# GadGadGad/Convolutional-KAN-for-Image-Classification

Measured on AMD Instinct MI355X. Metric: images/sec fwd+bwd KAN-VGG11 3x32x32 bs=256/GPU, higher is better.
Workload: dtype f32

## Files before the change

convolutional-kan-for-image-classification_amd/_lib.py:

```python
from __future__ import annotations

import ctypes as C
import os
from typing import Optional

_HERE = os.path.dirname(os.path.abspath(__file__))
LIB_PATH = os.environ.get("KANCONV_LIB") or os.path.join(_HERE, "libkanconv.so")

KAN_MAX_PLANES = 16
KAN_MAX_TABLE = 32
KAN_FP_WORDS = 192
BASIS_BSPLINE, BASIS_RBF, BASIS_CHEBY, BASIS_POLY, BASIS_FOURIER, BASIS_RELU, BASIS_GRAM = 0, 1, 2, 3, 4, 5, 6
ACT_NONE, ACT_IDENTITY, ACT_GELU, ACT_SILU, ACT_RELU, ACT_TANH, ACT_SIGMOID, ACT_GELU_TANH = -1, 0, 1, 2, 3, 4, 5, 6
ORDER_QUAD_FWD, ORDER_ROWBLK8_FWD, ORDER_QUAD_BWD_DATA, ORDER_FWD_WEIGHT_SIDE = 1, 2, 4, 8


class KanGeom(C.Structure):
    _fields_ = [(n, C.c_int) for n in ("B", "C", "H", "W", "O", "Ho", "Wo", "kh", "kw", "sh", "sw", "ph", "pw", "dh", "dw", "groups")] + \
               [("x_bstride", C.c_longlong), ("y_bstride", C.c_longlong)]


class KanBasis(C.Structure):
    _fields_ = [("kind", C.c_int), ("n_basis", C.c_int), ("order", C.c_int), ("act", C.c_int),
                ("p0", C.c_float), ("p1", C.c_float), ("table", C.c_float * KAN_MAX_TABLE), ("chan_table", C.c_void_p)]


class KanPlan(C.Structure):
    _fields_ = [(n, C.c_int) for n in ("P", "K", "IPC", "KC", "Kpad", "Opad", "fwd_splits", "bwd_data_splits", "bwd_weight_splits",
                                          "fwd_target", "bwd_data_target", "bwd_weight_target", "x_pm_wanted", "dz_pm_wanted", "bwd_weight_expanded", "row_blocks", "e_pm_wanted", "fwd_expanded", "fwd_halo", "bwd_weight_halo",
                                          "fwd_band", "bwd_weight_band")] + \
               [(n, C.c_longlong) for n in ("packed_weight_bytes", "bwd_data_weight_bytes", "fwd_slab_elems", "bwd_data_slab_elems",
                                            "bwd_weight_slab_elems", "e_pm_elems")]


class KanNormRoute(C.Structure):
    _fields_ = [(n, C.c_int) for n in ("kernel", "G", "EPL", "PPI", "NT", "pool", "lds", "held", "blocks", "strided")]


NORM_GENERIC, NORM_REGS = 0, 1
NORM_POOL_NONE, NORM_POOL_2X2, NORM_POOL_K = 0, 1, 2


class KanWavGeom(C.Structure):
    _fields_ = [(n, C.c_int) for n in ("B", "C", "H", "W", "O", "Ho", "Wo", "kh", "kw", "sh", "sw", "ph", "pw", "dh", "dw", "wavelet")] + \
               [("x_bstride", C.c_longlong), ("u_bstride", C.c_longlong)]


class KanWavRoute(C.Structure):
    _fields_ = [(n, C.c_int) for n in ("TH", "TW", "NIMG", "RH", "RW", "tiles_h", "tiles_w", "fwd_shrunk", "fwd_nimg_cut", "fwd_lds_bytes", "fwd_fits",
                                       "fwd_blocks", "bwd_input_kernel", "bwd_input_blocks", "params_kernel", "passes", "chunks", "BH", "NI", "RU",
                                       "CU", "XP", "UP", "bands", "items", "items_per_chunk", "lds_bytes", "px_per_chunk")]


WAV_BI_TAPS9, WAV_BI_STRIDE1, WAV_BI_STRIDED = 0, 1, 2
WAV_PAR_TILED, WAV_PAR_PIXEL = 0, 1


WAVELETS = {"mexican_hat": 0, "morlet": 1, "dog": 2, "meyer": 3, "shannon": 4}

_P, _I, _LL, _F, _D = C.c_void_p, C.c_int, C.c_longlong, C.c_float, C.c_double
_GP, _BP = C.POINTER(KanGeom), C.POINTER(KanBasis)
SIGNATURES = {
    "kan_version": (C.c_char_p, []),
    "kan_last_error": (C.c_char_p, []),
    "kan_plan": (_I, [_GP, _BP, C.POINTER(KanPlan)]),
    "kan_tile_orders": (_I, [_GP, _BP]),
    "kan_pack_weights": (_I, [_P, _P, _P, _P, _GP, _BP, _P]),
    "kan_pack_weights_iod": (_I, [_P, _P, _P, _GP, _BP, _P]),
    "kan_pack_cacheable": (_I, [_GP, _BP]),
    "kan_pack_weights_cached": (_I, [_P, _P, _P, _P, _GP, _BP, _P, _I, _I, _I, _P]),
    "kan_conv_fwd": (_I, [_P, _P, _P, _P, _GP, _BP, _P, _P]),
    "kan_position_major": (_I, [_P, _P, _I, _I, _I, _LL, _P]),
    "kan_conv_bwd_data": (_I, [_P, _P, _P, _P, _P, _P, _GP, _BP, _P, _P]),
    "kan_conv_bwd_data_params": (_I, [_P, _P, _P, _P, _P, _P, _P, _GP, _BP, _P, _P]),
    "kan_conv_bwd_weight": (_I, [_P, _P, _P, _P, _GP, _BP, _P, _P, _P]),
    "kan_position_major_expanded": (_I, [_P, _P, _GP, _BP, _P]),
    "kan_conv_fwd_expanded": (_I, [_P, _P, _P, _GP, _BP, _P]),
    "kan_conv_fwd_expanded_order": (_I, [_P, _P, _P, _GP, _BP, _P, _I]),
    "kan_conv_bwd_weight_expanded": (_I, [_P, _P, _P, _GP, _BP, _P]),
    "kan_unpack_wgrad": (_I, [_P, _P, _P, _GP, _BP, _P]),
    "kan_unpack_wgrad_iod": (_I, [_P, _P, _GP, _BP, _P]),
    "kan_slab_reduce": (_I, [_P, _I, _LL, _P, _I, _I, _I, _LL, _P]),
    "kan_instnorm_prelu_fwd": (_I, [_P, _I, _LL, _P, _P, _P, _P, _P, _P, _P, _I, _I, _I, _LL, _F, _I, _P]),
    "kan_instnorm_prelu_bwd": (_I, [_P, _P, _P, _P, _P, _P, _P, _P, _P, _P, _P, _I, _I, _I, _LL, _I, _P]),
    "kan_instnorm_prelu_pool_fwd": (_I, [_P, _I, _LL, _P, _P, _P, _P, _P, _P, _P, _P, _I, _I, _I, _I, _LL, _F, _I, _P]),
    "kan_instnorm_prelu_pool_bwd": (_I, [_P, _P, _P, _P, _P, _P, _P, _P, _P, _P, _P, _P, _I, _I, _I, _I, _LL, _I, _P]),
    "kan_instnorm_prelu_poolk_fwd": (_I, [_P, _I, _LL, _P, _P, _P, _P, _P, _P, _P, _P, _I, _I, _I, _I, _LL, _F, _I, _I, _I, _P]),
    "kan_instnorm_prelu_poolk_bwd": (_I, [_P, _P, _P, _P, _P, _P, _P, _P, _P, _P, _P, _P, _I, _I, _I, _I, _LL, _I, _I, _I, _P]),
    "kan_norm_route": (_I, [_I, _I, _I, _I, _I, _LL, _I, _LL, _I, _I, _I, _I, C.POINTER(KanNormRoute)]),
    "kan_batchnorm_workspace_bytes": (_LL, [_I, _I]),
    "kan_batchnorm_prelu_fwd": (_I, [_P, _I, _LL, _P, _P, _P, _P, _P, _P, _P, _P, _P, _P, _P, _I, _I, _I, _I, _LL, _F, _D, _I, _I, _P]),
    "kan_batchnorm_prelu_bwd": (_I, [_P, _P, _P, _P, _P, _P, _P, _P, _P, _P, _P, _P, _P, _I, _I, _I, _I, _LL, _I, _I, _P]),
    "kan_split_supported": (_I, [C.POINTER(KanGeom), C.POINTER(KanBasis)]),
    "kan_split_weight_bytes": (_LL, [C.POINTER(KanGeom), C.POINTER(KanBasis)]),
    "kan_split_pack_weights": (_I, [_P, _P, _P, C.POINTER(KanGeom), C.POINTER(KanBasis), _P]),
    "kan_conv_fwd_split": (_I, [_P, _P, _P, C.POINTER(KanGeom), C.POINTER(KanBasis), _P]),
    "kan_split_bwd_data_weight_bytes": (_LL, [C.POINTER(KanGeom), C.POINTER(KanBasis)]),
    "kan_split_pack_weights_bwd_data": (_I, [_P, _P, _P, C.POINTER(KanGeom), C.POINTER(KanBasis), _P]),
    "kan_conv_bwd_data_split": (_I, [_P, _P, _P, _P, C.POINTER(KanGeom), C.POINTER(KanBasis), _P]),
    "kan_split_bwd_weight_workspace_bytes": (_LL, [C.POINTER(KanGeom), C.POINTER(KanBasis)]),
    "kan_conv_bwd_weight_split": (_I, [_P, _P, _P, _P, _P, C.POINTER(KanGeom), C.POINTER(KanBasis), _P]),
    "kan_wav_fwd": (_I, [_P, _P, _P, _P, _P, C.POINTER(KanWavGeom), _P]),
    "kan_wav_bwd_input": (_I, [_P, _P, _P, _P, _P, _P, C.POINTER(KanWavGeom), _P]),
    "kan_wav_param_workspace": (_LL, [C.POINTER(KanWavGeom)]),
    "kan_wav_bwd_params": (_I, [_P, _P, _P, _P, _P, _P, _P, _P, _P, C.POINTER(KanWavGeom), _P]),
    "kan_wav_route": (_I, [C.POINTER(KanWavGeom), C.POINTER(KanWavRoute)]),
    "kan_adamw_step": (_I, [_P, _P, _P, _P, _LL, _D, _D, _D, _D, _D, _I, _F, _P]),
    "kan_adamw_step_segments": (_I, [_P, _P, _P, _P, _P, _P, _P, _P, _P, _I, _I, _D, _D, _D, _D, _D, _I, _F, _P]),
    "kan_adamw_advance": (_I, [_P, _P, _I, _P]),
    "kan_adamw_step_segments_dev": (_I, [_P, _P, _P, _P, _P, _P, _P, _P, _P, _P, _I, _I, _D, _D, _D, _D, _F, _P]),
    "kan_adamw_dev_args": (_I, [_P, _P, _D, _D, _D, _D, _F, _P, _P]),
    "kan_xent_workspace_bytes": (_LL, [_I]),
    "kan_xent_metrics_bytes": (_LL, [_I]),
    "kan_xent_fwd": (_I, [_P, _P, _I, _I, _P, _P, _P, _P, _P]),
    "kan_xent_bwd": (_I, [_P, _P, _P, _P, _P, _I, _I, _P]),
    "kan_feed_max_image_bytes": (_LL, []),
    "kan_feed_batch": (_I, [_P, _P, _P, _LL, _I, _I, _I, _I, _I, _I, _I, _P, _P, _P, _P, _P]),
    "kan_feed_resize_max_ksize": (_I, []),
    "kan_feed_resize_batch": (_I, [_P, _P, _P, _LL] + [_I] * 10 + [_P, _I] * 4 + [_P, _P, _P, _P, _P]),
}
SIGNATURES_DIGIT_NAMES = {
    "kan_set_u64_table": (_I, [_P, _I, _P, _I, _P]),
}
XENT_HEADER_WORDS = 8

_lib: Optional[C.CDLL] = None


class KanConvError(RuntimeError):
    pass


def load() -> C.CDLL:
    global _lib
    if _lib is None:
        if not os.path.exists(LIB_PATH):
            raise KanConvError(
                f"{LIB_PATH} not found: build it with `python -c 'import __graft_entry__ as g; g.build()'` "
                "(hipcc --offload-arch=gfx950).  There is no CPU / eager fallback for this path.")
        lib = C.CDLL(LIB_PATH)
        for name, (res, args) in {**SIGNATURES, **SIGNATURES_DIGIT_NAMES}.items():
            fn = getattr(lib, name)
            fn.restype, fn.argtypes = res, args
        _lib = lib
    return _lib


def check(rc: int, what: str) -> None:
    if rc != 0:
        msg = load().kan_last_error().decode(errors="replace")
        raise KanConvError(f"{what} failed (rc={rc}): {msg}")


def version() -> str:
    return load().kan_version().decode()
```

convolutional-kan-for-image-classification_amd/csrc/kan_internal.h:

```cpp
#pragma once
#include <type_traits>
#include "kanconv.h"

int kan_fail_msg(const char* fmt, const char* a);
int kan_raise_lds_limit(const void* kernel, int bytes);

enum : int {
    FAST_GENERIC = 0,
    FAST_BSPLINE_SILU = 1,
    FAST_BSPLINE_GELU = 2,
    FAST_RBF8 = 3,
    FAST_CHEBY5 = 4,
    FAST_CHEBY4 = 5,
    FAST_POLY4 = 6,
    FAST_POLY3 = 7,
    FAST_RBF5 = 8,
    FAST_RELU8 = 9,
    FAST_GRAM4 = 10,
    FAST_POLY1 = 11,
    FAST_LAST = 11
};
enum : unsigned {
    ON_TAP_MAJOR = 1u << 0,
    ON_BIG_TILES = 1u << 1,
    ON_HALO_FWD = 1u << 2,
    ON_HALO_BWD_WEIGHT = 1u << 3,
    ON_BAND_FWD = 1u << 4,
    ON_BAND_BWD_WEIGHT = 1u << 5,
    ON_EXPANDED_FWD = 1u << 6,
    ON_EXPANDED = 1u << 7,
    ON_ROWBLK_BWD_DATA = 1u << 8,
};
struct FastSpec {
    int kind, planes;
    bool base;
    bool xn_fwd, xn_bwd;
    int kc;
    unsigned routes;
};
constexpr FastSpec fast_spec(int f) {
    constexpr unsigned bspline = ON_TAP_MAJOR | ON_BIG_TILES | ON_HALO_FWD | ON_HALO_BWD_WEIGHT | ON_BAND_FWD | ON_BAND_BWD_WEIGHT |
                                 ON_EXPANDED_FWD | ON_EXPANDED | ON_ROWBLK_BWD_DATA;
    switch (f) {
        case FAST_BSPLINE_SILU: case FAST_BSPLINE_GELU: return {KAN_BASIS_BSPLINE, 9, true, false, false, 18, bspline};
        case FAST_RBF8: return {KAN_BASIS_RBF, 9, true, true, true, 18, ON_TAP_MAJOR | ON_BAND_FWD | ON_BAND_BWD_WEIGHT};
        case FAST_RBF5: return {KAN_BASIS_RBF, 6, true, true, true, 18, ON_TAP_MAJOR};
        case FAST_CHEBY5: return {KAN_BASIS_CHEBY, 5, false, false, false, 16, ON_TAP_MAJOR | ON_BIG_TILES | ON_BAND_FWD | ON_BAND_BWD_WEIGHT};
        case FAST_CHEBY4: return {KAN_BASIS_CHEBY, 4, false, false, false, 16, ON_TAP_MAJOR | ON_HALO_FWD | ON_BAND_FWD};
        case FAST_POLY4: return {KAN_BASIS_POLY, 5, true, true, false, 16, ON_TAP_MAJOR | ON_BIG_TILES | ON_HALO_FWD | ON_BAND_FWD};
        case FAST_POLY3: return {KAN_BASIS_POLY, 4, true, true, false, 16, ON_TAP_MAJOR};
        case FAST_POLY1: return {KAN_BASIS_POLY, 2, true, true, false, 16, ON_TAP_MAJOR};
        case FAST_RELU8: return {KAN_BASIS_RELU, 9, true, false, false, 16, ON_HALO_FWD | ON_HALO_BWD_WEIGHT | ON_EXPANDED_FWD | ON_EXPANDED};
        case FAST_GRAM4: return {KAN_BASIS_GRAM, 5, true, false, false, 16, ON_HALO_FWD | ON_HALO_BWD_WEIGHT | ON_EXPANDED};
        default: return {-1, 0, false, true, true, 0, 0};
    }
}
constexpr int fast_kind(int f) { return fast_spec(f).kind; }
constexpr int fast_planes(int f) { return fast_spec(f).planes; }
constexpr bool fast_has(int f, unsigned routes) { return (fast_spec(f).routes & routes) == routes && f != FAST_GENERIC; }

template <int V> using IC = std::integral_constant<int, V>;
template <unsigned ROUTES, int F = 1, class Fn>
bool dispatch_fast(int f, Fn&& fn) {
    if constexpr (F > FAST_LAST) {
        return false;
    } else {
        if constexpr (fast_has(F, ROUTES)) {
            if (f == F) { fn(IC<F>{}); return true; }
        }
        return dispatch_fast<ROUTES, F + 1>(f, fn);
    }
}
template <int V, int... REST, class Fn>
void pick(int v, Fn&& fn) {
    if constexpr (sizeof...(REST) == 0) fn(IC<V>{});
    else if (v == V) fn(IC<V>{});
    else pick<REST...>(v, fn);
}
template <class Fn>
void dispatch_kind(int kind, Fn&& fn) {
    pick<KAN_BASIS_BSPLINE, KAN_BASIS_RBF, KAN_BASIS_POLY, KAN_BASIS_FOURIER, KAN_BASIS_RELU, KAN_BASIS_GRAM, KAN_BASIS_CHEBY>(kind, fn);
}

#define KAN_BAND_MAX_TAPS 128
#define KAN_BAND_MAX_PHASES 16
typedef struct KanBandCfg {
    int ok;
    int fast, P, NG, NPLE, NPS;
    int NGR;
    int WO, MO, WP, TO, TP, NT;
    int tiles_o, tiles_p;
    int n_phase, n_taps, n_steps;
    int HC, span_r, OR0, OC0;
    int cells;
    int slots;
    int TS;
    int lds_bytes, wgs_per_cu;
    int fwd_splits;
    int bw_ok, bw_WR, bw_NI, bw_NT, bw_tiles_o, bw_row_tiles, bw_TPI, bw_ptiles, bw_cells, bw_slots, bw_lds_bytes, bw_splits;
    unsigned short bw_ph_rt0[KAN_BAND_MAX_PHASES + 1];
    unsigned char ph_a[KAN_BAND_MAX_PHASES], ph_b[KAN_BAND_MAX_PHASES];
    short ph_tap0[KAN_BAND_MAX_PHASES + 1];
    unsigned short tap_shift[KAN_BAND_MAX_TAPS];
    unsigned short tap_rt[KAN_BAND_MAX_TAPS];
    short tap_step[KAN_BAND_MAX_TAPS], tap_nt[KAN_BAND_MAX_TAPS];
} KanBandCfg;

void kan_band_cfg(const KanGeom* g, const KanBasis* b, int fast, KanBandCfg* cfg);
int kan_band_bwd_weight_launch(const float* dz, const float* x, const float* xn, float* dwp, const KanGeom* g, const KanBasis* b,
                               const KanBandCfg* cfg, int splits, long long slab_elems, void* stream);
int kan_band_fwd_launch(const float* x, const float* xn, const float* wp, float* z, const KanGeom* g, const KanBasis* b,
                        const KanBandCfg* cfg, int splits, long long slab_elems, void* stream);

constexpr int DW_T = 9;
constexpr int DW_MAX_TP = 96;

enum class Route { TAP_MAJOR, DW, BAND, HALO, EXPANDED };

struct FwdCfg { int TO, TP, tiles_o, tiles_p, chunks, splits, slots; };
struct BdCfg { int CH, tiles_c, tiles_p, n_ob, Opad32, chunks, splits; };
struct BwCfg { int TR, TO, tiles_r, tiles_o, chunks, splits, slots; };
struct BwHaloCfg { int R, nimg, spb, n_bands, tiles_r, tiles_o, splits, bands_per_split; };

struct ConvPlan {
    KanPlan pub;
    int fast;
    Route fwd, bwd_data, bwd_weight;
    bool pm_fwd, pm_bwd_data, pm_bwd_weight;
    bool rowblk_bwd_data;
    bool quad_fwd;
    bool quad_bd;
    bool rowblk8_fwd;
    bool fwd_wq;
    bool pmdma_xcd, pm_lpt, pm_xcd;
    FwdCfg fc;
    BdCfg bd;
    BwCfg bw;
    BwHaloCfg bwh;
    KanBandCfg band;
};
int plan_conv(const KanGeom* g, const KanBasis* b, ConvPlan* cp);

int live_taps_out(const KanGeom* g, int hw);
int live_taps_in(const KanGeom* g, int hw);
int live_positions_for_tap(const KanGeom* g, int tap);
int balance_tiles(const int* weight, int n, unsigned short* idx);
```

convolutional-kan-for-image-classification_amd/csrc/kanconv.hip:

```cpp
#include <hip/hip_runtime.h>
#include <cstdio>
#include <cstdlib>
#include <cstring>
#include <cmath>
#include <cstdint>
#include <mutex>
#include <type_traits>
#include <vector>
#include "kanconv.h"
#include "kan_device.h"

#include "kan_common.h"
#include "kan_internal.h"

namespace {


thread_local char g_err[512] = "";
int fail(const char* fmt, const char* a = "") {
    snprintf(g_err, sizeof(g_err), fmt, a);
    return -1;
}
}
int kan_fail_msg(const char* fmt, const char* a) { return fail(fmt, a); }

int kan_raise_lds_limit(const void* kernel, int bytes) {
    struct Raised { const void* kernel; int device, bytes; };
    static std::mutex mu;
    static std::vector<Raised> raised;
    int dev = 0;
    if (hipGetDevice(&dev) != hipSuccess) return -1;
    std::lock_guard<std::mutex> lock(mu);
    for (const Raised& r : raised)
        if (r.kernel == kernel && r.device == dev && r.bytes >= bytes) return 0;
    if (hipFuncSetAttribute(kernel, hipFuncAttributeMaxDynamicSharedMemorySize, bytes) != hipSuccess) return -1;
    raised.push_back(Raised{kernel, dev, bytes});
    return 0;
}
namespace {

struct PackGeo { int O, C, T, P, hb, nb, IPC, KC, Opad, pair, cmajor; FastDiv divT, divNb, divIPC, divP;
                 int band; short tap_step[KAN_BAND_MAX_TAPS], tap_nt[KAN_BAND_MAX_TAPS]; };

__device__ __forceinline__ int wp_row(const PackGeo& q, int tap, int c, int p) {
    if (q.band) {
        const int grp = fastdiv(c, q.divIPC);
        return (q.tap_step[tap] + grp * q.tap_nt[tap]) * q.KC + (c - grp * q.IPC) * q.P + p;
    }
    if (q.pair) return ((c >> 1) * q.T + tap) * q.KC + 2 * p + (c & 1);
    if (q.cmajor) return (c * q.T + tap) * q.P + p;
    const int item = tap * q.C + c;
    const int chunk = fastdiv(item, q.divIPC);
    return chunk * q.KC + (item - chunk * q.IPC) * q.P + p;
}
__device__ __forceinline__ int pack_row(const PackGeo& q, int src_kind, int j) {
    int cq = fastdiv(j, q.divT), tap = j - cq * q.T;
    int c = src_kind == 0 ? cq : fastdiv(cq, q.divNb);
    int p = src_kind == 0 ? 0 : q.hb + (cq - c * q.nb);
    return wp_row(q, tap, c, p);
}

constexpr int FP_LANES = 64;
__global__ __launch_bounds__(256) void k_fingerprint(const float* __restrict__ a, unsigned na, const float* __restrict__ b, unsigned nb,
                                                     unsigned stride, unsigned long long* __restrict__ ring, int cur) {
    __shared__ unsigned part[2][4];
    if (blockIdx.x == 0 && threadIdx.x < FP_LANES) ring[((cur + 1) % 3) * FP_LANES + threadIdx.x] = 0ull;
    unsigned h1 = 0u, h2 = 0u;
    auto fold = [&](unsigned w, unsigned p) { h1 += w * (2u * p + 1u); h2 += __builtin_rotateleft32(w, p & 31u); };
    constexpr int U = 8;
    const unsigned nthreads = gridDim.x * 256u, tid0 = blockIdx.x * 256u + threadIdx.x;
    auto pass = [&](const float* __restrict__ src, unsigned n, unsigned pos_base) {
        const unsigned nfull = n / 4u, ngr = (nfull + stride - 1u) / stride;
        for (unsigned i0 = tid0; i0 < ngr; i0 += nthreads * U) {
            float4 v[U]; unsigned e[U]; bool ok[U];
#pragma unroll
            for (int u = 0; u < U; ++u) {
                const unsigned i = i0 + u * nthreads;
                ok[u] = i < ngr;
                e[u] = (ok[u] ? i : ngr - 1u) * stride * 4u;
                v[u] = *reinterpret_cast<const float4*>(src + e[u]);
            }
#pragma unroll
            for (int u = 0; u < U; ++u) {
                const unsigned p = pos_base + e[u];
                if (ok[u]) { fold(__float_as_uint(v[u].x), p); fold(__float_as_uint(v[u].y), p + 1u); fold(__float_as_uint(v[u].z), p + 2u); fold(__float_as_uint(v[u].w), p + 3u); }
            }
        }
        if (tid0 == 0u) for (unsigned k = nfull * 4u; k < n; ++k) fold(__float_as_uint(src[k]), pos_base + k);
    };
    if (na) pass(a, na, 0u);
    pass(b, nb, na);
#pragma unroll
    for (int off = 32; off >= 1; off >>= 1) { h1 += __shfl_xor(h1, off, 64); h2 += __shfl_xor(h2, off, 64); }
    if ((threadIdx.x & 63) == 0) { part[0][threadIdx.x >> 6] = h1; part[1][threadIdx.x >> 6] = h2; }
    __syncthreads();
    if (threadIdx.x == 0) {
        const unsigned s1 = part[0][0] + part[0][1] + part[0][2] + part[0][3], s2 = part[1][0] + part[1][1] + part[1][2] + part[1][3];
        unsigned* w = reinterpret_cast<unsigned*>(ring + cur * FP_LANES + (blockIdx.x % FP_LANES));
        atomicAdd(w, s1);
        atomicAdd(w + 1, s2);
    }
}
__device__ __forceinline__ bool fp_unchanged(const unsigned long long* fp, int cur) {
    __shared__ int same;
    if (!fp) return false;
    if (threadIdx.x < 64) {
        const int t = threadIdx.x;
        unsigned lo_c = 0, hi_c = 0, lo_p = 0, hi_p = 0;
        if (t < FP_LANES) {
            const unsigned long long c = fp[cur * FP_LANES + t], p = fp[((cur + 2) % 3) * FP_LANES + t];
            lo_c = (unsigned)c; hi_c = (unsigned)(c >> 32); lo_p = (unsigned)p; hi_p = (unsigned)(p >> 32);
        }
#pragma unroll
        for (int off = 32; off >= 1; off >>= 1) {
            lo_c += __shfl_xor(lo_c, off, 64); hi_c += __shfl_xor(hi_c, off, 64);
            lo_p += __shfl_xor(lo_p, off, 64); hi_p += __shfl_xor(hi_p, off, 64);
        }
        if (t == 0) same = (lo_c == lo_p && hi_c == hi_p) ? 1 : 0;
    }
    __syncthreads();
    return same != 0;
}

__global__ __launch_bounds__(256) void k_pack(const float* __restrict__ src_base, const float* __restrict__ src_basis,
                                              float* __restrict__ wp, PackGeo q, int nb_base, long long wp_gstride, int tiles_x, int tiles_y,
                                              const unsigned long long* __restrict__ fp, int fp_cur) {
    __shared__ float tile[32][33];
    if (fp_unchanged(fp, fp_cur)) return;
    wp += (size_t)blockIdx.z * wp_gstride;
    const int tx = threadIdx.x & 31, ty = threadIdx.x >> 5;
    for (int tile_id = blockIdx.x; tile_id < tiles_x * tiles_y; tile_id += gridDim.x) {
        const int by = tile_id / tiles_x, bx0 = tile_id - by * tiles_x;
        const int src_kind = bx0 < nb_base ? 0 : 1;
        const int bx = src_kind == 0 ? bx0 : bx0 - nb_base;
        const int J = src_kind == 0 ? q.C * q.T : q.C * q.nb * q.T;
        const float* src = (src_kind == 0 ? src_base : src_basis) + (size_t)blockIdx.z * q.O * J;
        const int j0 = bx * 32, o0 = by * 32;
#pragma unroll
        for (int i = 0; i < 4; ++i) {
            int o = o0 + ty + 8 * i, j = j0 + tx;
            tile[ty + 8 * i][tx] = (o < q.O && j < J) ? src[(size_t)o * J + j] : 0.f;
        }
        __syncthreads();
#pragma unroll
        for (int i = 0; i < 4; ++i) {
            int j = j0 + ty + 8 * i, o = o0 + tx;
            if (j < J && o < q.Opad) wp[(size_t)pack_row(q, src_kind, j) * q.Opad + o] = tile[tx][ty + 8 * i];
        }
        __syncthreads();
    }
}

constexpr int UNPACK_TO = 64, UNPACK_TJ = 32;
__device__ __forceinline__ float4 f4_add(float4 a, float4 b) { return make_float4(a.x + b.x, a.y + b.y, a.z + b.z, a.w + b.w); }
template <int N>
__device__ __forceinline__ void unpack_tail(float4& r0, float4& r1, const float* a0, const float* a1, long long slab_elems) {
    float4 v0[N], v1[N];
#pragma unroll
    for (int i = 0; i < N; ++i) {
        v0[i] = *reinterpret_cast<const float4*>(a0 + (size_t)i * slab_elems);
        v1[i] = *reinterpret_cast<const float4*>(a1 + (size_t)i * slab_elems);
    }
#pragma unroll
    for (int i = 0; i < N; ++i) { r0 = f4_add(r0, v0[i]); r1 = f4_add(r1, v1[i]); }
}
__global__ __launch_bounds__(256) void k_unpack(const float* __restrict__ dwp, float* __restrict__ dst_base, float* __restrict__ dst_basis,
                                                PackGeo q, int nb_base, int n_slabs, long long slab_elems, long long dwp_gstride) {
    __shared__ float tile[UNPACK_TO][UNPACK_TJ + 1];
    const int src_kind = (int)blockIdx.x < nb_base ? 0 : 1;
    const int bx = src_kind == 0 ? blockIdx.x : blockIdx.x - nb_base;
    const int J = src_kind == 0 ? q.C * q.T : q.C * q.nb * q.T;
    dwp += (size_t)blockIdx.z * dwp_gstride;
    float* dst = (src_kind == 0 ? dst_base : dst_basis) + (size_t)blockIdx.z * q.O * J;
    const int j0 = bx * UNPACK_TJ, o0 = blockIdx.y * UNPACK_TO;
    const int ol = 4 * (threadIdx.x & 15), jl = threadIdx.x >> 4;
    const float* a0 = dwp + (size_t)pack_row(q, src_kind, min(j0 + jl, J - 1)) * q.Opad + o0 + ol;
    const float* a1 = dwp + (size_t)pack_row(q, src_kind, min(j0 + jl + 16, J - 1)) * q.Opad + o0 + ol;
    const float4 zero = make_float4(0.f, 0.f, 0.f, 0.f);
    float4 s[2][8];
#pragma unroll
    for (int i = 0; i < 8; ++i) s[0][i] = s[1][i] = zero;
    int sl = 0;
    for (; sl + 8 <= n_slabs; sl += 8) {
        float4 v[2][8];
#pragma unroll
        for (int i = 0; i < 8; ++i) {
            v[0][i] = *reinterpret_cast<const float4*>(a0 + (size_t)(sl + i) * slab_elems);
            v[1][i] = *reinterpret_cast<const float4*>(a1 + (size_t)(sl + i) * slab_elems);
        }
#pragma unroll
        for (int i = 0; i < 8; ++i) { s[0][i] = f4_add(s[0][i], v[0][i]); s[1][i] = f4_add(s[1][i], v[1][i]); }
    }
    {
        const float* b0 = a0 + (size_t)sl * slab_elems;
        const float* b1 = a1 + (size_t)sl * slab_elems;
        switch (n_slabs - sl) {
            case 1: unpack_tail<1>(s[0][0], s[1][0], b0, b1, slab_elems); break;
            case 2: unpack_tail<2>(s[0][0], s[1][0], b0, b1, slab_elems); break;
            case 3: unpack_tail<3>(s[0][0], s[1][0], b0, b1, slab_elems); break;
            case 4: unpack_tail<4>(s[0][0], s[1][0], b0, b1, slab_elems); break;
            case 5: unpack_tail<5>(s[0][0], s[1][0], b0, b1, slab_elems); break;
            case 6: unpack_tail<6>(s[0][0], s[1][0], b0, b1, slab_elems); break;
            case 7: unpack_tail<7>(s[0][0], s[1][0], b0, b1, slab_elems); break;
            default: break;
        }
    }
#pragma unroll
    for (int r = 0; r < 2; ++r) {
        const float4 t = f4_add(f4_add(f4_add(s[r][0], s[r][1]), f4_add(s[r][2], s[r][3])), f4_add(f4_add(s[r][4], s[r][5]), f4_add(s[r][6], s[r][7])));
        const int j = jl + 16 * r;
        tile[ol][j] = t.x; tile[ol + 1][j] = t.y; tile[ol + 2][j] = t.z; tile[ol + 3][j] = t.w;
    }
    __syncthreads();
    const int tx = threadIdx.x & 31, ty = threadIdx.x >> 5;
#pragma unroll
    for (int i = 0; i < UNPACK_TO / 8; ++i) {
        const int o = o0 + ty + 8 * i, j = j0 + tx;
        if (o < q.O && j < J) dst[(size_t)o * J + j] = tile[ty + 8 * i][tx];
    }
}

__global__ __launch_bounds__(256) void k_fold_slabs(float* __restrict__ slabs, int n_slabs, long long slab_elems, long long n) {
    __shared__ float part[4][64];
    const int e = threadIdx.x & 63, sg = threadIdx.x >> 6;
    const long long i = (long long)blockIdx.x * 64 + e;
    float a0 = 0.f, a1 = 0.f, a2 = 0.f, a3 = 0.f;
    if (i < n) {
        const float* p = slabs + i;
        int sl = sg;
        for (; sl + 12 < n_slabs; sl += 16) {
            a0 += p[(size_t)sl * slab_elems]; a1 += p[(size_t)(sl + 4) * slab_elems];
            a2 += p[(size_t)(sl + 8) * slab_elems]; a3 += p[(size_t)(sl + 12) * slab_elems];
        }
        for (; sl < n_slabs; sl += 4) a0 += p[(size_t)sl * slab_elems];
    }
    part[sg][e] = (a0 + a1) + (a2 + a3);
    __syncthreads();
    if (sg == 0 && i < n) slabs[i] = (part[0][e] + part[1][e]) + (part[2][e] + part[3][e]);
}

constexpr int IOD_TO = 256, IOD_PITCH = IOD_TO + 4;

__device__ __forceinline__ float4 iod_ld4(const float* p, bool vec) {
    return vec ? *reinterpret_cast<const float4*>(p) : make_float4(p[0], p[1], p[2], p[3]);
}
__device__ __forceinline__ void iod_st4(float* p, float4 v, bool vec) {
    if (vec) *reinterpret_cast<float4*>(p) = v;
    else { p[0] = v.x; p[1] = v.y; p[2] = v.z; p[3] = v.w; }
}
__device__ __forceinline__ float4 iod_add4(float4 a, float4 b) { return make_float4(a.x + b.x, a.y + b.y, a.z + b.z, a.w + b.w); }

struct IodTile { int c, o0, no, wq; };
__device__ __forceinline__ IodTile iod_tile(const PackGeo& q, long long tile_id, int o_tiles) {
    IodTile t;
    t.c = (int)(tile_id / o_tiles);
    t.o0 = (int)(tile_id - (long long)t.c * o_tiles) * IOD_TO;
    t.no = max(0, min(IOD_TO, q.O - t.o0));
    t.wq = min(IOD_TO, q.Opad - t.o0) >> 2;
    return t;
}

__global__ __launch_bounds__(256) void k_pack_iod(const float* __restrict__ coeffs, float* __restrict__ wp, PackGeo q, int o_tiles, long long n_tiles,
                                                  int vec) {
    __shared__ __attribute__((aligned(16))) float tile[KAN_MAX_PLANES * IOD_PITCH];
    const int n = q.nb, tid = threadIdx.x;
    for (long long tile_id = blockIdx.x; tile_id < n_tiles; tile_id += gridDim.x) {
        const IodTile t = iod_tile(q, tile_id, o_tiles);
        const float* src = coeffs + ((size_t)t.c * q.O + t.o0) * n;
        const int cnt = t.no * n;
        auto put = [&](int f, float v) { const int o = fastdiv(f, q.divNb); tile[(f - o * n) * IOD_PITCH + o] = v; };
        if (vec & 1) {
            for (int f = 4 * tid; f < cnt; f += 1024) {
                const float4 v = *reinterpret_cast<const float4*>(src + f);
                put(f, v.x); put(f + 1, v.y); put(f + 2, v.z); put(f + 3, v.w);
            }
        } else {
            for (int f = tid; f < cnt; f += 256) put(f, src[f]);
        }
        __syncthreads();
        for (int u = tid; u < n * t.wq; u += 256) {
            const int p = t.wq == IOD_TO / 4 ? u >> 6 : u / t.wq, o = 4 * (u - p * t.wq);
            float4 v = *reinterpret_cast<const float4*>(&tile[p * IOD_PITCH + o]);
            if (o + 3 >= t.no) { if (o >= t.no) v.x = 0.f; if (o + 1 >= t.no) v.y = 0.f; if (o + 2 >= t.no) v.z = 0.f; v.w = 0.f; }
            iod_st4(wp + (size_t)wp_row(q, 0, t.c, p) * q.Opad + t.o0 + o, v, vec & 2);
        }
        __syncthreads();
    }
}

__global__ __launch_bounds__(256) void k_unpack_iod(const float* __restrict__ dwp, float* __restrict__ dcoeffs, PackGeo q, int o_tiles, long long n_tiles,
                                                    int n_slabs, long long slab_elems, int vec) {
    __shared__ __attribute__((aligned(16))) float tile[KAN_MAX_PLANES * IOD_PITCH];
    const int n = q.nb, tid = threadIdx.x;
    for (long long tile_id = blockIdx.x; tile_id < n_tiles; tile_id += gridDim.x) {
        const IodTile t = iod_tile(q, tile_id, o_tiles);
        for (int u = tid; u < n * t.wq; u += 256) {
            const int p = t.wq == IOD_TO / 4 ? u >> 6 : u / t.wq, o = 4 * (u - p * t.wq);
            if (o >= t.no) continue;
            const float* a = dwp + (size_t)wp_row(q, 0, t.c, p) * q.Opad + t.o0 + o;
            const bool v2 = vec & 2;
            const float4 z = make_float4(0.f, 0.f, 0.f, 0.f);
            float4 s0 = z, s1 = z, s2 = z, s3 = z, s4 = z, s5 = z, s6 = z, s7 = z;
            int sl = 0;
            for (; sl + 8 <= n_slabs; sl += 8) {
                const float* b = a + (size_t)sl * slab_elems;
                s0 = iod_add4(s0, iod_ld4(b, v2)); s1 = iod_add4(s1, iod_ld4(b + slab_elems, v2));
                s2 = iod_add4(s2, iod_ld4(b + 2 * slab_elems, v2)); s3 = iod_add4(s3, iod_ld4(b + 3 * slab_elems, v2));
                s4 = iod_add4(s4, iod_ld4(b + 4 * slab_elems, v2)); s5 = iod_add4(s5, iod_ld4(b + 5 * slab_elems, v2));
                s6 = iod_add4(s6, iod_ld4(b + 6 * slab_elems, v2)); s7 = iod_add4(s7, iod_ld4(b + 7 * slab_elems, v2));
            }
            for (; sl < n_slabs; ++sl) s0 = iod_add4(s0, iod_ld4(a + (size_t)sl * slab_elems, v2));
            *reinterpret_cast<float4*>(&tile[p * IOD_PITCH + o]) =
                iod_add4(iod_add4(iod_add4(s0, s1), iod_add4(s2, s3)), iod_add4(iod_add4(s4, s5), iod_add4(s6, s7)));
        }
        __syncthreads();
        float* dst = dcoeffs + ((size_t)t.c * q.O + t.o0) * n;
        const int cnt = t.no * n;
        auto get = [&](int f) { const int o = fastdiv(f, q.divNb); return tile[(f - o * n) * IOD_PITCH + o]; };
        if (vec & 1) {
            for (int f = 4 * tid; f < cnt; f += 1024) *reinterpret_cast<float4*>(dst + f) = make_float4(get(f), get(f + 1), get(f + 2), get(f + 3));
        } else {
            for (int f = tid; f < cnt; f += 256) dst[f] = get(f);
        }
        __syncthreads();
    }
}

__global__ __launch_bounds__(256) void k_pack_bwd_data(const float* __restrict__ wp, float* __restrict__ wd, PackGeo q,
                                                       int CH, int n_ct, int Opad32, long long wp_gstride, int tiles_x, int tiles_y,
                                                       const unsigned long long* __restrict__ fp, int fp_cur) {
    __shared__ float tile[32][33];
    if (fp_unchanged(fp, fp_cur)) return;
    const int tap = blockIdx.z;
    const int tx = threadIdx.x & 31, ty = threadIdx.x >> 5;
    const int ncol = n_ct * 128;
    const float* const wp0 = wp; float* const wd0 = wd;
    for (int tile_id = blockIdx.x; tile_id < tiles_x * tiles_y; tile_id += gridDim.x) {
    const int byy = tile_id / tiles_x, bxx = tile_id - byy * tiles_x;
    const int oblk = Opad32 / 32, grp = byy / oblk;
    const int col0 = bxx * 32, o0 = (byy - grp * oblk) * 32;
    wp = wp0 + (size_t)grp * wp_gstride;
    wd = wd0 + (size_t)grp * q.T * Opad32 * ncol;
#pragma unroll
    for (int i = 0; i < 4; ++i) {
        int col = col0 + ty + 8 * i, o = o0 + tx;
        float v = 0.f;
        if (col < ncol) {
            int hf = col >> 6, w = col & 63, cl = fastdiv(w, q.divP), p = w - cl * q.P, c = hf * CH + cl;
            if (cl < CH && c < q.C && o < q.O) {
                v = wp[(size_t)wp_row(q, tap, c, p) * q.Opad + o];
            }
        }
        tile[ty + 8 * i][tx] = v;
    }
    __syncthreads();
#pragma unroll
    for (int i = 0; i < 4; ++i) {
        int o = o0 + ty + 8 * i, col = col0 + tx;
// ... 1210 lines not shown
    };

    f32x16 acc[2][2];
#pragma unroll
    for (int a = 0; a < 2; ++a)
#pragma unroll
        for (int b = 0; b < 2; ++b)
#pragma unroll
            for (int r = 0; r < 16; ++r) acc[a][b][r] = 0.f;

    unsigned tapmask = 0;
    for (int tap = 0; tap < T; ++tap) tapmask |= (tap_alive_out(g, pos, tap) ? 1u : 0u) << tap;
    auto seg = [&](int tap) { return (tap * g.C + 1) / 2; };
    int ch0, ch1;
    {
        const int L = live_step_count(tapmask, T, n_chunks, seg);
        const int S = min((int)gridDim.z, max(1, (L + chunks_per_split - 1) / chunks_per_split));
        if (blk.z >= S) { ch0 = ch1 = n_chunks; }
        else {
            ch0 = blk.z == 0 ? 0 : live_step_pos(tapmask, T, n_chunks, (int)((long long)L * blk.z / S), seg);
            ch1 = blk.z == S - 1 ? n_chunks : live_step_pos(tapmask, T, n_chunks, (int)((long long)L * (blk.z + 1) / S), seg);
        }
    }
    auto next_live = [&](int ch) -> int {
        while (ch < ch1) {
            const int tap = (2 * ch) / g.C;
            if ((tapmask >> tap) & 1u) return ch;
            ch = ((tap + 1) * g.C) / 2;
        }
        return ch1;
    };
    int ch = next_live(ch0);
    if (ch < ch1) issue(ch, 0);
    const int ao = w_o * 64 + (lane & 31), bp = w_p * 64 + (lane & 31);
    for (int cur = 0; ch < ch1; cur ^= 1) {
        asm volatile("s_waitcnt vmcnt(0)" ::: "memory");
        __syncthreads();
        ch = next_live(ch + 1);
        if (ch < ch1) issue(ch, cur ^ 1);
        const unsigned aw = lds_addr(sW + cur * (KC * TO) + kh2 * TO + ao), ae = lds_addr(sE + cur * (KC * TP) + kh2 * TP + bp);
        KAN_MFMA_STEP(KC / 2, aw, TO, ae, TP);
    }

    float* zs = z + (size_t)blk.z * slab_elems;
#pragma unroll
    for (int ni = 0; ni < 2; ++ni) {
        const int b = b0 + w_p * 64 + ni * 32 + (lane & 31);
        if (b >= g.B) continue;
        float* zb = zs + (size_t)b * g.ybs + pos;
#pragma unroll
        for (int mi = 0; mi < 2; ++mi)
#pragma unroll
            for (int r = 0; r < 16; ++r) {
                const int o = o_tile0 + w_o * 64 + mi * 32 + mfma_row(r, lane);
                if (o < g.O) zb[(size_t)o * HoWo] = acc[mi][ni][r];
            }
    }
}

template <int KC>
__global__ __launch_bounds__(256, 4) void k_conv_fwd_pmdma_wq(
    const float* __restrict__ e_pm, const float* __restrict__ wp, float* __restrict__ z, DevGeom g, int Opad, int n_chunks,
    int chunks_per_split, long long slab_elems, unsigned e_bytes, unsigned w_bytes, int tiles_o, int xcd) {
    constexpr int TO = 128, TP = 128, NQ = KC / 2, P = KC / 2, HW = 4;
    __shared__ __attribute__((aligned(16))) float sW[2 * KC * TO];
    __shared__ __attribute__((aligned(16))) float sE[2 * KC * TP];
    const int tid = threadIdx.x, lane = tid & 63;
    const int wave = __builtin_amdgcn_readfirstlane(tid >> 6);
    const int w_o = wave >> 1, w_p = wave & 1, kh2 = lane >> 5;
    const BlockId blk = xcd_block_order(xcd != 0);
    const int grp = blk.y / tiles_o, tiles_b = g.B / TP;
    const int sub = blk.x / tiles_b, b0 = (blk.x - sub * tiles_b) * TP;
    const int o_tile0 = ((blk.y - grp * tiles_o) * 4 + sub) * 32;
    const int pairs = g.C >> 1;
    e_pm += (size_t)grp * g.C * HW * P * g.B;
    z += (size_t)grp * g.O * HW;
    wp += (size_t)grp * n_chunks * KC * Opad;
    const kan_rsrc e_rs = make_rsrc(e_pm, e_bytes), w_rs = make_rsrc(wp, w_bytes);

    unsigned eoff[(NQ + 3) / 4];
#pragma unroll
    for (int j = 0; j < (NQ + 3) / 4; ++j) {
        const int r = min(2 * (j * 4 + wave) + (lane >> 5), KC - 1), cl = r / P, pp = r - cl * P;
        eoff[j] = (unsigned)(((cl * HW) * P + pp) * g.B + (lane & 31) * 4) * 4u;
    }
    unsigned woff;
    {
        const int col = (lane & 31) * 4, q = (col >> 4) & 3, o_l = (col >> 6) * 16 + (col & 15);
        const int tap0 = (1 - (q >> 1)) * 3 + (1 - (q & 1));
        woff = (unsigned)((tap0 * pairs * KC + (lane >> 5)) * Opad + o_l) * 4u;
    }
    auto issue = [&](int p, int pair, int buf) {
        const int se = __builtin_amdgcn_readfirstlane((((2 * pair * HW + p) * P) * g.B + b0) * 4);
        const int sw = __builtin_amdgcn_readfirstlane(((((3 * (p >> 1) + (p & 1)) * pairs + pair) * KC) * Opad + o_tile0) * 4);
        float* dE = sE + buf * (KC * TP);
        float* dW = sW + buf * (KC * TO);
#pragma unroll
        for (int j = 0; j < (NQ + 3) / 4; ++j) {
            const int q = j * 4 + wave;
            if (q < NQ) {
                __builtin_amdgcn_raw_ptr_buffer_load_lds(e_rs, (__attribute__((address_space(3))) void*)(dE + q * 256), 16, (int)eoff[j], se, 0, 0);
                __builtin_amdgcn_raw_ptr_buffer_load_lds(w_rs, (__attribute__((address_space(3))) void*)(dW + q * 256), 16, (int)woff,
                                                         sw + q * 2 * Opad * 4, 0, 0);
            }
        }
    };

    f32x16 acc[2][2];
#pragma unroll
    for (int a = 0; a < 2; ++a)
#pragma unroll
        for (int b = 0; b < 2; ++b)
#pragma unroll
            for (int r = 0; r < 16; ++r) acc[a][b][r] = 0.f;

    int ch0, ch1;
    {
        const int L = HW * pairs;
        const int S = min((int)gridDim.z, max(1, (L + chunks_per_split - 1) / chunks_per_split));
        if (blk.z >= S) { ch0 = ch1 = L; }
        else {
            ch0 = (int)((long long)L * blk.z / S);
            ch1 = blk.z == S - 1 ? L : (int)((long long)L * (blk.z + 1) / S);
        }
    }
    int p = ch0 / pairs, pair = ch0 - p * pairs;
    int ch = ch0;
    if (ch < ch1) issue(p, pair, 0);
    const int ao = w_o * 64 + (lane & 31), bp = w_p * 64 + (lane & 31);
    for (int cur = 0; ch < ch1; cur ^= 1) {
        asm volatile("s_waitcnt vmcnt(0)" ::: "memory");
        __syncthreads();
        ++ch;
        if (++pair == pairs) { pair = 0; ++p; }
        if (ch < ch1) issue(p, pair, cur ^ 1);
        const unsigned aw = lds_addr(sW + cur * (KC * TO) + kh2 * TO + ao), ae = lds_addr(sE + cur * (KC * TP) + kh2 * TP + bp);
        KAN_MFMA_STEP(KC / 2, aw, TO, ae, TP);
    }

    float* zs = z + (size_t)blk.z * slab_elems;
#pragma unroll
    for (int ni = 0; ni < 2; ++ni) {
        const int b = b0 + w_p * 64 + ni * 32 + (lane & 31);
        if (b >= g.B) continue;
        float* zb = zs + (size_t)b * g.ybs;
#pragma unroll
        for (int r = 0; r < 8; ++r) {
            const int o = o_tile0 + w_o * 16 + mfma_row(r, lane);
            if (o < g.O) *reinterpret_cast<float4*>(zb + (size_t)o * 4) = make_float4(acc[0][ni][r], acc[0][ni][r + 8], acc[1][ni][r], acc[1][ni][r + 8]);
        }
    }
}

constexpr int PM_ORDER_MAX = 72;
struct PmOrder { int n, tiles_r_per_tap, xcd; unsigned char tap[PM_ORDER_MAX], z[PM_ORDER_MAX]; int first[PM_ORDER_MAX + 1]; };

typedef float f32x4 __attribute__((ext_vector_type(4)));
__global__ __launch_bounds__(256, 4) void k_conv_bwd_weight_pmdma(
    const float* __restrict__ dz_pm, const float* __restrict__ e_pm, float* __restrict__ dwp, DevGeom g, int P, FastDiv divP, int Krows, int Opad,
    int n_chunks, int chunks_per_split, long long slab_elems, unsigned e_bytes, unsigned dz_bytes, int tiles_o, int max_splits, PmOrder ord) {
    constexpr int TR = 128, TO = 128, KPX = 16, ZB = KPX * TO, AB = KPX * TR;
    __shared__ __attribute__((aligned(16))) float sA[2 * AB];
    __shared__ __attribute__((aligned(16))) float sZ[2 * ZB];
    const int tid = threadIdx.x, lane = tid & 63;
    const int wave = __builtin_amdgcn_readfirstlane(tid >> 6);
    const int w_r = wave >> 1, w_c = wave & 1, kh2 = lane >> 5;
    const int HoWo = g.Ho * g.Wo, HW = g.H * g.W, CP = g.C * P;
    BlockId blk{(int)blockIdx.x, (int)blockIdx.y, (int)blockIdx.z};
    if (ord.n) {
        const int lin = (int)blockIdx.x;
        int e = 0;
        while (e + 1 < ord.n && lin >= ord.first[e + 1]) ++e;
        const int rel0 = lin - ord.first[e], per = ord.first[e + 1] - ord.first[e], ny = per / ord.tiles_r_per_tap;
        const int rel = ((per & 7) == 0 && (ord.first[e] & 7) == 0 && ord.xcd) ? (rel0 & 7) * (per >> 3) + (rel0 >> 3) : rel0;
        const int xr = rel / ny, y = rel - xr * ny;
        blk.x = (int)ord.tap[e] * ord.tiles_r_per_tap + xr; blk.y = y; blk.z = (int)ord.z[e];
    }
    const int grp = blk.y / tiles_o;
    const int k0 = blk.x * TR, o_tile0 = (blk.y - grp * tiles_o) * TO;
    e_pm += (size_t)grp * g.C * HW * P * g.B;
    dz_pm += (size_t)grp * g.O * HoWo * g.B;
    dwp += (size_t)grp * Krows * Opad;
    const int tap = k0 / CP, tr = tap / g.kw, tt = tap - tr * g.kw;
    const kan_rsrc e_rs = make_rsrc(e_pm, e_bytes), dz_rs = make_rsrc(dz_pm, dz_bytes);

    unsigned aoff[2], zoff[2];
#pragma unroll
    for (int j = 0; j < 2; ++j) {
        const int rl = 16 * (wave * 2 + j) + (lane >> 2), cs = (lane & 3) ^ ((rl >> 2) & 3);
        const int row = k0 + rl, rem = min(row, Krows - 1) - tap * CP, c = fastdiv(rem, divP), pp = rem - c * P;
        const unsigned va = (unsigned)(((c * HW) * P + pp) * g.B + cs * 4) * 4u, vz = (unsigned)((o_tile0 + rl) * HoWo * g.B + cs * 4) * 4u;
        aoff[j] = row < Krows ? va : KAN_OOB;
        zoff[j] = o_tile0 + rl < g.O ? vz : KAN_OOB;
    }
    unsigned aA[2][2], bB[2][2];
#pragma unroll
    for (int mi = 0; mi < 2; ++mi) {
        const int rl = w_r * 64 + mi * 32 + (lane & 31), ol = w_c * 64 + mi * 32 + (lane & 31);
#pragma unroll
        for (int h = 0; h < 2; ++h) {
            aA[mi][h] = lds_addr(sA + rl * KPX + (((2 * h + kh2) ^ ((rl >> 2) & 3)) * 4));
            bB[mi][h] = lds_addr(sZ + ol * KPX + (((2 * h + kh2) ^ ((ol >> 2) & 3)) * 4));
        }
    }
    auto issue = [&](int ch, int buf) {
        const int px = ch * KPX, pos = px / g.B, b0 = px - pos * g.B;
        const int ho = pos / g.Wo, wo = pos - ho * g.Wo;
        const int inpos = (ho * g.sh - g.ph + tr * g.dh) * g.W + (wo * g.sw - g.pw + tt * g.dw);
        const int sa = __builtin_amdgcn_readfirstlane((inpos * P * g.B + b0) * 4), sz = __builtin_amdgcn_readfirstlane((pos * g.B + b0) * 4);
        float* dA = sA + buf * AB + wave * (2 * 256);
        float* dZ = sZ + buf * ZB + wave * (2 * 256);
#pragma unroll
        for (int j = 0; j < 2; ++j) {
            __builtin_amdgcn_raw_ptr_buffer_load_lds(e_rs, (__attribute__((address_space(3))) void*)(dA + j * 256), 16, (int)aoff[j], sa, 0, 0);
            __builtin_amdgcn_raw_ptr_buffer_load_lds(dz_rs, (__attribute__((address_space(3))) void*)(dZ + j * 256), 16, (int)zoff[j], sz, 0, 0);
        }
    };

    f32x16 acc[2][2];
#pragma unroll
    for (int a = 0; a < 2; ++a)
#pragma unroll
        for (int b = 0; b < 2; ++b)
#pragma unroll
            for (int r = 0; r < 16; ++r) acc[a][b][r] = 0.f;

    unsigned hwmask = 0;
    for (int hw = 0; hw < HoWo; ++hw) hwmask |= (tap_alive_out(g, hw, tap) ? 1u : 0u) << hw;
    auto seg = [&](int hw) { return (hw * g.B + KPX - 1) / KPX; };
    int ch0, ch1;
    {
        const int L = live_step_count(hwmask, HoWo, n_chunks, seg);
        const int S = min(max_splits, max(1, (L + chunks_per_split - 1) / chunks_per_split));
        if (blk.z >= S) { ch0 = ch1 = n_chunks; }
        else {
            ch0 = blk.z == 0 ? 0 : live_step_pos(hwmask, HoWo, n_chunks, (int)((long long)L * blk.z / S), seg);
            ch1 = blk.z == S - 1 ? n_chunks : live_step_pos(hwmask, HoWo, n_chunks, (int)((long long)L * (blk.z + 1) / S), seg);
        }
    }
    auto next_live = [&](int ch) -> int {
        while (ch < ch1) {
            const int hw = (ch * KPX) / g.B;
            if ((hwmask >> hw) & 1u) return ch;
            ch = ((hw + 1) * g.B) / KPX;
        }
        return ch1;
    };
    int ch = next_live(ch0);
    if (ch < ch1) issue(ch, 0);
#define KAN_RD4(CUR, h_)                                                                                                    \
    asm volatile("ds_read_b128 %0, %4 offset:%8\n\tds_read_b128 %1, %5 offset:%8\n\tds_read_b128 %2, %6 offset:%8\n\tds_read_b128 %3, %7 offset:%8" \
                 : "=&v"(fa[h_][0]), "=&v"(fa[h_][1]), "=&v"(fb[h_][0]), "=&v"(fb[h_][1])                                      \
                 : "v"(aA[0][h_]), "v"(aA[1][h_]), "v"(bB[0][h_]), "v"(bB[1][h_]), "n"((CUR) * AB * 4) : "memory")
#define KAN_PM_HALF(h_)                                                                                                     \
    _Pragma("unroll") for (int e = 0; e < 4; ++e) {                                                                          \
        acc[0][0] = MFMA32(fa[h_][0][e], fb[h_][0][e], acc[0][0]);                                                            \
        acc[0][1] = MFMA32(fa[h_][0][e], fb[h_][1][e], acc[0][1]);                                                            \
        acc[1][0] = MFMA32(fa[h_][1][e], fb[h_][0][e], acc[1][0]);                                                            \
        acc[1][1] = MFMA32(fa[h_][1][e], fb[h_][1][e], acc[1][1]);                                                            \
    }
#define KAN_PM_STEP(CUR)                                                                                     \
    do {                                                                                                     \
        asm volatile("s_waitcnt vmcnt(0)" ::: "memory");                                                     \
        __syncthreads();                                                                                     \
        ch = next_live(ch + 1);                                                                              \
        if (ch < ch1) issue(ch, (CUR) ^ 1);                                                                  \
        f32x4 fa[2][2], fb[2][2];                                                                            \
        KAN_RD4(CUR, 0);                                                                                     \
        KAN_RD4(CUR, 1);                                                                                     \
        asm volatile("s_waitcnt lgkmcnt(4)" : "+v"(fa[0][0]), "+v"(fa[0][1]), "+v"(fb[0][0]), "+v"(fb[0][1]) :: "memory"); \
        KAN_PM_HALF(0)                                                                                       \
        asm volatile("s_waitcnt lgkmcnt(0)" : "+v"(fa[1][0]), "+v"(fa[1][1]), "+v"(fb[1][0]), "+v"(fb[1][1]) :: "memory"); \
        KAN_PM_HALF(1)                                                                                       \
    } while (0)
    static_assert(AB == ZB, "one immediate serves both operands");
    while (ch < ch1) {
        KAN_PM_STEP(0);
        if (ch < ch1) { KAN_PM_STEP(1); }
    }
#undef KAN_PM_STEP
#undef KAN_PM_HALF
#undef KAN_RD4

    float* out = dwp + (size_t)blk.z * slab_elems;
#pragma unroll
    for (int mi = 0; mi < 2; ++mi)
#pragma unroll
        for (int r = 0; r < 16; ++r) {
            const int row = k0 + w_r * 64 + mi * 32 + mfma_row(r, lane);
            if (row >= Krows) continue;
#pragma unroll
            for (int ni = 0; ni < 2; ++ni) {
                const int o = o_tile0 + w_c * 64 + ni * 32 + (lane & 31);
                out[(size_t)row * Opad + o] = acc[mi][ni][r];
            }
        }
}


__device__ __forceinline__ int dw_krow(int tap, int p, int IPC, int KC, int P) {
    const int chunk = tap / IPC;
    return chunk * KC + (tap - chunk * IPC) * P + p;
}

template <int KIND>
__global__ __launch_bounds__(256) void k_dw_fwd(const float* __restrict__ x, const float* __restrict__ xn, const float* __restrict__ wp,
                                                float* __restrict__ z, DevGeom g, DevBasis bs, int Opad, int IPC, int KC, int Kpad) {
    __shared__ float sTab[KAN_MAX_TABLE];
    __shared__ float sWt[DW_MAX_TP * 2];
    const int grp = blockIdx.y, T = g.kh * g.kw, P = bs.P, HoWo = g.Ho * g.Wo, HW = g.H * g.W;
    if (threadIdx.x < KAN_MAX_TABLE) sTab[threadIdx.x] = bs.tab[threadIdx.x];
    for (int i = threadIdx.x; i < T * P * 2; i += 256) {
        const int o = i & 1, tp = i >> 1, tap = tp / P, p = tp - tap * P;
        sWt[i] = o < g.O ? wp[((size_t)grp * Kpad + dw_krow(tap, p, IPC, KC, P)) * Opad + o] : 0.f;
    }
    __syncthreads();
    const int e = blockIdx.x * 256 + threadIdx.x;
    if (e >= g.B * HoWo) return;
    const int b = e / HoWo, hw = e - b * HoWo, ho = hw / g.Wo, wo = hw - ho * g.Wo;
    const size_t xbase = (size_t)b * g.xbs + (size_t)grp * HW;
    float acc0 = 0.f, acc1 = 0.f;
    for (int tap = 0; tap < T; ++tap) {
        const int r = tap / g.kw, t = tap - r * g.kw;
        const int hi = ho * g.sh - g.ph + r * g.dh, wi = wo * g.sw - g.pw + t * g.dw;
        if ((unsigned)hi >= (unsigned)g.H || (unsigned)wi >= (unsigned)g.W) continue;
        const float xa = x[xbase + hi * g.W + wi], xb = xn[xbase + hi * g.W + wi];
        float v[KAN_PMAX];
        kan_planes<KIND, false>(bs, sTab, xa, xb, v);
#pragma unroll
        for (int p = 0; p < KAN_PMAX; ++p)
            if (p < P) { acc0 += v[p] * sWt[(tap * P + p) * 2]; acc1 += v[p] * sWt[(tap * P + p) * 2 + 1]; }
    }
    float* zb = z + (size_t)b * g.ybs + (size_t)grp * g.O * HoWo + hw;
    zb[0] = acc0;
    if (g.O > 1) zb[HoWo] = acc1;
}

template <int KIND>
__global__ __launch_bounds__(256) void k_dw_bwd_data(const float* __restrict__ dz, const float* __restrict__ x, const float* __restrict__ xn,
                                                     const float* __restrict__ wp, float* __restrict__ dx, float* __restrict__ dxn,
                                                     DevGeom g, DevBasis bs, int Opad, int IPC, int KC, int Kpad) {
    __shared__ float sTab[KAN_MAX_TABLE];
    __shared__ float sWt[DW_MAX_TP * 2];
    const int grp = blockIdx.y, T = g.kh * g.kw, P = bs.P, HoWo = g.Ho * g.Wo, HW = g.H * g.W;
    if (threadIdx.x < KAN_MAX_TABLE) sTab[threadIdx.x] = bs.tab[threadIdx.x];
    for (int i = threadIdx.x; i < T * P * 2; i += 256) {
        const int o = i & 1, tp = i >> 1, tap = tp / P, p = tp - tap * P;
        sWt[i] = o < g.O ? wp[((size_t)grp * Kpad + dw_krow(tap, p, IPC, KC, P)) * Opad + o] : 0.f;
    }
    __syncthreads();
    const int e = blockIdx.x * 256 + threadIdx.x;
    if (e >= g.B * HW) return;
    const int b = e / HW, hw = e - b * HW, h = hw / g.W, w = hw - h * g.W;
    const size_t xi = (size_t)b * g.xbs + (size_t)grp * HW + hw;
    float G[KAN_PMAX];
#pragma unroll
    for (int p = 0; p < KAN_PMAX; ++p) G[p] = 0.f;
    for (int tap = 0; tap < T; ++tap) {
        const int r = tap / g.kw, t = tap - r * g.kw;
        const int hn = h + g.ph - r * g.dh, wn = w + g.pw - t * g.dw;
        if (hn < 0 || wn < 0) continue;
        const int ho = hn / g.sh, wo = wn / g.sw;
        if (ho * g.sh != hn || wo * g.sw != wn || ho >= g.Ho || wo >= g.Wo) continue;
        const float* zb = dz + (size_t)b * g.ybs + (size_t)grp * g.O * HoWo + ho * g.Wo + wo;
        const float d0 = zb[0], d1 = g.O > 1 ? zb[HoWo] : 0.f;
#pragma unroll
        for (int p = 0; p < KAN_PMAX; ++p)
            if (p < P) G[p] += d0 * sWt[(tap * P + p) * 2] + d1 * sWt[(tap * P + p) * 2 + 1];
    }
    float d[KAN_PMAX];
    kan_planes<KIND, true>(bs, sTab, x[xi], xn[xi], d);
    float s_base = 0.f, s_bas = 0.f;
#pragma unroll
    for (int p = 0; p < KAN_PMAX; ++p)
        if (p < P) { if (p < bs.hb) s_base += d[p] * G[p]; else s_bas += d[p] * G[p]; }
    if (dxn) { dx[xi] = s_base; dxn[xi] = s_bas; }
    else dx[xi] = s_base + s_bas;
}

template <int KIND>
__global__ __launch_bounds__(256) void k_dw_bwd_weight(const float* __restrict__ dz, const float* __restrict__ x, const float* __restrict__ xn,
                                                       float* __restrict__ dwp, DevGeom g, DevBasis bs, int Krows, int Opad,
                                                       long long slab_elems) {
    __shared__ float sTab[KAN_MAX_TABLE];
    __shared__ float sRed[4][DW_T * KAN_PMAX];
    const int grp = blockIdx.y, T = g.kh * g.kw, P = bs.P, HoWo = g.Ho * g.Wo, HW = g.H * g.W;
    const int lane = threadIdx.x & 63, wave = threadIdx.x >> 6;
    if (threadIdx.x < KAN_MAX_TABLE) sTab[threadIdx.x] = bs.tab[threadIdx.x];
    __syncthreads();
    float* out = dwp + (size_t)blockIdx.x * slab_elems + (size_t)grp * Krows * Opad;
    const int total = g.B * HoWo;
    for (int o = 0; o < g.O; ++o) {
        float acc[DW_T][KAN_PMAX];
#pragma unroll
        for (int a = 0; a < DW_T; ++a)
#pragma unroll
            for (int p = 0; p < KAN_PMAX; ++p) acc[a][p] = 0.f;
        for (int e = blockIdx.x * 256 + threadIdx.x; e < total; e += gridDim.x * 256) {
            const int b = e / HoWo, hw = e - b * HoWo, ho = hw / g.Wo, wo = hw - ho * g.Wo;
            const float dzv = dz[(size_t)b * g.ybs + (size_t)(grp * g.O + o) * HoWo + hw];
            const size_t xbase = (size_t)b * g.xbs + (size_t)grp * HW;
#pragma unroll
            for (int tap = 0; tap < DW_T; ++tap) {
                if (tap < T) {
                    const int r = tap / g.kw, t = tap - r * g.kw;
                    const int hi = ho * g.sh - g.ph + r * g.dh, wi = wo * g.sw - g.pw + t * g.dw;
                    if ((unsigned)hi < (unsigned)g.H && (unsigned)wi < (unsigned)g.W) {
                        float v[KAN_PMAX];
                        kan_planes<KIND, false>(bs, sTab, x[xbase + hi * g.W + wi], xn[xbase + hi * g.W + wi], v);
#pragma unroll
                        for (int p = 0; p < KAN_PMAX; ++p) acc[tap][p] += v[p] * dzv;
                    }
                }
            }
        }
#pragma unroll
        for (int a = 0; a < DW_T; ++a)
#pragma unroll
            for (int p = 0; p < KAN_PMAX; ++p) {
                float v = acc[a][p];
#pragma unroll
                for (int off = 32; off >= 1; off >>= 1) v += __shfl_xor(v, off, 64);
                if (lane == 0) sRed[wave][a * KAN_PMAX + p] = v;
            }
        __syncthreads();
        for (int i = threadIdx.x; i < T * P; i += 256) {
            const int tap = i / P, p = i - tap * P, q = tap * KAN_PMAX + p;
            out[(size_t)i * Opad + o] = (sRed[0][q] + sRed[1][q]) + (sRed[2][q] + sRed[3][q]);
        }
        __syncthreads();
    }
}

__global__ __launch_bounds__(256) void k_slab_reduce(const float* __restrict__ slabs, int n_slabs, long long slab_elems,
                                                     float* __restrict__ out, int Cn, int HW, long long bstride, long long total) {
    const long long plane = (long long)Cn * HW;
    for (long long i = blockIdx.x * 256ll + threadIdx.x; i < total; i += (long long)gridDim.x * 256) {
        long long b = i / plane, rem = i - b * plane;
        size_t a = (size_t)b * bstride + rem;
        float s = 0.f;
        for (int sl = 0; sl < n_slabs; ++sl) s += slabs[a + (size_t)sl * slab_elems];
        out[a] = s;
    }
}


struct PoolGeo { int k, s, Hp, Wp, nc; FastDiv divWp, divS, divK, divNc; int lds; };

template <int G>
// ... 640 lines not shown
            float4 P = ((float4*)p)[i], G = ((const float4*)g)[i], M = ((float4*)m)[i], V = ((float4*)v)[i];
            adam1(P.x, G.x, M.x, V.x, a); adam1(P.y, G.y, M.y, V.y, a); adam1(P.z, G.z, M.z, V.z, a); adam1(P.w, G.w, M.w, V.w, a);
            ((float4*)p)[i] = P; ((float4*)m)[i] = M; ((float4*)v)[i] = V;
        }
        const int t = (n & ~3) + threadIdx.x;
        if (t < n) adam1(p[t], g[t], m[t], v[t], a);
    } else {
        for (int i = threadIdx.x; i < n; i += 256) adam1(p[i], g[i], m[i], v[i], a);
    }
}

__global__ void k_adamw_dev_args(const double* __restrict__ lr_dev, const int* __restrict__ step_dev, AdamHyper h, float* __restrict__ out9) {
    if (threadIdx.x != 0 || blockIdx.x != 0) return;
    const AdamArgs a = adam_args_dev(lr_dev[0], step_dev[0], h);
    out9[0] = a.decay; out9[1] = a.w1; out9[2] = a.b1; out9[3] = a.b2; out9[4] = a.w2; out9[5] = a.gscale; out9[6] = a.inv_bc2_sqrt; out9[7] = a.eps;
    out9[8] = a.neg_step;
}

struct U64x64 { unsigned long long v[64]; };
__global__ __launch_bounds__(64) void k_set_u64_table(unsigned long long* __restrict__ table, int first, int n, U64x64 vals) {
    const int t = threadIdx.x;
    if (t < n) table[first + t] = vals.v[t];
}

#include "wavkan.inc"

}

extern "C" {

const char* kan_version(void) { return "kanconv 0.5 (gfx950, fp32 MFMA 32x32x2, halo forward, 128/256-output tiles)"; }
const char* kan_last_error(void) { return g_err; }

int kan_plan(const KanGeom* geom, const KanBasis* basis, KanPlan* plan) {
    if (!plan) return fail("null plan");
    ConvPlan cp;
    if (int rc = plan_conv(geom, basis, &cp)) return rc;
    *plan = cp.pub;
    return 0;
}

static bool pack_needs_clear(const KanGeom* g, const KanPlan& pl) {
    if (pl.fwd_band) return pl.KC != pl.IPC * pl.P || g->C % pl.IPC != 0;
    return pl.KC != pl.IPC * pl.P || (g->C * g->kh * g->kw) % pl.IPC != 0;
}

static int iod_scope(const KanGeom* g, const KanBasis* b) {
    if (!g || !b) return fail("null geometry or basis");
    if (g->kh != 1 || g->kw != 1) return fail("the [I][O][n] coefficient layout takes 1x1 kernels only");
    if (ngroups(g) != 1) return fail("the [I][O][n] coefficient layout takes one group only");
    if (b->act != KAN_ACT_NONE) return fail("the [I][O][n] coefficient layout has no base branch (act must be KAN_ACT_NONE)");
    return 0;
}
struct IodLaunch { int o_tiles; long long n_tiles; unsigned blocks; };
static IodLaunch iod_launch(const KanGeom* g, const KanPlan& pl) {
    IodLaunch l;
    l.o_tiles = ceil_div(pl.Opad, IOD_TO);
    l.n_tiles = (long long)g->C * l.o_tiles;
    l.blocks = (unsigned)(l.n_tiles < 16384 ? l.n_tiles : 16384);
    return l;
}
static int iod_vec(const void* coeffs, const void* packed, const KanGeom* g, const KanBasis* b) {
    return ((((size_t)coeffs & 15) == 0 && ((long long)g->O * b->n_basis) % 4 == 0) ? 1 : 0) | ((((size_t)packed & 15) == 0) ? 2 : 0);
}

static int pack_weights_impl(const float* w_base, const float* w_basis, float* wp, float* wd, const KanGeom* g, const KanBasis* b,
                             const unsigned long long* fp, int fp_cur, void* stream, bool iod = false) {
    ConvPlan cp;
    if (int rc = plan_conv(g, b, &cp)) return rc;
    const KanPlan& pl = cp.pub;
    const int hb = b->act != KAN_ACT_NONE;
    if ((hb && !w_base) || !w_basis || !wp) return fail("null weight pointer");
    hipStream_t st = (hipStream_t)stream;
    const int T = g->kh * g->kw, NI = g->C * T, G = ngroups(g);
    const long long wp_gs = (long long)pl.Kpad * pl.Opad;
    PackGeo q = pack_geo(g, b, cp, false);
    if (fp && (pack_needs_clear(g, pl) || cp.fwd == Route::DW)) return fail("cached packing is not offered for this geometry (kan_pack_cacheable)");
    if (pl.KC != pl.IPC * pl.P || (pl.fwd_band && pack_needs_clear(g, pl))) {
        if (hipMemsetAsync(wp, 0, (size_t)pl.packed_weight_bytes, st) != hipSuccess) return fail("memset failed");
    } else if (!pl.fwd_band && NI % pl.IPC != 0) {
        if (G > 1) {
            if (hipMemsetAsync(wp, 0, (size_t)pl.packed_weight_bytes, st) != hipSuccess) return fail("memset failed");
        } else {
            size_t off = (size_t)(pl.Kpad - pl.KC) * pl.Opad;
            if (hipMemsetAsync(wp + off, 0, (size_t)pl.KC * pl.Opad * 4, st) != hipSuccess) return fail("memset failed");
        }
    }
    const int nb_base = hb ? ceil_div(g->C * T, 32) : 0;
    const int tiles_x = nb_base + ceil_div(g->C * b->n_basis * T, 32), tiles_y = pl.Opad / 32;
    const long long n_tiles = (long long)tiles_x * tiles_y;
    const long long cap = fp ? 1024 : 4096;
    dim3 grid((unsigned)(n_tiles < cap ? n_tiles : cap), 1, G);
    if (iod) {
        const IodLaunch l = iod_launch(g, pl);
        hipLaunchKernelGGL(k_pack_iod, dim3(l.blocks), dim3(256), 0, st, w_basis, wp, q, l.o_tiles, l.n_tiles, iod_vec(w_basis, wp, g, b));
    } else {
        hipLaunchKernelGGL(k_pack, grid, dim3(256), 0, st, w_base, w_basis, wp, q, nb_base, wp_gs, tiles_x, tiles_y, fp, fp_cur);
    }
    if (wd && cp.bwd_data == Route::DW) {
        if (hipMemcpyAsync(wd, wp, (size_t)pl.packed_weight_bytes, hipMemcpyDeviceToDevice, st) != hipSuccess) return fail("memcpy failed");
    } else if (wd) {
        const BdCfg& c = cp.bd;
        const int bx = c.tiles_c * 4, by = c.Opad32 / 32 * G;
        const long long nt = (long long)bx * by;
        const long long capd = fp ? 128 : 1024;
        dim3 gd((unsigned)(nt < capd ? nt : capd), 1, T);
        hipLaunchKernelGGL(k_pack_bwd_data, gd, dim3(256), 0, st, (const float*)wp, wd, q, c.CH, c.tiles_c, c.Opad32, wp_gs, bx, by, fp, fp_cur);
    }
    return launch_ok("pack");
}

int kan_pack_weights(const float* w_base, const float* w_basis, float* wp, float* wd, const KanGeom* g, const KanBasis* b, void* stream) {
    return pack_weights_impl(w_base, w_basis, wp, wd, g, b, nullptr, 0, stream);
}

int kan_pack_weights_iod(const float* coeffs, float* wp, float* wd, const KanGeom* g, const KanBasis* b, void* stream) {
    if (int rc = iod_scope(g, b)) return rc;
    return pack_weights_impl(nullptr, coeffs, wp, wd, g, b, nullptr, 0, stream, true);
}

int kan_tile_orders(const KanGeom* g, const KanBasis* b) {
    ConvPlan cp;
    if (plan_conv(g, b, &cp)) return 0;
    const bool halo = cp.fwd == Route::HALO;
    return (halo && cp.quad_fwd ? KAN_ORDER_QUAD_FWD : 0) | (halo && cp.rowblk8_fwd ? KAN_ORDER_ROWBLK8_FWD : 0) | (cp.quad_bd ? KAN_ORDER_QUAD_BWD_DATA : 0) |
           (cp.fwd_wq ? KAN_ORDER_FWD_WEIGHT_SIDE : 0);
}

int kan_pack_cacheable(const KanGeom* g, const KanBasis* b) {
    ConvPlan cp;
    if (plan_conv(g, b, &cp)) return 0;
    if ((long long)g->O * g->C * (b->n_basis + 1) * g->kh * g->kw >= (1ll << 31)) return 0;
    return (!pack_needs_clear(g, cp.pub) && cp.fwd != Route::DW && ngroups(g) == 1) ? 1 : 0;
}

int kan_pack_weights_cached(const float* w_base, const float* w_basis, float* wp, float* wd, const KanGeom* g, const KanBasis* b,
                            unsigned long long* ring, int cur, int force, int sample_stride, void* stream) {
    static_assert(KAN_FP_WORDS == 3 * FP_LANES, "ring size");
    if (!ring || cur < 0 || cur > 2 || sample_stride < 1) return fail("bad fingerprint ring arguments");
    if (!kan_pack_cacheable(g, b)) return fail("cached packing is not offered for this geometry (kan_pack_cacheable)");
    const int hb = b->act != KAN_ACT_NONE;
    if ((hb && !w_base) || !w_basis) return fail("null weight pointer");
    if (((size_t)w_basis & 15) || (hb && ((size_t)w_base & 15))) return fail("cached packing needs 16-byte aligned weight tensors");
    const int T = g->kh * g->kw;
    const long long na = hb ? (long long)g->O * g->C * T : 0, nbs = (long long)g->O * g->C * b->n_basis * T;
    const long long groups4 = ((na + 3) / 4 + (nbs + 3) / 4 + sample_stride - 1) / sample_stride;
    long long blocks = (groups4 + 256 * 8 - 1) / (256 * 8); if (blocks > 4096) blocks = 4096; if (blocks < 1) blocks = 1;
    hipLaunchKernelGGL(k_fingerprint, dim3((unsigned)blocks), dim3(256), 0, (hipStream_t)stream, hb ? w_base : w_basis, (unsigned)na, w_basis,
                       (unsigned)nbs, (unsigned)sample_stride, ring, cur);
    if (int rc = launch_ok("fingerprint")) return rc;
    return pack_weights_impl(w_base, w_basis, wp, wd, g, b, force ? nullptr : ring, cur, stream);
}

static int unpack_wgrad_impl(const float* dwp, float* dw_base, float* dw_basis, const KanGeom* g, const KanBasis* b, void* stream, bool iod) {
    ConvPlan cp;
    if (int rc = plan_conv(g, b, &cp)) return rc;
    const KanPlan& pl = cp.pub;
    const int hb = b->act != KAN_ACT_NONE;
    if ((hb && !dw_base) || !dw_basis || !dwp) return fail("null weight-gradient pointer");
    hipStream_t st = (hipStream_t)stream;
    const int T = g->kh * g->kw, G = ngroups(g);
    const long long dwp_gs = (long long)(pl.bwd_weight_band ? pl.Kpad : pl.K) * pl.Opad;
    PackGeo q = pack_geo(g, b, cp, true);
    int n_slabs = pl.bwd_weight_splits;
    if (n_slabs >= 32) {
        hipLaunchKernelGGL(k_fold_slabs, dim3(ceil_div(pl.bwd_weight_slab_elems, 64)), dim3(256), 0, st, const_cast<float*>(dwp), n_slabs,
                           pl.bwd_weight_slab_elems, pl.bwd_weight_slab_elems);
        n_slabs = 1;
    }
    const int nb_base = hb ? ceil_div(g->C * T, UNPACK_TJ) : 0;
    dim3 grid(nb_base + ceil_div(g->C * b->n_basis * T, UNPACK_TJ), ceil_div(g->O, UNPACK_TO), G);
    if (iod) {
        const IodLaunch l = iod_launch(g, pl);
        hipLaunchKernelGGL(k_unpack_iod, dim3(l.blocks), dim3(256), 0, st, dwp, dw_basis, q, l.o_tiles, l.n_tiles, n_slabs, pl.bwd_weight_slab_elems,
                           iod_vec(dw_basis, dwp, g, b));
    } else {
        hipLaunchKernelGGL(k_unpack, grid, dim3(256), 0, st, dwp, dw_base, dw_basis, q, nb_base, n_slabs, pl.bwd_weight_slab_elems, dwp_gs);
    }
    return launch_ok("unpack");
}

int kan_unpack_wgrad(const float* dwp, float* dw_base, float* dw_basis, const KanGeom* g, const KanBasis* b, void* stream) {
    return unpack_wgrad_impl(dwp, dw_base, dw_basis, g, b, stream, false);
}

int kan_unpack_wgrad_iod(const float* dwp, float* dcoeffs, const KanGeom* g, const KanBasis* b, void* stream) {
    if (int rc = iod_scope(g, b)) return rc;
    return unpack_wgrad_impl(dwp, nullptr, dcoeffs, g, b, stream, true);
}

int kan_position_major(const float* src, float* dst, int B, int Cn, int HW, long long bstride, void* stream) {
    if (!src || !dst || B < 1 || Cn < 1 || HW < 1) return fail("bad position_major arguments");
    dim3 grid(ceil_div((long long)Cn * HW, 32), ceil_div(B, 32));
    hipLaunchKernelGGL(k_position_major, grid, dim3(256), 0, (hipStream_t)stream, src, dst, B, Cn * HW, bstride);
    return launch_ok("position_major");
}

int kan_conv_fwd(const float* x, const float* xn, const float* wp, float* z, const KanGeom* g, const KanBasis* b, const float* x_pm,
                 void* stream) {
    ConvPlan cp;
    if (int rc = plan_conv(g, b, &cp)) return rc;
    const KanPlan& pl = cp.pub;
    if (!x || !xn || !wp || !z) return fail("null tensor pointer");
    if ((b->kind == KAN_BASIS_RELU || b->kind == KAN_BASIS_GRAM) && !b->chan_table) return fail("ReLU / Gram bases need their device parameter table (chan_table)");
    hipStream_t st = (hipStream_t)stream;
    if (cp.fwd == Route::DW) {
        DevGeom dgd = dev_geom(g); DevBasis dbd = dev_basis(b);
        dim3 grid(ceil_div((long long)g->B * g->Ho * g->Wo, 256), ngroups(g));
        dispatch_kind(b->kind, [&](auto kind) {
            hipLaunchKernelGGL((k_dw_fwd<decltype(kind)::value>), grid, dim3(256), 0, st, x, xn, wp, z, dgd, dbd, pl.Opad, pl.IPC, pl.KC, pl.Kpad);
        });
        return launch_ok("dw_fwd");
    }
    if (cp.fwd == Route::BAND) {
        if (x != xn && !fast_spec(cp.fast).xn_fwd) return fail("this basis / activation pair runs on single-input kernels: pass xn == x");
        return kan_band_fwd_launch(x, xn, wp, z, g, b, &cp.band, pl.fwd_splits, pl.fwd_slab_elems, stream);
    }
    const FwdCfg& c = cp.fc;
    if ((long long)c.tiles_o * ngroups(g) > 65535) return fail("groups * output tiles exceed the grid limit");
    const unsigned x_bytes = (unsigned)((long long)g->B * g->x_bstride * 4);
    if (cp.fwd == Route::HALO) {
        if (x != xn) return fail("internal: halo forward kernel needs a single input tensor");
        DevGeom dgh = dev_geom(g); DevBasis dbh = dev_basis(b);
        const int n_pairs = g->C / 2, pps = ceil_div(n_pairs, pl.fwd_splits);
        dim3 gridh(c.tiles_p, c.tiles_o * ngroups(g), pl.fwd_splits);
        dispatch_fast<ON_HALO_FWD>(cp.fast, [&](auto fv) {
            constexpr int F = decltype(fv)::value;
            auto launch = [&](auto wo, auto w, auto r, auto nimg, auto quad) {
                constexpr int WOV = decltype(wo)::value;
                hipLaunchKernelGGL((k_conv_fwd_halo<F, WOV, decltype(w)::value, decltype(r)::value, decltype(nimg)::value, decltype(quad)::value>), gridh,
                                   dim3(WOV * 128), 0, st, x, wp, z, dgh, dbh, pl.Opad, n_pairs, pps, pl.fwd_slab_elems, x_bytes, c.tiles_o);
            };
            auto planes = [&](auto wo) {
                if constexpr (decltype(wo)::value == 4) {
                    if (g->W == 4 && cp.quad_fwd && ((uintptr_t)z & 7u) == 0 && (g->y_bstride & 1) == 0 && (pl.fwd_slab_elems & 1) == 0)
                        return launch(wo, IC<4>{}, IC<4>{}, IC<8>{}, IC<1>{});
                }
                if (g->W == 32) launch(wo, IC<32>{}, IC<4>{}, IC<1>{}, IC<0>{});
                else if (g->W == 16) launch(wo, IC<16>{}, IC<8>{}, IC<1>{}, IC<0>{});
                else if (g->W == 8) {
                    if constexpr (decltype(wo)::value == 4) {
                        if (cp.rowblk8_fwd) return launch(wo, IC<8>{}, IC<4>{}, IC<4>{}, IC<0>{});
                    }
                    launch(wo, IC<8>{}, IC<8>{}, IC<2>{}, IC<0>{});
                }
                else launch(wo, IC<4>{}, IC<4>{}, IC<8>{}, IC<0>{});
            };
            if constexpr (fast_has(F, ON_BIG_TILES)) {
                if (c.TO == 256) return planes(IC<4>{});
            }
            planes(IC<2>{});
        });
        return launch_ok("conv_fwd_halo");
    }
    DevGeom dg = dev_geom(g);
    dg.pix_major = (x_pm && x == xn && cp.pm_fwd) ? 1 : 0;
    if (dg.pix_major) { x = x_pm; xn = x_pm; }
    DevBasis db = dev_basis(b);
    dim3 grid(c.tiles_p, c.tiles_o * ngroups(g), pl.fwd_splits);
    const int cps = dg.pix_major ? pl.fwd_target : ceil_div(c.chunks, pl.fwd_splits);
    TilePerm perm; perm.n = 0;
    if (dg.pix_major) perm = tile_perm(c.tiles_p, [&](int t) {
        const int hw = (int)(((long long)t * c.TP) / g->B);
        return ceil_div(live_taps_out(g, hw < g->Ho * g->Wo ? hw : 0) * ceil_div(g->C, pl.IPC), cps > 0 ? cps : 1);
    });
    if (x != xn && !fast_spec(cp.fast).xn_fwd)
        return fail("this basis / activation pair runs on single-input kernels: pass xn == x");
    auto launch = [&](auto kind, auto fast, auto wo, auto kc) {
        constexpr int WO = decltype(wo)::value;
        hipLaunchKernelGGL((k_conv_fwd<decltype(kind)::value, decltype(fast)::value, WO, 2, decltype(kc)::value>), grid, dim3(WO * 2 * 64), 0, st,
                           x, xn, wp, z, dg, db, pl.Opad, pl.IPC, c.chunks, cps, pl.fwd_slab_elems, x_bytes, perm, c.tiles_o);
    };
    const bool fast = dispatch_fast<ON_TAP_MAJOR>(cp.fast, [&](auto fv) {
        constexpr int F = decltype(fv)::value;
        if constexpr (fast_has(F, ON_BIG_TILES)) {
            if (c.TO == 256) return launch(IC<fast_kind(F)>{}, fv, IC<4>{}, IC<fast_spec(F).kc>{});
        }
        if (c.TO == 128) launch(IC<fast_kind(F)>{}, fv, IC<2>{}, IC<fast_spec(F).kc>{});
        else launch(IC<fast_kind(F)>{}, fv, IC<1>{}, IC<fast_spec(F).kc>{});
    });
    if (!fast) dispatch_kind(b->kind, [&](auto kind) {
        pick<18, 12, 16>(pl.KC, [&](auto kc) {
            if (c.TO == 128) launch(kind, IC<FAST_GENERIC>{}, IC<2>{}, kc);
            else launch(kind, IC<FAST_GENERIC>{}, IC<1>{}, kc);
        });
    });
    return launch_ok("conv_fwd");
}

static int conv_bwd_data_impl(const float* dz, const float* x, const float* xn, const float* wd, float* dx, float* dxn, float* dpar,
                              const KanGeom* g, const KanBasis* b, const float* dz_pm, void* stream);

int kan_conv_bwd_data(const float* dz, const float* x, const float* xn, const float* wd, float* dx, float* dxn,
                      const KanGeom* g, const KanBasis* b, const float* dz_pm, void* stream) {
    return conv_bwd_data_impl(dz, x, xn, wd, dx, dxn, nullptr, g, b, dz_pm, stream);
}

int kan_conv_bwd_data_params(const float* dz, const float* x, const float* xn, const float* wd, float* dx, float* dxn, float* dparams,
                             const KanGeom* g, const KanBasis* b, const float* dz_pm, void* stream) {
    if (!dparams) return fail("null dparams");
    if (b && b->kind != KAN_BASIS_RELU && b->kind != KAN_BASIS_GRAM) return fail("kan_conv_bwd_data_params: only the ReLU-KAN and GRAM bases accumulate parameter gradients in this launch");
    return conv_bwd_data_impl(dz, x, xn, wd, dx, dxn, dparams, g, b, dz_pm, stream);
}

static int conv_bwd_data_impl(const float* dz, const float* x, const float* xn, const float* wd, float* dx, float* dxn, float* dpar,
                              const KanGeom* g, const KanBasis* b, const float* dz_pm, void* stream) {
    ConvPlan cp;
    if (int rc = plan_conv(g, b, &cp)) return rc;
    const KanPlan& pl = cp.pub;
    if (dpar && cp.bwd_data == Route::DW) return fail("kan_conv_bwd_data_params: depthwise layers take the weight-gradient route");
    if (!dz || !x || !xn || !wd || !dx) return fail("null tensor pointer");
    if ((b->kind == KAN_BASIS_RELU || b->kind == KAN_BASIS_GRAM) && !b->chan_table) return fail("ReLU / Gram bases need their device parameter table (chan_table)");
    if (!dxn && x != xn) return fail("dxn is required when xn != x");
    hipStream_t st = (hipStream_t)stream;
    if (cp.bwd_data == Route::DW) {
        DevGeom dgd = dev_geom(g); DevBasis dbd = dev_basis(b);
        dim3 grid(ceil_div((long long)g->B * g->H * g->W, 256), ngroups(g));
        dispatch_kind(b->kind, [&](auto kind) {
            hipLaunchKernelGGL((k_dw_bwd_data<decltype(kind)::value>), grid, dim3(256), 0, st, dz, x, xn, wd, dx, dxn, dgd, dbd, pl.Opad, pl.IPC, pl.KC, pl.Kpad);
        });
        return launch_ok("dw_bwd_data");
    }
    const BdCfg& c = cp.bd;
    DevGeom dg = dev_geom(g);
    dg.pix_major = (dz_pm && cp.pm_bwd_data) ? 1 : 0;
    if (dg.pix_major) dz = dz_pm;
    DevBasis db = dev_basis(b);
    if ((long long)c.tiles_c * ngroups(g) > 65535) return fail("groups * channel tiles exceed the grid limit");
    dim3 grid(c.tiles_p, c.tiles_c * ngroups(g), pl.bwd_data_splits);
    const int cps = dg.pix_major ? pl.bwd_data_target : ceil_div(c.chunks, pl.bwd_data_splits);
    TilePerm perm; perm.n = 0;
    if (dg.pix_major) perm = tile_perm(c.tiles_p, [&](int t) {
        const int hw = (int)(((long long)t * 128) / g->B);
        return ceil_div(live_taps_in(g, hw < g->H * g->W ? hw : 0) * c.n_ob, cps > 0 ? cps : 1);
    });
    const int fast = (fast_spec(cp.fast).xn_bwd ? (x != xn && dxn) : (x == xn && !dxn)) ? cp.fast : FAST_GENERIC;
    const bool rb = !dg.pix_major && cp.rowblk_bwd_data;
    const bool quad = rb && cp.quad_bd && dz_pm && x == xn && !dxn;
    const unsigned dz_bytes = (unsigned)((long long)g->B * g->y_bstride * 4);
    auto launch = [&](auto kind, auto fast, auto rbv) {
        hipLaunchKernelGGL((k_conv_bwd_data<decltype(kind)::value, decltype(fast)::value, decltype(rbv)::value>), grid, dim3(256), 0, st,
                           decltype(rbv)::value == 2 ? dz_pm : dz, x, xn, wd,
                           dx, dxn, dg, db, c.CH, c.tiles_c, c.n_ob, c.Opad32, c.chunks, cps, pl.bwd_data_slab_elems, dz_bytes, perm, dpar);
    };
    const bool launched = dispatch_fast<ON_TAP_MAJOR>(fast, [&](auto fv) {
        constexpr int F = decltype(fv)::value;
        if constexpr (fast_has(F, ON_ROWBLK_BWD_DATA)) {
            if (quad) return launch(IC<fast_kind(F)>{}, fv, IC<2>{});
            if (rb) return launch(IC<fast_kind(F)>{}, fv, IC<1>{});
        }
        launch(IC<fast_kind(F)>{}, fv, IC<0>{});
    });
    if (!launched) dispatch_kind(b->kind, [&](auto kind) { launch(kind, IC<FAST_GENERIC>{}, IC<0>{}); });
    return launch_ok("conv_bwd_data");
}

int kan_conv_bwd_weight(const float* dz, const float* x, const float* xn, float* dwp, const KanGeom* g, const KanBasis* b,
                        const float* x_pm, const float* dz_pm, void* stream) {
    ConvPlan cp;
    if (int rc = plan_conv(g, b, &cp)) return rc;
    const KanPlan& pl = cp.pub;
    if (!dz || !x || !xn || !dwp) return fail("null tensor pointer");
    if ((b->kind == KAN_BASIS_RELU || b->kind == KAN_BASIS_GRAM) && !b->chan_table) return fail("ReLU / Gram bases need their device parameter table (chan_table)");
    hipStream_t st = (hipStream_t)stream;
    if (cp.bwd_weight == Route::DW) {
        DevGeom dgd = dev_geom(g); DevBasis dbd = dev_basis(b);
        dim3 grid(pl.bwd_weight_splits, ngroups(g));
        dispatch_kind(b->kind, [&](auto kind) {
            hipLaunchKernelGGL((k_dw_bwd_weight<decltype(kind)::value>), grid, dim3(256), 0, st, dz, x, xn, dwp, dgd, dbd, pl.K, pl.Opad, pl.bwd_weight_slab_elems);
        });
        return launch_ok("dw_bwd_weight");
    }
    if (cp.bwd_weight == Route::BAND) {
        if (x != xn && !fast_spec(cp.fast).xn_fwd) return fail("this basis / activation pair runs on single-input kernels: pass xn == x");
        return kan_band_bwd_weight_launch(dz, x, xn, dwp, g, b, &cp.band, pl.bwd_weight_splits, pl.bwd_weight_slab_elems, stream);
    }
    const unsigned x_bytes = (unsigned)((long long)g->B * g->x_bstride * 4), dz_bytes = (unsigned)((long long)g->B * g->y_bstride * 4);
    if (cp.bwd_weight == Route::HALO) {
        if (x != xn) return fail("internal: the channel-major weight-gradient layout needs x == xn");
        const BwHaloCfg& hc = cp.bwh;
        const DevGeom dgh = dev_geom(g); const DevBasis dbh = dev_basis(b);
        if ((long long)hc.tiles_o * ngroups(g) > 65535) return fail("groups * output tiles exceed the grid limit");
        dim3 grid(hc.tiles_r, hc.tiles_o * ngroups(g), hc.splits);
        dispatch_fast<ON_HALO_BWD_WEIGHT>(cp.fast, [&](auto fv) {
            auto launch = [&](auto w, auto r, auto nimg) {
                hipLaunchKernelGGL((k_conv_bwd_weight_halo<decltype(fv)::value, decltype(w)::value, decltype(r)::value, decltype(nimg)::value>), grid,
                                   dim3(256), 0, st, dz, x, dwp, dgh, dbh, pl.K, pl.Opad, hc.n_bands, hc.bands_per_split, pl.bwd_weight_slab_elems,
                                   x_bytes, dz_bytes, hc.tiles_o);
            };
            if (g->W == 16) launch(IC<16>{}, IC<4>{}, IC<1>{});
            else if (g->W == 8) launch(IC<8>{}, IC<8>{}, IC<1>{});
            else launch(IC<4>{}, IC<4>{}, IC<2>{});
        });
        return launch_ok("conv_bwd_weight_halo");
    }
    const BwCfg& c = cp.bw;
    DevGeom dg = dev_geom(g);
    dg.pix_major = (x_pm && dz_pm && x == xn && cp.pm_bwd_weight) ? 1 : 0;
    if (dg.pix_major) { x = x_pm; xn = x_pm; dz = dz_pm; }
    DevBasis db = dev_basis(b);
    if ((long long)c.tiles_o * ngroups(g) > 65535) return fail("groups * output tiles exceed the grid limit");
    dim3 grid(c.tiles_r, c.tiles_o * ngroups(g), pl.bwd_weight_splits);
    const int cps = dg.pix_major ? pl.bwd_weight_target : ceil_div(c.chunks, pl.bwd_weight_splits);
    if (x != xn && !fast_spec(cp.fast).xn_fwd)
        return fail("this basis / activation pair runs on single-input kernels: pass xn == x");
    auto launch = [&](auto kind, auto fast, auto wr, auto wc) {
        constexpr int WR = decltype(wr)::value, WC = decltype(wc)::value;
        hipLaunchKernelGGL((k_conv_bwd_weight<decltype(kind)::value, decltype(fast)::value, WR, WC>), grid, dim3(WR * WC * 64), 0, st, dz, x, xn, dwp,
                           dg, db, pl.K, pl.Opad, c.chunks, cps, pl.bwd_weight_slab_elems, x_bytes, dz_bytes, c.tiles_o);
    };
    auto tiles = [&](auto kind, auto fast) {
        if (c.TO == 128) launch(kind, fast, IC<2>{}, IC<2>{});
        else launch(kind, fast, IC<4>{}, IC<1>{});
    };
    const bool fast = dispatch_fast<ON_TAP_MAJOR>(cp.fast, [&](auto fv) {
        constexpr int F = decltype(fv)::value;
        if constexpr (fast_has(F, ON_BIG_TILES)) {
            if (c.TO == 256) return launch(IC<fast_kind(F)>{}, fv, IC<2>{}, IC<4>{});
        }
        tiles(IC<fast_kind(F)>{}, fv);
    });
    if (!fast) dispatch_kind(b->kind, [&](auto kind) { tiles(kind, IC<FAST_GENERIC>{}); });
    return launch_ok("conv_bwd_weight");
}

int kan_position_major_expanded(const float* x, float* e_pm, const KanGeom* g, const KanBasis* b, void* stream) {
    ConvPlan cp;
    if (int rc = plan_conv(g, b, &cp)) return rc;
    const KanPlan& pl = cp.pub;
    if (!x || !e_pm) return fail("null tensor pointer");
    if (!pl.e_pm_wanted) return fail("this geometry / basis does not use the expanded position-major copy (plan.e_pm_wanted)");
    const int G = ngroups(g), CHW = G * g->C * g->H * g->W;
    DevBasis db = dev_basis(b);
    dim3 grid(ceil_div(CHW, 32), ceil_div(g->B, 32));
    float* dump = e_pm + (pl.e_pm_elems - 256);
    if ((b->kind == KAN_BASIS_RELU || b->kind == KAN_BASIS_GRAM) && !b->chan_table) return fail("ReLU / Gram bases need their device parameter table (chan_table)");
    dispatch_fast<ON_EXPANDED>(cp.fast, [&](auto fv) {
        constexpr int F = decltype(fv)::value;
        hipLaunchKernelGGL((k_expand_pm<fast_kind(F), F>), grid, dim3(256), 0, (hipStream_t)stream, x, e_pm, db, g->B, CHW, g->H * g->W, g->C, g->x_bstride, dump);
    });
    return launch_ok("position_major_expanded");
}

static int conv_fwd_expanded_impl(const float* e_pm, const float* wp, float* z, const KanGeom* g, const KanBasis* b, void* stream, int order) {
    ConvPlan cp;
    if (int rc = plan_conv(g, b, &cp)) return rc;
    const KanPlan& pl = cp.pub;
    if (!e_pm || !wp || !z) return fail("null tensor pointer");
    if (cp.fwd != Route::EXPANDED) return fail("the forward of this geometry / basis does not read the expanded position-major copy (plan.fwd_expanded)");
    if (order >= 0 && order != 0 && order != KAN_ORDER_FWD_WEIGHT_SIDE) return fail("order must be 0 or KAN_ORDER_FWD_WEIGHT_SIDE");
    if (order == KAN_ORDER_FWD_WEIGHT_SIDE && !cp.fwd_wq) return fail("this geometry does not offer the weight-side order (kan_tile_orders)");
    const FwdCfg& c = cp.fc;
    DevGeom dg = dev_geom(g);
    dg.pix_major = 1;
    if ((long long)c.tiles_o * ngroups(g) > 65535) return fail("groups * output tiles exceed the grid limit");
    if (order < 0 ? cp.fwd_wq : order != 0) {
        if ((size_t)z & 15) return fail("the weight-side forward stores 16-byte groups: z must be 16-byte aligned");
        dim3 grid(c.tiles_p, c.tiles_o * ngroups(g), pl.fwd_splits);
        hipLaunchKernelGGL((k_conv_fwd_pmdma_wq<18>), grid, dim3(256), 0, (hipStream_t)stream, e_pm, wp, z, dg, pl.Opad, c.chunks, pl.fwd_target,
                           pl.fwd_slab_elems, (unsigned)(((long long)pl.e_pm_elems - 256) * 4), (unsigned)((long long)pl.Kpad * pl.Opad * 4), c.tiles_o,
                           cp.pmdma_xcd ? 1 : 0);
        return launch_ok("conv_fwd_expanded");
    }
    TilePerm perm; perm.n = 0;
    if (!cp.pmdma_xcd) {
        const int tpp = ceil_div(g->B, c.TP), cpt = ceil_div(g->C, pl.IPC);
        perm = tile_perm(c.tiles_p, [&](int t) { return live_taps_out(g, t / tpp) * cpt; });
    }
    dim3 grid(c.tiles_p, c.tiles_o * ngroups(g), pl.fwd_splits);
    hipLaunchKernelGGL((k_conv_fwd_pmdma<18>), grid, dim3(256), 0, (hipStream_t)stream, e_pm, wp, z, dg, pl.P, make_fastdiv(pl.P), pl.Opad, c.chunks,
                       pl.fwd_target, pl.fwd_slab_elems, (unsigned)(((long long)pl.e_pm_elems - 256) * 4),
                       (unsigned)((long long)pl.Kpad * pl.Opad * 4), perm, c.tiles_o, cp.pmdma_xcd ? 1 : 0);
    return launch_ok("conv_fwd_expanded");
}

int kan_conv_fwd_expanded(const float* e_pm, const float* wp, float* z, const KanGeom* g, const KanBasis* b, void* stream) {
    return conv_fwd_expanded_impl(e_pm, wp, z, g, b, stream, -1);
}

int kan_conv_fwd_expanded_order(const float* e_pm, const float* wp, float* z, const KanGeom* g, const KanBasis* b, void* stream, int order) {
    if (order < 0) return fail("order must be 0 or KAN_ORDER_FWD_WEIGHT_SIDE");
    return conv_fwd_expanded_impl(e_pm, wp, z, g, b, stream, order);
}

int kan_conv_bwd_weight_expanded(const float* dz_pm, const float* e_pm, float* dwp, const KanGeom* g, const KanBasis* b, void* stream) {
    ConvPlan cp;
    if (int rc = plan_conv(g, b, &cp)) return rc;
    const KanPlan& pl = cp.pub;
    if (!dz_pm || !e_pm || !dwp) return fail("null tensor pointer");
    if (cp.bwd_weight != Route::EXPANDED) return fail("the weight gradient of this geometry / basis does not read the expanded position-major copy (plan.bwd_weight_expanded)");
    const BwCfg& c = cp.bw;
    DevGeom dg = dev_geom(g);
    dg.pix_major = 1;
    if ((long long)c.tiles_o * ngroups(g) > 65535) return fail("groups * output tiles exceed the grid limit");
    dim3 grid(c.tiles_r, c.tiles_o * ngroups(g), pl.bwd_weight_splits);
    PmOrder ord; ord.n = 0; ord.xcd = 0;
    const int T = g->kh * g->kw, S = pl.bwd_weight_splits, trpt = (g->C * pl.P) / 128;
    if (cp.pm_lpt && T * S <= PM_ORDER_MAX && T <= 255 && S <= 255 && trpt * T == c.tiles_r) {
        int steps[PM_ORDER_MAX], idx[PM_ORDER_MAX], n = 0;
        unsigned char tp[PM_ORDER_MAX], zz[PM_ORDER_MAX];
        const int per_pos = ceil_div(g->B, 16), tgt = pl.bwd_weight_target > 0 ? pl.bwd_weight_target : 1;
        for (int tap = 0; tap < T; ++tap) {
            const int L = live_positions_for_tap(g, tap) * per_pos;
            int St = ceil_div(L, tgt); St = St < 1 ? 1 : St; St = St > S ? S : St;
            for (int z = 0; z < S; ++z) {
                steps[n] = z < St ? (int)((long long)L * (z + 1) / St - (long long)L * z / St) : 0;
                tp[n] = (unsigned char)tap; zz[n] = (unsigned char)z; idx[n] = n; ++n;
            }
        }
        for (int i = 1; i < n; ++i) {
            const int v = idx[i]; int j = i;
            while (j > 0 && steps[idx[j - 1]] < steps[v]) { idx[j] = idx[j - 1]; --j; }
            idx[j] = v;
        }
        const int per_entry = trpt * c.tiles_o * ngroups(g);
        ord.n = n; ord.tiles_r_per_tap = trpt; ord.xcd = cp.pm_xcd ? 1 : 0;
        for (int i = 0; i < n; ++i) { ord.tap[i] = tp[idx[i]]; ord.z[i] = zz[idx[i]]; ord.first[i] = i * per_entry; }
        ord.first[n] = n * per_entry;
        grid = dim3((unsigned)(n * per_entry), 1, 1);
    }
    hipLaunchKernelGGL(k_conv_bwd_weight_pmdma, grid, dim3(256), 0, (hipStream_t)stream, dz_pm, e_pm, dwp, dg, pl.P, make_fastdiv(pl.P), pl.K, pl.Opad, c.chunks,
                       pl.bwd_weight_target, pl.bwd_weight_slab_elems, (unsigned)(((long long)pl.e_pm_elems - 256) * 4),
                       (unsigned)((long long)g->B * g->y_bstride * 4), c.tiles_o, pl.bwd_weight_splits, ord);
    return launch_ok("conv_bwd_weight_expanded");
}

int kan_slab_reduce(const float* slabs, int n_slabs, long long slab_elems, float* out, int B, int Cn, int HW, long long bstride, void* stream) {
    if (!slabs || !out || n_slabs < 1) return fail("bad slab_reduce arguments");
    long long total = (long long)B * Cn * HW;
    int blocks = (int)((total + 255) / 256); if (blocks > 4096) blocks = 4096; if (blocks < 1) blocks = 1;
    hipLaunchKernelGGL(k_slab_reduce, dim3(blocks), dim3(256), 0, (hipStream_t)stream, slabs, n_slabs, slab_elems, out, Cn, HW, bstride, total);
    return launch_ok("slab_reduce");
}

static bool norm_float2_ok(const void* z, const void* z_out, long long bstride, int HW, long long slab_elems) {
    return ((bstride | HW) & 1) == 0 && (((size_t)z | (size_t)z_out) & 7) == 0 && (slab_elems & 1) == 0;
}
static int norm_pool_mode(const void* pidx, const PoolGeo& pg) { return !pidx ? KAN_NORM_POOL_NONE : pg.k ? KAN_NORM_POOL_K : KAN_NORM_POOL_2X2; }

static int instnorm_fwd_any(const float* z, int n_slabs, long long slab_elems, float* z_out, const float* gamma, const float* beta,
                            const float* prelu_a, float* y, float* mean, float* rstd, int B, int Cn, int HW, long long bstride, float eps,
                            int prelu_span, unsigned char* pidx, int W, void* stream, PoolGeo pg = PoolGeo{}) {
    if (!z || !z_out || !y || !mean || !rstd || n_slabs < 1 || B < 1 || Cn < 1 || HW < 1) return fail("bad instnorm_fwd arguments");
    hipStream_t st = (hipStream_t)stream;
    int planes = B * Cn;
    const KanNormRoute r = norm_route(false, planes, HW, norm_pool_mode(pidx, pg), norm_float2_ok(z, z_out, bstride, HW, slab_elems));
    bool ok;
    if (r.kernel == KAN_NORM_REGS && r.pool)
        ok = pick_regs_pool2(r, [&](auto v) { launch_in_fwd_regs<decltype(v)::G, decltype(v)::EPL, decltype(v)::PPI, true>(st, r, planes, z, n_slabs, slab_elems, z_out, gamma, beta, prelu_a, y, mean, rstd, Cn, HW, bstride, eps, prelu_span, pidx, W); });
    else if (r.kernel == KAN_NORM_REGS)
        ok = pick_regs_plain(r, [&](auto v) { launch_in_fwd_regs<decltype(v)::G, decltype(v)::EPL, decltype(v)::PPI, false>(st, r, planes, z, n_slabs, slab_elems, z_out, gamma, beta, prelu_a, y, mean, rstd, Cn, HW, bstride, eps, prelu_span, pidx, W); });
    else
        ok = pick_generic(r, [&](auto v) { launch_in_fwd<decltype(v)::G>(st, r, planes, z, n_slabs, slab_elems, z_out, gamma, beta, prelu_a, y, mean, rstd, Cn, HW, bstride, eps, prelu_span, pidx, W, pg); });
    if (!ok) return fail("instnorm_fwd: no kernel for the route");
    return launch_ok("instnorm_fwd");
}

int kan_instnorm_prelu_fwd(const float* z, int n_slabs, long long slab_elems, float* z_out, const float* gamma, const float* beta,
                           const float* prelu_a, float* y, float* mean, float* rstd, int B, int Cn, int HW, long long bstride, float eps,
                           int prelu_span, void* stream) {
    return instnorm_fwd_any(z, n_slabs, slab_elems, z_out, gamma, beta, prelu_a, y, mean, rstd, B, Cn, HW, bstride, eps, prelu_span, nullptr, 0,
                            stream);
}

int kan_instnorm_prelu_pool_fwd(const float* z, int n_slabs, long long slab_elems, float* z_out, const float* gamma, const float* beta,
                                const float* prelu_a, float* y_pooled, unsigned char* pool_idx, float* mean, float* rstd, int B, int Cn,
                                int H, int W, long long bstride, float eps, int prelu_span, void* stream) {
    if (!pool_idx || H < 2 || W < 2 || (H & 1) || (W & 1)) return fail("fused 2x2 max-pool needs even H and W and an index buffer");
    return instnorm_fwd_any(z, n_slabs, slab_elems, z_out, gamma, beta, prelu_a, y_pooled, mean, rstd, B, Cn, H * W, bstride, eps, prelu_span,
                            pool_idx, W, stream);
}

static int instnorm_bwd_any(const float* dy, const float* z, const float* mean, const float* rstd, const float* gamma, const float* beta,
                            const float* prelu_a, float* dz, float* dgamma, float* dbeta, float* dprelu, int B, int Cn, int HW,
                            long long bstride, int prelu_span, const unsigned char* pidx, int W, void* stream, PoolGeo pg = PoolGeo{}) {
    if (!dy || !z || !mean || !rstd || !dz || B < 1 || Cn < 1 || HW < 1) return fail("bad instnorm_bwd arguments");
    hipStream_t st = (hipStream_t)stream;
    int planes = B * Cn;
    const KanNormRoute r = norm_route(true, planes, HW, norm_pool_mode(pidx, pg), true);
    bool ok;
    if (r.kernel == KAN_NORM_REGS)
        ok = pick_regs_plain(r, [&](auto v) { launch_in_bwd_regs<decltype(v)::G, decltype(v)::EPL, decltype(v)::PPI>(st, r, planes, dy, z, mean, rstd, gamma, beta, prelu_a, dz, dgamma, dbeta, dprelu, Cn, HW, bstride, prelu_span, pidx, W); });
    else
        ok = pick_generic(r, [&](auto v) { launch_in_bwd<decltype(v)::G>(st, r, planes, dy, z, mean, rstd, gamma, beta, prelu_a, dz, dgamma, dbeta, dprelu, Cn, HW, bstride, prelu_span, pidx, W, pg); });
    if (!ok) return fail("instnorm_bwd: no kernel for the route");
    return launch_ok("instnorm_bwd");
}

int kan_instnorm_prelu_bwd(const float* dy, const float* z, const float* mean, const float* rstd, const float* gamma, const float* beta,
                           const float* prelu_a, float* dz, float* dgamma, float* dbeta, float* dprelu, int B, int Cn, int HW,
                           long long bstride, int prelu_span, void* stream) {
    return instnorm_bwd_any(dy, z, mean, rstd, gamma, beta, prelu_a, dz, dgamma, dbeta, dprelu, B, Cn, HW, bstride, prelu_span, nullptr, 0, stream);
}

int kan_instnorm_prelu_pool_bwd(const float* dy_pooled, const unsigned char* pool_idx, const float* z, const float* mean, const float* rstd,
                                const float* gamma, const float* beta, const float* prelu_a, float* dz, float* dgamma, float* dbeta,
                                float* dprelu, int B, int Cn, int H, int W, long long bstride, int prelu_span, void* stream) {
    if (!pool_idx || H < 2 || W < 2 || (H & 1) || (W & 1)) return fail("fused 2x2 max-pool needs even H and W and the forward's index buffer");
    return instnorm_bwd_any(dy_pooled, z, mean, rstd, gamma, beta, prelu_a, dz, dgamma, dbeta, dprelu, B, Cn, H * W, bstride, prelu_span,
                            pool_idx, W, stream);
}

static int pool_geo(int H, int W, int k, int st, PoolGeo* pg) {
    if (k < 2 || k > 15 || st < 1 || st > k || H < k || W < k) return fail("fused max-pool: need 2 <= kernel <= 15, 1 <= stride <= kernel, plane >= kernel");
    pg->k = k; pg->s = st; pg->Hp = (H - k) / st + 1; pg->Wp = (W - k) / st + 1;
    pg->divWp = make_fastdiv(pg->Wp); pg->divS = make_fastdiv(st); pg->divK = make_fastdiv(k); pg->nc = (k + st - 1) / st; pg->divNc = make_fastdiv(pg->nc); pg->lds = 0;
    return 0;
}

int kan_instnorm_prelu_poolk_fwd(const float* z, int n_slabs, long long slab_elems, float* z_out, const float* gamma, const float* beta,
                                 const float* prelu_a, float* y_pooled, unsigned char* pool_idx, float* mean, float* rstd, int B, int Cn,
                                 int H, int W, long long bstride, float eps, int prelu_span, int pool_k, int pool_s, void* stream) {
    PoolGeo pg;
    if (!pool_idx) return fail("fused max-pool needs an index buffer");
    if (pool_geo(H, W, pool_k, pool_s, &pg)) return -1;
    return instnorm_fwd_any(z, n_slabs, slab_elems, z_out, gamma, beta, prelu_a, y_pooled, mean, rstd, B, Cn, H * W, bstride, eps, prelu_span,
                            pool_idx, W, stream, pg);
}

int kan_instnorm_prelu_poolk_bwd(const float* dy_pooled, const unsigned char* pool_idx, const float* z, const float* mean, const float* rstd,
                                 const float* gamma, const float* beta, const float* prelu_a, float* dz, float* dgamma, float* dbeta,
                                 float* dprelu, int B, int Cn, int H, int W, long long bstride, int prelu_span, int pool_k, int pool_s,
                                 void* stream) {
    PoolGeo pg;
    if (!pool_idx) return fail("fused max-pool needs the forward's index buffer");
    if (pool_geo(H, W, pool_k, pool_s, &pg)) return -1;
    return instnorm_bwd_any(dy_pooled, z, mean, rstd, gamma, beta, prelu_a, dz, dgamma, dbeta, dprelu, B, Cn, H * W, bstride, prelu_span,
                            pool_idx, W, stream, pg);
}

int kan_norm_route(int backward, int B, int Cn, int H, int W, long long bstride, int n_slabs, long long slab_elems, int pool2x2, int pool_k,
                   int pool_s, int aligned8, KanNormRoute* route) {
    if (!route || n_slabs < 1 || B < 1 || Cn < 1 || H < 1 || W < 1) return fail("bad norm_route arguments");
    if (pool2x2 && (pool_k || H < 2 || W < 2 || (H & 1) || (W & 1))) return fail("fused 2x2 max-pool needs even H and W");
    PoolGeo pg{};
    if (pool_k && pool_geo(H, W, pool_k, pool_s, &pg)) return -1;
    const int HW = H * W;
    *route = norm_route(backward != 0, B * Cn, HW, pool_k ? KAN_NORM_POOL_K : pool2x2 ? KAN_NORM_POOL_2X2 : KAN_NORM_POOL_NONE,
                        aligned8 && norm_float2_ok(nullptr, nullptr, bstride, HW, slab_elems));
    return 0;
}

int kan_adamw_step(float* p, const float* g, float* m, float* v, long long n, double lr, double beta1, double beta2, double eps,
                   double weight_decay, int step, float grad_scale, void* stream) {
    if (!p || !g || !m || !v) return fail("null tensor pointer");
    if (n < 0 || step < 1) return fail("adamw: n must be >= 0 and step >= 1");
    if (((uintptr_t)p | (uintptr_t)g | (uintptr_t)m | (uintptr_t)v) & 15u) return fail("adamw: blocks must be 16-byte aligned");
    if (n == 0) return 0;
    const AdamArgs a = adam_args(lr, beta1, beta2, eps, weight_decay, step, grad_scale);
    long long blocks = ((n >> 2) + 255) / 256;
    if (blocks > 256 * 16) blocks = 256 * 16;
    if (blocks < 1) blocks = 1;
    hipLaunchKernelGGL(k_adamw, dim3((unsigned)blocks), dim3(256), 0, (hipStream_t)stream, p, g, m, v, n, a);
    return launch_ok("adamw");
}

int kan_adamw_step_segments(float* p, float* m, float* v, const unsigned long long* seg_grad, const long long* seg_off, const int* seg_n,
                            const int* chunk_seg, const int* chunk_start, const float* seg_bias, int n_chunks, int chunk_elems, double lr,
                            double beta1, double beta2, double eps, double weight_decay, int step, float grad_scale, void* stream) {
    if (!p || !m || !v || !seg_grad || !seg_off || !seg_n || !chunk_seg || !chunk_start) return fail("null tensor pointer");
    if (n_chunks < 0 || step < 1 || chunk_elems < 4 || (chunk_elems & 3)) return fail("adamw: bad chunk table or step");
    if (((uintptr_t)p | (uintptr_t)m | (uintptr_t)v) & 15u) return fail("adamw: blocks must be 16-byte aligned");
    if (n_chunks == 0) return 0;
    const AdamArgs a = adam_args(lr, beta1, beta2, eps, weight_decay, step, grad_scale);
    hipLaunchKernelGGL(k_adamw_seg, dim3((unsigned)n_chunks), dim3(256), 0, (hipStream_t)stream, p, m, v, seg_grad, seg_off, seg_n, chunk_seg,
                       chunk_start, seg_bias, chunk_elems, a);
    return launch_ok("adamw_seg");
}

static bool adam_hyper(double beta1, double beta2, double eps, double weight_decay, float grad_scale, AdamHyper* h) {
    if (!(beta1 >= 0.0 && beta1 < 1.0 && beta2 >= 0.0 && beta2 < 1.0) || !(eps >= 0.0) || !(weight_decay >= 0.0)) return false;
    h->beta1 = beta1; h->beta2 = beta2; h->eps = eps; h->weight_decay = weight_decay; h->gscale = grad_scale;
    return true;
}

int kan_adamw_advance(int* seg_step, const unsigned long long* seg_grad, int n_seg, void* stream) {
    if (!seg_step || !seg_grad) return fail("null tensor pointer");
// ... 44 lines not shown
```

convolutional-kan-for-image-classification_amd/ops.py:

```python
from __future__ import annotations

import contextlib
import ctypes as C
import os
import weakref
from collections import OrderedDict
from dataclasses import dataclass, replace
from functools import lru_cache, partial, wraps
from typing import List, NamedTuple, Optional, Sequence, Tuple

import torch
from torch.autograd.function import once_differentiable

from . import _lib as L


@dataclass(frozen=True)
class ConvSpec:
    kind: int
    n_basis: int
    order: int
    act: int
    p0: float
    p1: float
    table: Tuple[float, ...]
    kernel: Tuple[int, int]
    stride: Tuple[int, int]
    padding: Tuple[int, int]
    dilation: Tuple[int, int]
    groups: int = 1
    first: int = 0
    w_layout: int = 0

    @property
    def has_base(self) -> bool:
        return self.act != L.ACT_NONE

    def out_hw(self, H: int, W: int) -> Tuple[int, int]:
        (kh, kw), (sh, sw), (ph, pw), (dh, dw) = self.kernel, self.stride, self.padding, self.dilation
        return (H + 2 * ph - dh * (kh - 1) - 1) // sh + 1, (W + 2 * pw - dw * (kw - 1) - 1) // sw + 1


W_IOD = 1


def _outputs(spec: ConvSpec, w_basis: Sequence[torch.Tensor]) -> int:
    return w_basis[0].shape[1] if spec.w_layout == W_IOD else sum(w.shape[0] for w in w_basis)


def _device_table(spec: ConvSpec) -> bool:
    return spec.kind == L.BASIS_POLY and len(spec.table) > L.KAN_MAX_TABLE


def _basis_struct(spec: ConvSpec) -> L.KanBasis:
    b = L.KanBasis()
    b.kind, b.n_basis, b.act, b.p0, b.p1 = spec.kind, spec.n_basis, spec.act, spec.p0, spec.p1
    b.order = spec.order | (spec.first << 8)
    if _device_table(spec):
        return b
    if len(spec.table) > L.KAN_MAX_TABLE:
        raise L.KanConvError(f"basis table of {len(spec.table)} entries exceeds KAN_MAX_TABLE={L.KAN_MAX_TABLE}")
    for i, v in enumerate(spec.table):
        b.table[i] = v
    return b


@lru_cache(maxsize=512)
def _plan_cached(spec: ConvSpec, B: int, Cg: int, H: int, W: int, Og: int, C_total: int, O_total: int):
    Ho, Wo = spec.out_hw(H, W)
    if Ho <= 0 or Wo <= 0:
        raise L.KanConvError(f"empty output ({Ho}x{Wo}) for input {H}x{W}")
    g = L.KanGeom()
    g.B, g.C, g.H, g.W, g.O, g.Ho, g.Wo = B, Cg, H, W, Og, Ho, Wo
    (g.kh, g.kw), (g.sh, g.sw), (g.ph, g.pw), (g.dh, g.dw) = spec.kernel, spec.stride, spec.padding, spec.dilation
    g.x_bstride, g.y_bstride = C_total * H * W, O_total * Ho * Wo
    g.groups = spec.groups
    b = _basis_struct(spec)
    p = L.KanPlan()
    bp = b
    if _device_table(spec):
        bp = L.KanBasis.from_buffer_copy(b)
        bp.chan_table = 1
    L.check(L.load().kan_plan(C.byref(g), C.byref(bp), C.byref(p)), "kan_plan")
    p.tile_orders = L.load().kan_tile_orders(C.byref(g), C.byref(bp))
    return g, b, p


def _plan_key(spec: ConvSpec, shape, Og: int) -> tuple:
    B, Ct, H, W = shape
    return (spec, B, Ct // spec.groups, H, W, Og, Ct, Og * spec.groups)


def _with_phases(basis: L.KanBasis, phases: Optional[torch.Tensor], mode: int = 0) -> L.KanBasis:
    if phases is None:
        return basis
    b = L.KanBasis.from_buffer_copy(basis)
    b.chan_table, b.order = phases.data_ptr(), mode
    return b


_TABLES: "dict[tuple, torch.Tensor]" = {}


def _with_table(basis: L.KanBasis, spec: ConvSpec, device) -> L.KanBasis:
    if not _device_table(spec):
        return basis
    key = (spec.table, torch.device(device))
    t = _TABLES.get(key)
    if t is None:
        t = _TABLES[key] = torch.tensor(list(spec.table) + [0.0] * 3, dtype=torch.float32, device=device)
    b = L.KanBasis.from_buffer_copy(basis)
    b.chan_table = t.data_ptr()
    return b


def _ptr(t: Optional[torch.Tensor], offset: int = 0) -> C.c_void_p:
    if t is None:
        return C.c_void_p(0)
    return C.c_void_p(t.data_ptr() + 4 * offset)


def _stream(t: torch.Tensor) -> C.c_void_p:
    return C.c_void_p(torch.cuda.current_stream(t.device).cuda_stream)


def _dense(t: torch.Tensor) -> torch.Tensor:
    t = t.contiguous()
    return t.clone() if t.data_ptr() & 15 else t


def _require(t: torch.Tensor, name: str, align: bool = True) -> torch.Tensor:
    if not isinstance(t, torch.Tensor):
        raise L.KanConvError(f"{name} must be a tensor, got {type(t).__name__}")
    if not t.is_cuda:
        raise L.KanConvError(f"{name} is on {t.device}: this path runs only on a ROCm device (MI355X); there is no CPU fallback")
    if t.dtype != torch.float32:
        raise L.KanConvError(f"{name} must be float32, got {t.dtype}")
    return _dense(t) if align else t.contiguous()


def _split_weights(spec: ConvSpec, weights: Sequence[torch.Tensor]):
    G = spec.groups
    if spec.has_base:
        return list(weights[:G]), list(weights[G:2 * G])
    return [None] * G, list(weights[:G])


PROFILE: Optional[list] = None


@dataclass
class KernelSample:
    name: str
    flops: float
    executed: float
    layer: str
    start: "torch.cuda.Event"
    end: "torch.cuda.Event"


def _launch(sample, t: torch.Tensor, fn) -> None:
    name, flops, executed, layer = sample
    if PROFILE is None:
        L.check(fn(), name)
        return
    e0, e1 = torch.cuda.Event(enable_timing=True), torch.cuda.Event(enable_timing=True)
    stream = torch.cuda.current_stream(t.device)
    e0.record(stream)
    L.check(fn(), name)
    e1.record(stream)
    PROFILE.append(KernelSample(name, flops, executed, layer, e0, e1))


def _conv_flops(geom, plan) -> float:
    return 2.0 * geom.B * geom.O * geom.Ho * geom.Wo * geom.C * plan.P * geom.kh * geom.kw * max(1, geom.groups)


@lru_cache(maxsize=256)
def _live_fraction(which: str, H: int, W: int, Ho: int, Wo: int, kh: int, kw: int, sh: int, sw: int, ph: int, pw: int, dh: int, dw: int) -> float:
    live = 0
    for ho in range(Ho):
        for wo in range(Wo):
            for r in range(kh):
                for t in range(kw):
                    hi, wi = ho * sh - ph + r * dh, wo * sw - pw + t * dw
                    live += 0 <= hi < H and 0 <= wi < W
    return live / float(Ho * Wo * kh * kw)


_ROW_BLOCK_BIT = {"fwd": 1, "bwd_data": 2, "bwd_weight": 0}


def _quadrant_order(geom, plan, which: str) -> bool:
    return which == "fwd" and bool(plan.row_blocks & 1) and geom.B % 32 == 0


def _quadrant_bwd_data(geom, plan, have_dz_pm: bool) -> bool:
    return bool(have_dz_pm) and bool(plan.row_blocks & 2) and bool(getattr(plan, "tile_orders", 0) & L.ORDER_QUAD_BWD_DATA)


def _row_blocks8_forward(geom, plan) -> bool:
    return geom.H == 8 and geom.W == 8 and bool(getattr(plan, "tile_orders", 0) & L.ORDER_ROWBLK8_FWD)


def _executed_flops(geom, plan, which: str, have_dz_pm: bool = False) -> float:
    target = {"fwd": plan.fwd_target, "bwd_data": plan.bwd_data_target, "bwd_weight": plan.bwd_weight_target}[which]
    dense = _conv_flops(geom, plan)
    g = geom
    if target <= 0:
        if _quadrant_order(geom, plan, which) or (which == "bwd_data" and _quadrant_bwd_data(geom, plan, have_dz_pm)):
            return dense * _live_fraction(which, g.H, g.W, g.Ho, g.Wo, g.kh, g.kw, g.sh, g.sw, g.ph, g.pw, g.dh, g.dw)
        if plan.row_blocks & _ROW_BLOCK_BIT[which]:
            return dense * (5.0 / 6.0)
        if which == "fwd" and _row_blocks8_forward(geom, plan):
            return dense * (11.0 / 12.0)
        return dense
    return dense * _live_fraction(which, g.H, g.W, g.Ho, g.Wo, g.kh, g.kw, g.sh, g.sw, g.ph, g.pw, g.dh, g.dw)


def _layer_tag(geom) -> str:
    return f"{geom.C * max(1, geom.groups)}->{geom.O * max(1, geom.groups)}@{geom.H}x{geom.W} k{geom.kh}x{geom.kw}"


def _sample(which: str, geom, plan, pm: bool, two: bool = False, expanded: bool = False):
    tile = "128" if plan.Opad % 128 == 0 else "64"
    if which == "bwd_data":
        name = "k_conv_bwd_data"
    elif expanded:
        name = f"k_conv_{which}_pmdma/o{tile}"
    elif plan.fwd_band if which == "fwd" else plan.bwd_weight_band:
        name = f"k_band_{which}/o" + ("128" if plan.Opad % 128 == 0 else "192" if plan.Opad == 192 else "64")
    else:
        halo = plan.fwd_halo if which == "fwd" else (plan.bwd_weight_halo and not two)
        name = f"k_conv_{which}{'_halo' if halo else ''}/o{tile}"
    skips = expanded or pm or bool(plan.row_blocks & _ROW_BLOCK_BIT[which]) or (which == "fwd" and _row_blocks8_forward(geom, plan))
    dense = _conv_flops(geom, plan)
    return name, dense, _executed_flops(geom, plan, which, pm) if skips else dense, _layer_tag(geom)


def _position_major(t: torch.Tensor, ch_off: int, Cn: int) -> torch.Tensor:
    B, Ct, H, W = t.shape
    out = torch.empty(Cn * H * W * B, device=t.device, dtype=torch.float32)
    L.check(L.load().kan_position_major(_ptr(t, ch_off * H * W), _ptr(out), B, Cn, H * W, Ct * H * W, _stream(t)), "kan_position_major")
    return out


def _stack(ws: Sequence[Optional[torch.Tensor]]) -> Optional[torch.Tensor]:
    if ws[0] is None:
        return None
    return ws[0].unsqueeze(0) if len(ws) == 1 else torch.stack(list(ws))


_PACKED: "OrderedDict[tuple, PackedWeights]" = OrderedDict()
_PACK_CACHE_MAX = int(os.environ.get("KAN_PACK_CACHE", "256"))
_PACK_CACHE_BYTES = int(os.environ.get("KAN_PACK_CACHE_BYTES", str(16 << 30)))
_PACK_SAMPLE = max(1, int(os.environ.get("KAN_PACK_SAMPLE", "1")))
_PACK_VERIFY_EVERY = int(os.environ.get("KAN_PACK_VERIFY_EVERY", "16"))
_EPOCH = 0
PACK_STATS = {"calls": 0, "forced": 0, "skipped": 0}


_ALWAYS_PACK = False


@contextlib.contextmanager
def always_pack():
    global _ALWAYS_PACK
    prev, _ALWAYS_PACK = _ALWAYS_PACK, True
    try:
        yield
    finally:
        _ALWAYS_PACK = prev


@dataclass(frozen=True)
class SplitMode:
    inference: bool = False
    fwd: bool = False
    bwd_data: bool = False
    bwd_weight: bool = False


_SPLIT = SplitMode()


@contextlib.contextmanager
def _split(**on):
    global _SPLIT
    prev, _SPLIT = _SPLIT, replace(_SPLIT, **on)
    try:
        yield
    finally:
        _SPLIT = prev


def split_precision_inference():
    return _split(inference=True)


def split_precision_forward():
    return _split(fwd=True)
# ... 197 lines not shown

def _layout_key(spec: "ConvSpec", geom, plan) -> tuple:
    return (spec, geom.C, geom.O, plan.P, plan.IPC, plan.KC, plan.Kpad, plan.Opad, plan.fwd_halo, plan.fwd_band, plan.packed_weight_bytes, plan.bwd_data_weight_bytes)


@lru_cache(maxsize=512)
def _cacheable(plan_key) -> bool:
    geom, basis, _ = _plan_cached(*plan_key)
    return bool(L.load().kan_pack_cacheable(C.byref(geom), C.byref(basis)))


def _owner(w: torch.Tensor) -> torch.Tensor:
    return w._base if w._base is not None else w


def _packed_entry(key, owners):
    ent = _PACKED.get(key)
    if ent is None:
        ent = PackedWeights()
        _PACKED[key] = ent
        for o in owners:
            weakref.finalize(o, _PACKED.pop, key, None)
        while len(_PACKED) > _PACK_CACHE_MAX or (len(_PACKED) > 1 and sum(e.nbytes() for e in _PACKED.values()) > _PACK_CACHE_BYTES):
            _PACKED.popitem(last=False)
    else:
        _PACKED.move_to_end(key)
    return ent


def _pack(lib, spec, geom, basis, plan, plan_key, w_base, w_basis, need_dgrad, phases, device, st):
    def fresh():
        wp = torch.empty(plan.packed_weight_bytes // 4, device=device, dtype=torch.float32)
        wd = torch.empty(plan.bwd_data_weight_bytes // 4, device=device, dtype=torch.float32) if need_dgrad else None
        wb_all, ws_all = _stack(w_base), _stack(w_basis)
        L.check(lib.kan_pack_weights(_ptr(wb_all), _ptr(ws_all), _ptr(wp), _ptr(wd), C.byref(geom), C.byref(basis), st), "kan_pack_weights")
        return wp, wd
    if spec.w_layout == W_IOD:
        wp = torch.empty(plan.packed_weight_bytes // 4, device=device, dtype=torch.float32)
        wd = torch.empty(plan.bwd_data_weight_bytes // 4, device=device, dtype=torch.float32) if need_dgrad else None
        L.check(lib.kan_pack_weights_iod(_ptr(w_basis[0]), _ptr(wp), _ptr(wd), C.byref(geom), C.byref(basis), st), "kan_pack_weights_iod")
        return wp, wd
    if _PACK_CACHE_MAX <= 0 or spec.groups != 1 or phases is not None or not _cacheable(plan_key):
        return fresh()
    ws, wb = w_basis[0], w_base[0]
    if (ws.data_ptr() | (wb.data_ptr() if wb is not None else 0)) & 15:
        return fresh()
    owners = [_owner(w) for w in (wb, ws) if w is not None]
    if not all(o.is_leaf for o in owners):
        return fresh()
    ent = _packed_entry((_layout_key(spec, geom, plan), device.index) + tuple(id(o) for o in owners), owners)
    stamps = [(w.data_ptr(), o._version, tuple(w.shape)) for w, o in zip((w for w in (wb, ws) if w is not None), owners)]
    force = _ALWAYS_PACK or ent.wp is None or ent.stamps != stamps or (need_dgrad and ent.wd is None)
    if ent.wp is None:
        ent.wp = torch.empty(plan.packed_weight_bytes // 4, device=device, dtype=torch.float32)
        ent.ring = torch.zeros(L.KAN_FP_WORDS, device=device, dtype=torch.int64)
    if need_dgrad and ent.wd is None:
        ent.wd = torch.empty(plan.bwd_data_weight_bytes // 4, device=device, dtype=torch.float32)
    if not force and ent.epoch == _EPOCH and _PACK_VERIFY_EVERY != 1 and (_PACK_VERIFY_EVERY == 0 or ent.unverified + 1 < _PACK_VERIFY_EVERY):
        ent.unverified += 1
        PACK_STATS["skipped"] += 1
        return ent.wp, (ent.wd if need_dgrad else None)
    ent.epoch, ent.unverified = _EPOCH, 0
    if force:
        for t in (ent.wp, ent.wd):
            if t is not None:
                torch.autograd.graph.increment_version(t)
    L.check(lib.kan_pack_weights_cached(_ptr(wb), _ptr(ws), _ptr(ent.wp), _ptr(ent.wd), C.byref(geom), C.byref(basis),
                                        C.c_void_p(ent.ring.data_ptr()), ent.cur, int(force), _PACK_SAMPLE, st), "kan_pack_weights_cached")
    PACK_STATS["calls"] += 1
    PACK_STATS["forced"] += int(force)
    ent.cur = (ent.cur + 1) % 3
    ent.stamps = stamps
    return ent.wp, (ent.wd if need_dgrad else None)


def _conv_forward(spec: ConvSpec, x, xn, w_base, w_basis, need_dgrad: bool = True, phases=None):
    lib = L.load()
    Ct = x.shape[1]
    plan_key = _plan_key(spec, x.shape, _outputs(spec, w_basis) // spec.groups)
    geom, basis, plan = _plan_cached(*plan_key)
    basis = _with_table(_with_phases(basis, phases), spec, x.device)
    st = _stream(x)
    z = torch.empty((plan.fwd_splits, geom.B, geom.O * spec.groups, geom.Ho, geom.Wo), device=x.device, dtype=torch.float32)
    wp, wd = _pack(lib, spec, geom, basis, plan, plan_key, w_base, w_basis, need_dgrad, phases, x.device, st)
    if plan.fwd_expanded and xn is None:
        e_pm = _expand_pm(x, geom, basis, plan, st)
        _launch(_sample("fwd", geom, plan, True, expanded=True), x,
                lambda: lib.kan_conv_fwd_expanded(_ptr(e_pm), _ptr(wp), _ptr(z), C.byref(geom), C.byref(basis), st))
        return z, (wd, _position_major(x, 0, Ct) if plan.x_pm_wanted else e_pm), geom, basis, plan
    x_pm = _position_major(x, 0, Ct) if (plan.x_pm_wanted and xn is None) else None
    _launch(_sample("fwd", geom, plan, x_pm is not None, xn is not None), x,
            lambda: lib.kan_conv_fwd(_ptr(x), _ptr(xn if xn is not None else x), _ptr(wp), _ptr(z), C.byref(geom), C.byref(basis),
                                     _ptr(x_pm), st))
    return z, (wd, x_pm), geom, basis, plan


def _expand_pm(x, geom, basis, plan, st):
    e_pm = torch.empty(plan.e_pm_elems, device=x.device, dtype=torch.float32)
    L.check(L.load().kan_position_major_expanded(_ptr(x), _ptr(e_pm), C.byref(geom), C.byref(basis), st), "kan_position_major_expanded")
    return e_pm


class GradSink:
    __slots__ = ("ref", "view", "used")

    def __init__(self, ref, view):
        self.ref, self.view, self.used = ref, view, False


GRAD_SINKS: "dict[int, GradSink]" = {}


def _sink_for(wid, shape, device):
    ent = GRAD_SINKS.get(wid) if wid is not None else None
    if ent is None or ent.used:
        return None
    p, t = ent.ref(), ent.view
    if p is None or p.grad is not None or tuple(t.shape) != tuple(shape) or t.device != device or not t.is_contiguous():
        return None
    ent.used = True
    return t


def _conv_backward(spec: ConvSpec, x, xn, packed, dz, need_x: bool, need_xn: bool, need_w: bool, phases=None, mode: int = 0, wids=None, dparams=None, wcd=None, dw_split: bool = False):
    lib = L.load()
    B, Ct, H, W = x.shape
    G = spec.groups
    Cg = Ct // G
    Ot = dz.shape[1]
    Og = Ot // G
    geom, basis, plan = _plan_cached(*_plan_key(spec, x.shape, Og))
    basis = _with_table(_with_phases(basis, phases, mode), spec, x.device)
    kh, kw = spec.kernel
    st = _stream(x)
    xs = xn if xn is not None else x
    wd, x_pm = packed
    dw_base: List[Optional[torch.Tensor]] = [None] * G
    dw_basis: List[Optional[torch.Tensor]] = [None] * G
    split_w = need_w and dw_split
    split_x = need_x and wcd is not None
    exact_w = need_w and not split_w
    exact_x = (need_x or need_xn) and not split_x
    dz_pm = _position_major(dz, 0, Ot) if (plan.dz_pm_wanted and xn is None and (exact_w or exact_x)) else None
    if split_w:
        sb, ss = (_sink_for(wids[0], (Og, Cg, kh, kw), x.device), _sink_for(wids[1], (Og, Cg * spec.n_basis, kh, kw), x.device)) if wids else (None, None)
        dwb = sb if sb is not None else torch.empty((Og, Cg, kh, kw), device=x.device, dtype=torch.float32)
        dws = ss if ss is not None else torch.empty((Og, Cg * spec.n_basis, kh, kw), device=x.device, dtype=torch.float32)
        kan_conv_bwd_weight_split(spec, x, dz, out=(dwb, dws))
        dw_base, dw_basis = list(dwb.unsqueeze(0).unbind(0)), list(dws.unsqueeze(0).unbind(0))
    elif exact_w:
        dwp = torch.empty(plan.bwd_weight_splits * plan.bwd_weight_slab_elems, device=x.device, dtype=torch.float32)
        if plan.bwd_weight_expanded and xn is None and dz_pm is not None:
            e_pm = x_pm if (plan.fwd_expanded and not plan.x_pm_wanted and x_pm is not None and mode == 0) else _expand_pm(x, geom, basis, plan, st)
            _launch(_sample("bwd_weight", geom, plan, True, expanded=True), x,
                    lambda: lib.kan_conv_bwd_weight_expanded(_ptr(dz_pm), _ptr(e_pm), _ptr(dwp), C.byref(geom), C.byref(basis), st))
        else:
            _launch(_sample("bwd_weight", geom, plan, x_pm is not None and dz_pm is not None, xn is not None), x,
                    lambda: lib.kan_conv_bwd_weight(_ptr(dz), _ptr(x), _ptr(xs), _ptr(dwp), C.byref(geom), C.byref(basis), _ptr(x_pm),
                                                    _ptr(dz_pm), st))
        if spec.w_layout == W_IOD:
            dco = torch.empty((Cg, Og, spec.n_basis), device=x.device, dtype=torch.float32)
            L.check(lib.kan_unpack_wgrad_iod(_ptr(dwp), _ptr(dco), C.byref(geom), C.byref(basis), st), "kan_unpack_wgrad_iod")
            dw_basis = [dco]
        else:
            sb = _sink_for(wids[0], (Og, Cg, kh, kw), x.device) if (wids and G == 1 and spec.has_base) else None
            ss = _sink_for(wids[1], (Og, Cg * spec.n_basis, kh, kw), x.device) if (wids and G == 1) else None
            dwb = (sb.unsqueeze(0) if sb is not None else
                   torch.empty((G, Og, Cg, kh, kw), device=x.device, dtype=torch.float32)) if spec.has_base else None
            dws = ss.unsqueeze(0) if ss is not None else torch.empty((G, Og, Cg * spec.n_basis, kh, kw), device=x.device, dtype=torch.float32)
            L.check(lib.kan_unpack_wgrad(_ptr(dwp), _ptr(dwb), _ptr(dws), C.byref(geom), C.byref(basis), st), "kan_unpack_wgrad")
            dw_basis = list(dws.unbind(0))
            if spec.has_base:
                dw_base = list(dwb.unbind(0))
    dx = dxn = None
    if split_x:
        dx, _ = kan_conv_bwd_data_split(spec, x, dz, None, None, wcd)
    elif exact_x:
        S = plan.bwd_data_splits
        separate = xn is not None
        dxs = torch.empty((S, B, Ct, H, W), device=x.device, dtype=torch.float32)
        dxns = torch.empty_like(dxs) if separate else None
        head, tail = (_ptr(dz), _ptr(x), _ptr(xs), _ptr(wd), _ptr(dxs), _ptr(dxns)), (C.byref(geom), C.byref(basis), _ptr(dz_pm), st)
        _launch(_sample("bwd_data", geom, plan, dz_pm is not None), x,
                (lambda: lib.kan_conv_bwd_data(*head, *tail)) if dparams is None else
                (lambda: lib.kan_conv_bwd_data_params(*head, _ptr(dparams), *tail)))
        dx, dxn = _sum_slabs(dxs, B, Ct, H * W), (_sum_slabs(dxns, B, Ct, H * W) if separate else None)
    return dx, dxn, dw_base, dw_basis


def _sum_slabs(slabs: torch.Tensor, B: int, Cn: int, HW: int) -> torch.Tensor:
    if slabs.shape[0] == 1:
        return slabs[0]
    out = torch.empty_like(slabs[0])
    L.check(L.load().kan_slab_reduce(_ptr(slabs), slabs.shape[0], slabs[0].numel(), _ptr(out), B, Cn, HW, Cn * HW, _stream(slabs)),
            "kan_slab_reduce")
    return out


def _flat_grads(spec: ConvSpec, dw_base, dw_basis):
    return tuple(dw_base) + tuple(dw_basis) if spec.has_base else tuple(dw_basis)


def _save(ctx, **named) -> None:
    ctx.saved_names = tuple(k for k, t in named.items() if t is not None)
    ctx.save_for_backward(*(t for t in named.values() if t is not None))


def _once(backward):
    inner = once_differentiable(backward)

    @wraps(backward)
    def wrapper(ctx, *grads):
        if torch.is_grad_enabled() and not any(g is not None and g.requires_grad for g in grads):
            grads = tuple(g.detach().requires_grad_(True) if g is not None else None for g in grads)
        return inner(ctx, *grads)
    return wrapper


def _asked(ctx, grads: tuple) -> tuple:
    return tuple(g if need else None for g, need in zip(grads, ctx.needs_input_grad))


def _saved(ctx, *names):
    kept = dict(zip(ctx.saved_names, ctx.saved_tensors))
    return tuple(kept.get(n) for n in names)


def _is_depthwise(spec: ConvSpec, x, w_basis) -> bool:
    return x.shape[1] // spec.groups == 1 and w_basis[0].shape[0] <= 2 and spec.kernel[0] * spec.kernel[1] <= 9


class _KanConv(torch.autograd.Function):

    @staticmethod
    def forward(ctx, spec: ConvSpec, split: bool, x, xn, phases, *weights):
        x = _require(x, "x")
        xn = _require(xn, "xn") if xn is not None else None
        weights = [_require(w, "weight", align=False) for w in weights]
        w_base, w_basis = _split_weights(spec, weights)
        if spec.w_layout == W_IOD:
            want = (x.shape[1], w_basis[0].shape[1] if w_basis[0].dim() == 3 else -1, spec.n_basis)
            if len(weights) != 1 or tuple(w_basis[0].shape) != want or spec.groups != 1 or spec.kernel != (1, 1) or spec.has_base or phases is not None:
                raise L.KanConvError(f"w_layout = W_IOD takes one [inputs, outputs, n_basis] coefficient tensor, a 1x1 kernel, one group and no base branch; "
                                     f"got {[tuple(w.shape) for w in weights]} for input {tuple(x.shape)}, n_basis {spec.n_basis}")
        if phases is not None:
            phases = _require(phases, "phases")
            want = (x.shape[1] // spec.groups, 2, spec.n_basis) if spec.kind == L.BASIS_RELU else (spec.n_basis,)
            if tuple(phases.shape) != want:
                raise L.KanConvError(f"parameter table {tuple(phases.shape)} != {want} for basis kind {spec.kind}")
        need_dgrad = bool(ctx.needs_input_grad[2] or (xn is not None and ctx.needs_input_grad[3]))
        need_w = any(ctx.needs_input_grad[5:])
        with torch.cuda.device(x.device):
            zs, (wd, x_pm), _, stage = _conv_forward_or_split(spec, x, xn, phases, w_base, w_basis, split, need_dgrad, need_w)
            z = _sum_slabs(zs, zs.shape[1], zs.shape[2], zs.shape[3] * zs.shape[4])
        ctx.spec, ctx.wsplit = spec, stage.dw_split
        kept_w = {f"w_basis{g}": w for g, w in enumerate(w_basis)} if phases is not None else {}
        _save(ctx, x=x, xn=xn, phases=phases, wd=wd, x_pm=x_pm, wcd=stage.wcd, **kept_w)
        return z

    @staticmethod
    @_once
    def backward(ctx, dz):
        spec, G = ctx.spec, ctx.spec.groups
        x, xn, phases, wd, x_pm, wcd, *w_basis = _saved(ctx, "x", "xn", "phases", "wd", "x_pm", "wcd", *(f"w_basis{g}" for g in range(G)))
        packed = (wd, x_pm)
        need_x, need_xn = ctx.needs_input_grad[2], xn is not None and ctx.needs_input_grad[3]
        need_p, need_w = ctx.needs_input_grad[4], any(ctx.needs_input_grad[5:])
        dz = _dense(dz)
        dph = None
        with torch.cuda.device(x.device):
            in_epilogue = need_p and (need_x or need_xn) and not _is_depthwise(spec, x, w_basis)
            dpar = None
            if in_epilogue:
                dpar = torch.zeros_like(phases) if spec.kind == L.BASIS_RELU else phases.new_zeros((64, spec.n_basis))
            dx, dxn, dwb, dws = _conv_backward(spec, x, xn, packed, dz, need_x, need_xn, need_w, phases, dparams=dpar, wcd=wcd, dw_split=ctx.wsplit)
            if in_epilogue:
                dph = dpar if spec.kind == L.BASIS_RELU else dpar.sum(dim=0)
            if need_p and not in_epilogue:
                Cg, n = x.shape[1] // G, spec.n_basis
                W = torch.stack(list(w_basis)).view(G, -1, Cg, n, spec.kernel[0] * spec.kernel[1])

                def factor(mode):
                    _, _, _, dwm = _conv_backward(spec, x, xn, packed, dz, False, False, True, phases, mode)
                    return W * torch.stack(list(dwm)).view_as(W)
                if spec.kind == L.BASIS_RELU:
                    dph = torch.stack([factor(mode).sum(dim=(0, 1, 4)) for mode in (1, 2)], dim=1)
                else:
                    dph = torch.zeros_like(phases)
                    for mode in range(1, n - 1):
                        dph[mode + 1] = factor(mode).sum()
        return _asked(ctx, (None, None, dx, dxn, dph) + _flat_grads(spec, dwb, dws))


def _cat(ts: Sequence[Optional[torch.Tensor]]) -> Optional[torch.Tensor]:
    if ts[0] is None:
        return None
    return ts[0] if len(ts) == 1 else torch.cat([t.reshape(-1) for t in ts])


@dataclass(frozen=True, eq=False)
class BatchStats:
    running_mean: Optional[torch.Tensor]
    running_var: Optional[torch.Tensor]
    momentum: float
    training: bool

    @property
    def batch(self) -> bool:
# ... 453 lines not shown
```

include/kanconv.h:

```cpp
#ifndef KANCONV_H
#define KANCONV_H

#ifdef __cplusplus
extern "C" {
#endif

#define KAN_MAX_PLANES 16
#define KAN_MAX_TABLE  32
#define KAN_FP_WORDS   192

enum { KAN_BASIS_BSPLINE = 0, KAN_BASIS_RBF = 1, KAN_BASIS_CHEBY = 2, KAN_BASIS_POLY = 3, KAN_BASIS_FOURIER = 4, KAN_BASIS_RELU = 5, KAN_BASIS_GRAM = 6 };
enum { KAN_ACT_NONE = -1, KAN_ACT_IDENTITY = 0, KAN_ACT_GELU = 1, KAN_ACT_SILU = 2, KAN_ACT_RELU = 3,
       KAN_ACT_TANH = 4, KAN_ACT_SIGMOID = 5, KAN_ACT_GELU_TANH = 6 };

typedef struct KanGeom {
    int B, C, H, W;
    int O, Ho, Wo;
    int kh, kw, sh, sw, ph, pw, dh, dw;
    int groups;
    long long x_bstride;
    long long y_bstride;
} KanGeom;

#define KAN_ORDER_PACK(mode, first) ((int)(mode) | ((int)(first) << 8))
#define KAN_ORDER_MODE(order) ((int)(order) & 0xff)
#define KAN_ORDER_FIRST(order) ((int)(order) >> 8)
typedef struct KanBasis {
    int kind, n_basis, order, act;
    float p0, p1;
    float table[KAN_MAX_TABLE];
    const float* chan_table;
} KanBasis;

typedef struct KanPlan {
    int P;
    int K;
    int IPC, KC;
    int Kpad, Opad;
    int fwd_splits;
    int bwd_data_splits;
    int bwd_weight_splits;
    int fwd_target, bwd_data_target, bwd_weight_target;
    int x_pm_wanted, dz_pm_wanted;
    int bwd_weight_expanded;
    int row_blocks;
    int e_pm_wanted, fwd_expanded;
    int fwd_halo, bwd_weight_halo;
    int fwd_band, bwd_weight_band;
    long long packed_weight_bytes;
    long long bwd_data_weight_bytes;
    long long fwd_slab_elems;
    long long bwd_data_slab_elems;
    long long bwd_weight_slab_elems;
    long long e_pm_elems;
} KanPlan;

const char* kan_version(void);
const char* kan_last_error(void);

int kan_plan(const KanGeom* geom, const KanBasis* basis, KanPlan* plan);

#define KAN_ORDER_QUAD_FWD 1
#define KAN_ORDER_ROWBLK8_FWD 2
#define KAN_ORDER_QUAD_BWD_DATA 4
#define KAN_ORDER_FWD_WEIGHT_SIDE 8
int kan_tile_orders(const KanGeom* geom, const KanBasis* basis);

int kan_pack_weights(const float* w_base, const float* w_basis, float* wp, float* wd,
                     const KanGeom* geom, const KanBasis* basis, void* stream);

int kan_pack_weights_iod(const float* coeffs, float* wp, float* wd, const KanGeom* geom, const KanBasis* basis, void* stream);

int kan_pack_cacheable(const KanGeom* geom, const KanBasis* basis);
int kan_pack_weights_cached(const float* w_base, const float* w_basis, float* wp, float* wd,
                            const KanGeom* geom, const KanBasis* basis, unsigned long long* ring, int cur, int force,
                            int sample_stride, void* stream);

int kan_conv_fwd(const float* x, const float* xn, const float* wp, float* z,
                 const KanGeom* geom, const KanBasis* basis, const float* x_pm, void* stream);

int kan_position_major(const float* src, float* dst, int B, int Cn, int HW, long long bstride, void* stream);

int kan_conv_bwd_data(const float* dz, const float* x, const float* xn, const float* wd,
                      float* dx, float* dxn,
                      const KanGeom* geom, const KanBasis* basis, const float* dz_pm, void* stream);

int kan_conv_bwd_data_params(const float* dz, const float* x, const float* xn, const float* wd, float* dx, float* dxn, float* dparams,
                             const KanGeom* geom, const KanBasis* basis, const float* dz_pm, void* stream);

int kan_conv_bwd_weight(const float* dz, const float* x, const float* xn, float* dwp,
                        const KanGeom* geom, const KanBasis* basis, const float* x_pm, const float* dz_pm, void* stream);

int kan_position_major_expanded(const float* x, float* e_pm, const KanGeom* geom, const KanBasis* basis, void* stream);
int kan_conv_fwd_expanded(const float* e_pm, const float* wp, float* z, const KanGeom* geom, const KanBasis* basis, void* stream);
int kan_conv_fwd_expanded_order(const float* e_pm, const float* wp, float* z, const KanGeom* geom, const KanBasis* basis, void* stream, int order);
int kan_conv_bwd_weight_expanded(const float* dz_pm, const float* e_pm, float* dwp,
                                 const KanGeom* geom, const KanBasis* basis, void* stream);

int kan_unpack_wgrad(const float* dwp, float* dw_base, float* dw_basis,
                     const KanGeom* geom, const KanBasis* basis, void* stream);

int kan_unpack_wgrad_iod(const float* dwp, float* dcoeffs, const KanGeom* geom, const KanBasis* basis, void* stream);

int kan_slab_reduce(const float* slabs, int n_slabs, long long slab_elems, float* out,
                    int B, int Cn, int HW, long long bstride, void* stream);

int kan_instnorm_prelu_fwd(const float* z, int n_slabs, long long slab_elems, float* z_out,
                           const float* gamma, const float* beta, const float* prelu_a,
                           float* y, float* mean, float* rstd,
                           int B, int Cn, int HW, long long bstride, float eps, int prelu_span, void* stream);

int kan_instnorm_prelu_bwd(const float* dy, const float* z, const float* mean, const float* rstd,
                           const float* gamma, const float* beta, const float* prelu_a,
                           float* dz, float* dgamma, float* dbeta, float* dprelu,
                           int B, int Cn, int HW, long long bstride, int prelu_span, void* stream);

int kan_instnorm_prelu_pool_fwd(const float* z, int n_slabs, long long slab_elems, float* z_out,
                                const float* gamma, const float* beta, const float* prelu_a,
                                float* y_pooled, unsigned char* pool_idx, float* mean, float* rstd,
                                int B, int Cn, int H, int W, long long bstride, float eps, int prelu_span, void* stream);
int kan_instnorm_prelu_pool_bwd(const float* dy_pooled, const unsigned char* pool_idx, const float* z, const float* mean, const float* rstd,
                                const float* gamma, const float* beta, const float* prelu_a,
                                float* dz, float* dgamma, float* dbeta, float* dprelu,
                                int B, int Cn, int H, int W, long long bstride, int prelu_span, void* stream);

int kan_instnorm_prelu_poolk_fwd(const float* z, int n_slabs, long long slab_elems, float* z_out,
                                 const float* gamma, const float* beta, const float* prelu_a,
                                 float* y_pooled, unsigned char* pool_idx, float* mean, float* rstd,
                                 int B, int Cn, int H, int W, long long bstride, float eps, int prelu_span, int pool_k, int pool_s, void* stream);
int kan_instnorm_prelu_poolk_bwd(const float* dy_pooled, const unsigned char* pool_idx, const float* z, const float* mean, const float* rstd,
                                 const float* gamma, const float* beta, const float* prelu_a,
                                 float* dz, float* dgamma, float* dbeta, float* dprelu,
                                 int B, int Cn, int H, int W, long long bstride, int prelu_span, int pool_k, int pool_s, void* stream);

enum { KAN_NORM_GENERIC = 0, KAN_NORM_REGS = 1 };
enum { KAN_NORM_POOL_NONE = 0, KAN_NORM_POOL_2X2 = 1, KAN_NORM_POOL_K = 2 };
typedef struct KanNormRoute {
    int kernel, G, EPL, PPI, NT, pool, lds, held, blocks, strided;
} KanNormRoute;

int kan_norm_route(int backward, int B, int Cn, int H, int W, long long bstride, int n_slabs, long long slab_elems,
                   int pool2x2, int pool_k, int pool_s, int aligned8, KanNormRoute* route);

long long kan_batchnorm_workspace_bytes(int B, int Cn);
int kan_batchnorm_prelu_fwd(const float* z, int n_slabs, long long slab_elems, float* z_out,
                            const float* gamma, const float* beta, const float* prelu_a,
                            float* y, unsigned char* pool_idx, float* mean, float* rstd,
                            float* running_mean, float* running_var, void* workspace,
                            int B, int Cn, int H, int W, long long bstride, float eps, double momentum,
                            int prelu_span, int training, void* stream);

int kan_batchnorm_prelu_bwd(const float* dy, const unsigned char* pool_idx, const float* z, const float* mean, const float* rstd,
                            const float* gamma, const float* beta, const float* prelu_a,
                            float* dz, float* dgamma, float* dbeta, float* dprelu, void* workspace,
                            int B, int Cn, int H, int W, long long bstride, int prelu_span, int training, void* stream);

int kan_split_supported(const KanGeom* geom, const KanBasis* basis);
long long kan_split_weight_bytes(const KanGeom* geom, const KanBasis* basis);
int kan_split_pack_weights(const float* w_base, const float* w_basis, void* wc, const KanGeom* geom, const KanBasis* basis, void* stream);
int kan_conv_fwd_split(const float* x, const void* wc, float* z, const KanGeom* geom, const KanBasis* basis, void* stream);

long long kan_split_bwd_data_weight_bytes(const KanGeom* geom, const KanBasis* basis);
int kan_split_pack_weights_bwd_data(const float* w_base, const float* w_basis, void* wcd, const KanGeom* geom, const KanBasis* basis, void* stream);
int kan_conv_bwd_data_split(const float* dz, const float* x, const void* wcd, float* dx, const KanGeom* geom, const KanBasis* basis, void* stream);

long long kan_split_bwd_weight_workspace_bytes(const KanGeom* geom, const KanBasis* basis);
int kan_conv_bwd_weight_split(const float* dz, const float* x, float* dw_base, float* dw_basis, void* workspace,
                              const KanGeom* geom, const KanBasis* basis, void* stream);

int kan_adamw_step(float* p, const float* g, float* m, float* v, long long n, double lr, double beta1, double beta2, double eps,
                   double weight_decay, int step, float grad_scale, void* stream);

int kan_adamw_step_segments(float* p, float* m, float* v, const unsigned long long* seg_grad, const long long* seg_off, const int* seg_n,
                            const int* chunk_seg, const int* chunk_start, const float* seg_bias, int n_chunks, int chunk_elems, double lr,
                            double beta1, double beta2, double eps, double weight_decay, int step, float grad_scale, void* stream);

int kan_adamw_advance(int* seg_step, const unsigned long long* seg_grad, int n_seg, void* stream);

int kan_adamw_step_segments_dev(float* p, float* m, float* v, const unsigned long long* seg_grad, const long long* seg_off, const int* seg_n,
                                const int* chunk_seg, const int* chunk_start, const double* lr_dev, const int* seg_step, int n_chunks,
                                int chunk_elems, double beta1, double beta2, double eps, double weight_decay, float grad_scale, void* stream);

int kan_adamw_dev_args(const double* lr_dev, const int* step_dev, double beta1, double beta2, double eps, double weight_decay, float grad_scale,
                       float* out9, void* stream);

int kan_set_u64_table(unsigned long long* table, int first, const unsigned long long* values, int n, void* stream);

long long kan_xent_workspace_bytes(int B);
long long kan_xent_metrics_bytes(int C);
int kan_xent_fwd(const float* logits, const long long* target, int B, int C, float* loss, float* lse, void* metrics ,
                 void* workspace, void* stream);
int kan_xent_bwd(const float* logits, const long long* target, const float* lse, const float* grad_loss , float* dlogits,
                 int B, int C, void* stream);

long long kan_feed_max_image_bytes(void);
int kan_feed_batch(const unsigned char* images, const long long* labels , const int* table, long long N, int B, int C, int H, int W,
                   int Ho, int Wo, int channels_last, const float* mean , const float* std , float* data,
                   long long* target , void* stream);

int kan_feed_resize_max_ksize(void);
int kan_feed_resize_batch(const unsigned char* images, const long long* labels , const int* table, long long N, int B, int C, int H,
                          int W, int Rh, int Rw, int Ho, int Wo, int channels_last, int out_channels, const int* k1x, int ksize1x, const int* k1y,
                          int ksize1y, const int* k2x, int ksize2x, const int* k2y, int ksize2y, const float* mean ,
                          const float* std , float* data, long long* target , void* stream);

enum { KAN_WAV_MEXICAN_HAT = 0, KAN_WAV_MORLET = 1, KAN_WAV_DOG = 2, KAN_WAV_MEYER = 3, KAN_WAV_SHANNON = 4 };
typedef struct {
    int B, C, H, W, O, Ho, Wo, kh, kw, sh, sw, ph, pw, dh, dw;
    int wavelet;
    long long x_bstride, u_bstride;
} KanWavGeom;
int kan_wav_fwd(const float* x, const float* scale, const float* trans, const float* w, float* u, const KanWavGeom* geom, void* stream);
int kan_wav_bwd_input(const float* du, const float* x, const float* scale, const float* trans, const float* w, float* dx,
                      const KanWavGeom* geom, void* stream);
long long kan_wav_param_workspace(const KanWavGeom* geom);
int kan_wav_bwd_params(const float* du, const float* x, const float* scale, const float* trans, const float* w, float* dw, float* dscale,
                       float* dtrans, float* workspace, const KanWavGeom* geom, void* stream);

enum { KAN_WAV_BI_TAPS9 = 0, KAN_WAV_BI_STRIDE1 = 1, KAN_WAV_BI_STRIDED = 2 };
enum { KAN_WAV_PAR_TILED = 0, KAN_WAV_PAR_PIXEL = 1 };
typedef struct KanWavRoute {
    int TH, TW, NIMG, RH, RW, tiles_h, tiles_w, fwd_shrunk, fwd_nimg_cut, fwd_lds_bytes, fwd_fits, fwd_blocks;
    int bwd_input_kernel, bwd_input_blocks;
    int params_kernel, passes, chunks, BH, NI, RU, CU, XP, UP, bands, items, items_per_chunk, lds_bytes, px_per_chunk;
} KanWavRoute;
int kan_wav_route(const KanWavGeom* geom, KanWavRoute* route);

#ifdef __cplusplus
}
#endif
#endif
```

Measured before the change: 18140.

## Launch only live weight-gradient splits per tap and skip dead slabs in unpack

For small-spatial geometries, the expanded weight-gradient kernel now enumerates only the (tap, split) items that have live output positions, instead of launching every split for every tap. The unpack kernel gets a LIVE variant that reads only slabs actually written, using buffer loads that return zero for the skipped ones. An optional persistent (resident) mode loops blocks over work items. The aim is to remove idle blocks and redundant slab reads and zeroing in the backward weight pass for deep, tiny-feature-map layers, at the cost of more indexing logic and per-item setup.

```diff
diff --git a/convolutional-kan-for-image-classification_amd/_lib.py b/convolutional-kan-for-image-classification_amd/_lib.py
--- a/convolutional-kan-for-image-classification_amd/_lib.py
+++ b/convolutional-kan-for-image-classification_amd/_lib.py
@@ -13,6 +13,7 @@
 BASIS_BSPLINE, BASIS_RBF, BASIS_CHEBY, BASIS_POLY, BASIS_FOURIER, BASIS_RELU, BASIS_GRAM = 0, 1, 2, 3, 4, 5, 6
 ACT_NONE, ACT_IDENTITY, ACT_GELU, ACT_SILU, ACT_RELU, ACT_TANH, ACT_SIGMOID, ACT_GELU_TANH = -1, 0, 1, 2, 3, 4, 5, 6
 ORDER_QUAD_FWD, ORDER_ROWBLK8_FWD, ORDER_QUAD_BWD_DATA, ORDER_FWD_WEIGHT_SIDE = 1, 2, 4, 8
+PM_ALL_SPLITS, PM_LIVE_ITEMS, PM_RESIDENT = 0, 1, 2
 
 
 class KanGeom(C.Structure):
@@ -78,6 +79,8 @@
     "kan_conv_fwd_expanded": (_I, [_P, _P, _P, _GP, _BP, _P]),
     "kan_conv_fwd_expanded_order": (_I, [_P, _P, _P, _GP, _BP, _P, _I]),
     "kan_conv_bwd_weight_expanded": (_I, [_P, _P, _P, _GP, _BP, _P]),
+    "kan_conv_bwd_weight_expanded_mode": (_I, [_P, _P, _P, _GP, _BP, _P, _I]),
+    "kan_pm_live_split": (_I, [_GP, _I, _I, _I, _I, C.POINTER(C.c_int)]),
     "kan_unpack_wgrad": (_I, [_P, _P, _P, _GP, _BP, _P]),
     "kan_unpack_wgrad_iod": (_I, [_P, _P, _GP, _BP, _P]),
     "kan_slab_reduce": (_I, [_P, _I, _LL, _P, _I, _I, _I, _LL, _P]),
diff --git a/convolutional-kan-for-image-classification_amd/csrc/kan_internal.h b/convolutional-kan-for-image-classification_amd/csrc/kan_internal.h
--- a/convolutional-kan-for-image-classification_amd/csrc/kan_internal.h
+++ b/convolutional-kan-for-image-classification_amd/csrc/kan_internal.h
@@ -144,4 +144,43 @@
 int live_taps_out(const KanGeom* g, int hw);
 int live_taps_in(const KanGeom* g, int hw);
 int live_positions_for_tap(const KanGeom* g, int tap);
+
+constexpr int PM_ORDER_MAX = 72;
+struct PmLive { unsigned hwmask; int L, S; };
+__host__ __device__ inline int pm_seg_start(int B, int hw) { return (hw * B + 15) / 16; }
+template <class G>
+__host__ __device__ inline PmLive pm_live_splits(const G& g, int tap, int target, int max_splits) {
+    const int r = tap / g.kw, t = tap - r * g.kw, HoWo = g.Ho * g.Wo;
+    PmLive v; v.hwmask = 0u; v.L = 0;
+    for (int hw = 0; hw < HoWo; ++hw) {
+        const int ho = hw / g.Wo, wo = hw - ho * g.Wo;
+        const int hi = ho * g.sh - g.ph + r * g.dh, wi = wo * g.sw - g.pw + t * g.dw;
+        if ((unsigned)hi < (unsigned)g.H && (unsigned)wi < (unsigned)g.W) {
+            v.hwmask |= 1u << hw;
+            v.L += pm_seg_start(g.B, hw + 1) - pm_seg_start(g.B, hw);
+        }
+    }
+    const int tg = target > 0 ? target : 1, want = (v.L + tg - 1) / tg;
+    v.S = want < 1 ? 1 : want > max_splits ? max_splits : want;
+    return v;
+}
+__host__ __device__ inline int pm_live_step_pos(const PmLive& v, int B, int HoWo, int n_steps, int n) {
+    int acc = 0;
+    for (int hw = 0; hw < HoWo; ++hw) {
+        if (!((v.hwmask >> hw) & 1u)) continue;
+        const int s0 = pm_seg_start(B, hw), len = pm_seg_start(B, hw + 1) - s0;
+        if (n < acc + len) return s0 + (n - acc);
+        acc += len;
+    }
+    return n_steps;
+}
+__host__ __device__ inline void pm_split_range(const PmLive& v, int B, int HoWo, int n_steps, int z, int* ch0, int* ch1) {
+    if (z >= v.S) { *ch0 = *ch1 = n_steps; return; }
+    *ch0 = z == 0 ? 0 : pm_live_step_pos(v, B, HoWo, n_steps, (int)((long long)v.L * z / v.S));
+    *ch1 = z == v.S - 1 ? n_steps : pm_live_step_pos(v, B, HoWo, n_steps, (int)((long long)v.L * (z + 1) / v.S));
+}
+__host__ __device__ inline int pm_split_steps(const PmLive& v, int z) {
+    return z < v.S ? (int)((long long)v.L * (z + 1) / v.S - (long long)v.L * z / v.S) : 0;
+}
+
 int balance_tiles(const int* weight, int n, unsigned short* idx);
diff --git a/convolutional-kan-for-image-classification_amd/csrc/kanconv.hip b/convolutional-kan-for-image-classification_amd/csrc/kanconv.hip
--- a/convolutional-kan-for-image-classification_amd/csrc/kanconv.hip
+++ b/convolutional-kan-for-image-classification_amd/csrc/kanconv.hip
@@ -153,19 +153,29 @@
 
 constexpr int UNPACK_TO = 64, UNPACK_TJ = 32;
 __device__ __forceinline__ float4 f4_add(float4 a, float4 b) { return make_float4(a.x + b.x, a.y + b.y, a.z + b.z, a.w + b.w); }
-template <int N>
-__device__ __forceinline__ void unpack_tail(float4& r0, float4& r1, const float* a0, const float* a1, long long slab_elems) {
+struct SlabLive { unsigned long long m[32]; };
+template <bool LIVE> struct SlabRow;
+template <> struct SlabRow<false> {
+    const float* a; long long slab_elems;
+    __device__ __forceinline__ float4 ld(int s) const { return *reinterpret_cast<const float4*>(a + (size_t)s * slab_elems); }
+};
+template <> struct SlabRow<true> {
+    kan_rsrc rs; unsigned off, slab_bytes; int n;
+    __device__ __forceinline__ float4 ld(int s) const {
+        return __builtin_bit_cast(float4, __builtin_amdgcn_raw_buffer_load_b128(rs, (int)(s < n ? off + (unsigned)s * slab_bytes : KAN_OOB), 0, 0));
+    }
+};
+template <int N, class Row>
+__device__ __forceinline__ void unpack_tail(float4& r0, float4& r1, const Row& a0, const Row& a1, int sl) {
     float4 v0[N], v1[N];
 #pragma unroll
-    for (int i = 0; i < N; ++i) {
-        v0[i] = *reinterpret_cast<const float4*>(a0 + (size_t)i * slab_elems);
-        v1[i] = *reinterpret_cast<const float4*>(a1 + (size_t)i * slab_elems);
-    }
+    for (int i = 0; i < N; ++i) { v0[i] = a0.ld(sl + i); v1[i] = a1.ld(sl + i); }
 #pragma unroll
     for (int i = 0; i < N; ++i) { r0 = f4_add(r0, v0[i]); r1 = f4_add(r1, v1[i]); }
 }
+template <bool LIVE>
 __global__ __launch_bounds__(256) void k_unpack(const float* __restrict__ dwp, float* __restrict__ dst_base, float* __restrict__ dst_basis,
-                                                PackGeo q, int nb_base, int n_slabs, long long slab_elems, long long dwp_gstride) {
+                                                PackGeo q, int nb_base, int n_slabs, long long slab_elems, long long dwp_gstride, SlabLive live) {
     __shared__ float tile[UNPACK_TO][UNPACK_TJ + 1];
     const int src_kind = (int)blockIdx.x < nb_base ? 0 : 1;
     const int bx = src_kind == 0 ? blockIdx.x : blockIdx.x - nb_base;
@@ -174,8 +184,20 @@
     float* dst = (src_kind == 0 ? dst_base : dst_basis) + (size_t)blockIdx.z * q.O * J;
     const int j0 = bx * UNPACK_TJ, o0 = blockIdx.y * UNPACK_TO;
     const int ol = 4 * (threadIdx.x & 15), jl = threadIdx.x >> 4;
-    const float* a0 = dwp + (size_t)pack_row(q, src_kind, min(j0 + jl, J - 1)) * q.Opad + o0 + ol;
-    const float* a1 = dwp + (size_t)pack_row(q, src_kind, min(j0 + jl + 16, J - 1)) * q.Opad + o0 + ol;
+    const int ja = min(j0 + jl, J - 1), jb = min(j0 + jl + 16, J - 1);
+    const size_t e0 = (size_t)pack_row(q, src_kind, ja) * q.Opad + o0 + ol, e1 = (size_t)pack_row(q, src_kind, jb) * q.Opad + o0 + ol;
+    auto row = [&](size_t e, int j) {
+        if constexpr (LIVE) {
+            const int tap = j - fastdiv(j, q.divT) * q.T;
+            int n = 0;
+            for (int z = 0; z < n_slabs; ++z) n += (int)((live.m[z] >> tap) & 1ull);
+            return SlabRow<true>{make_rsrc(dwp, (unsigned)((size_t)n_slabs * slab_elems * 4 - (size_t)blockIdx.z * dwp_gstride * 4)), (unsigned)(e * 4),
+                                 (unsigned)(slab_elems * 4), n};
+        } else {
+            return SlabRow<false>{dwp + e, slab_elems};
+        }
+    };
+    const auto a0 = row(e0, ja), a1 = row(e1, jb);
     const float4 zero = make_float4(0.f, 0.f, 0.f, 0.f);
     float4 s[2][8];
 #pragma unroll
@@ -184,26 +206,19 @@
     for (; sl + 8 <= n_slabs; sl += 8) {
         float4 v[2][8];
 #pragma unroll
-        for (int i = 0; i < 8; ++i) {
-            v[0][i] = *reinterpret_cast<const float4*>(a0 + (size_t)(sl + i) * slab_elems);
-            v[1][i] = *reinterpret_cast<const float4*>(a1 + (size_t)(sl + i) * slab_elems);
-        }
+        for (int i = 0; i < 8; ++i) { v[0][i] = a0.ld(sl + i); v[1][i] = a1.ld(sl + i); }
 #pragma unroll
         for (int i = 0; i < 8; ++i) { s[0][i] = f4_add(s[0][i], v[0][i]); s[1][i] = f4_add(s[1][i], v[1][i]); }
     }
-    {
-        const float* b0 = a0 + (size_t)sl * slab_elems;
-        const float* b1 = a1 + (size_t)sl * slab_elems;
-        switch (n_slabs - sl) {
-            case 1: unpack_tail<1>(s[0][0], s[1][0], b0, b1, slab_elems); break;
-            case 2: unpack_tail<2>(s[0][0], s[1][0], b0, b1, slab_elems); break;
-            case 3: unpack_tail<3>(s[0][0], s[1][0], b0, b1, slab_elems); break;
-            case 4: unpack_tail<4>(s[0][0], s[1][0], b0, b1, slab_elems); break;
-            case 5: unpack_tail<5>(s[0][0], s[1][0], b0, b1, slab_elems); break;
-            case 6: unpack_tail<6>(s[0][0], s[1][0], b0, b1, slab_elems); break;
-            case 7: unpack_tail<7>(s[0][0], s[1][0], b0, b1, slab_elems); break;
-            default: break;
-        }
+    switch (n_slabs - sl) {
+        case 1: unpack_tail<1>(s[0][0], s[1][0], a0, a1, sl); break;
+        case 2: unpack_tail<2>(s[0][0], s[1][0], a0, a1, sl); break;
+        case 3: unpack_tail<3>(s[0][0], s[1][0], a0, a1, sl); break;
+        case 4: unpack_tail<4>(s[0][0], s[1][0], a0, a1, sl); break;
+        case 5: unpack_tail<5>(s[0][0], s[1][0], a0, a1, sl); break;
+        case 6: unpack_tail<6>(s[0][0], s[1][0], a0, a1, sl); break;
+        case 7: unpack_tail<7>(s[0][0], s[1][0], a0, a1, sl); break;
+        default: break;
     }
 #pragma unroll
     for (int r = 0; r < 2; ++r) {
@@ -1720,12 +1735,12 @@
     }
 }
 
-constexpr int PM_ORDER_MAX = 72;
 struct PmOrder { int n, tiles_r_per_tap, xcd; unsigned char tap[PM_ORDER_MAX], z[PM_ORDER_MAX]; int first[PM_ORDER_MAX + 1]; };
 
 typedef float f32x4 __attribute__((ext_vector_type(4)));
+template <bool RES>
 __global__ __launch_bounds__(256, 4) void k_conv_bwd_weight_pmdma(
-    const float* __restrict__ dz_pm, const float* __restrict__ e_pm, float* __restrict__ dwp, DevGeom g, int P, FastDiv divP, int Krows, int Opad,
+    const float* __restrict__ dz_pm0, const float* __restrict__ e_pm0, float* __restrict__ dwp0, DevGeom g, int P, FastDiv divP, int Krows, int Opad,
     int n_chunks, int chunks_per_split, long long slab_elems, unsigned e_bytes, unsigned dz_bytes, int tiles_o, int max_splits, PmOrder ord) {
     constexpr int TR = 128, TO = 128, KPX = 16, ZB = KPX * TO, AB = KPX * TR;
     __shared__ __attribute__((aligned(16))) float sA[2 * AB];
@@ -1734,33 +1749,6 @@
     const int wave = __builtin_amdgcn_readfirstlane(tid >> 6);
     const int w_r = wave >> 1, w_c = wave & 1, kh2 = lane >> 5;
     const int HoWo = g.Ho * g.Wo, HW = g.H * g.W, CP = g.C * P;
-    BlockId blk{(int)blockIdx.x, (int)blockIdx.y, (int)blockIdx.z};
-    if (ord.n) {
-        const int lin = (int)blockIdx.x;
-        int e = 0;
-        while (e + 1 < ord.n && lin >= ord.first[e + 1]) ++e;
-        const int rel0 = lin - ord.first[e], per = ord.first[e + 1] - ord.first[e], ny = per / ord.tiles_r_per_tap;
-        const int rel = ((per & 7) == 0 && (ord.first[e] & 7) == 0 && ord.xcd) ? (rel0 & 7) * (per >> 3) + (rel0 >> 3) : rel0;
-        const int xr = rel / ny, y = rel - xr * ny;
-        blk.x = (int)ord.tap[e] * ord.tiles_r_per_tap + xr; blk.y = y; blk.z = (int)ord.z[e];
-    }
-    const int grp = blk.y / tiles_o;
-    const int k0 = blk.x * TR, o_tile0 = (blk.y - grp * tiles_o) * TO;
-    e_pm += (size_t)grp * g.C * HW * P * g.B;
-    dz_pm += (size_t)grp * g.O * HoWo * g.B;
-    dwp += (size_t)grp * Krows * Opad;
-    const int tap = k0 / CP, tr = tap / g.kw, tt = tap - tr * g.kw;
-    const kan_rsrc e_rs = make_rsrc(e_pm, e_bytes), dz_rs = make_rsrc(dz_pm, dz_bytes);
-
-    unsigned aoff[2], zoff[2];
-#pragma unroll
-    for (int j = 0; j < 2; ++j) {
-        const int rl = 16 * (wave * 2 + j) + (lane >> 2), cs = (lane & 3) ^ ((rl >> 2) & 3);
-        const int row = k0 + rl, rem = min(row, Krows - 1) - tap * CP, c = fastdiv(rem, divP), pp = rem - c * P;
-        const unsigned va = (unsigned)(((c * HW) * P + pp) * g.B + cs * 4) * 4u, vz = (unsigned)((o_tile0 + rl) * HoWo * g.B + cs * 4) * 4u;
-        aoff[j] = row < Krows ? va : KAN_OOB;
-        zoff[j] = o_tile0 + rl < g.O ? vz : KAN_OOB;
-    }
     unsigned aA[2][2], bB[2][2];
 #pragma unroll
     for (int mi = 0; mi < 2; ++mi) {
@@ -1771,6 +1759,11 @@
             bB[mi][h] = lds_addr(sZ + ol * KPX + (((2 * h + kh2) ^ ((ol >> 2) & 3)) * 4));
         }
     }
+    int k0, o_tile0, tr, tt, ch, ch1;
+    unsigned hwmask;
+    float* out;
+    kan_rsrc e_rs, dz_rs;
+    unsigned aoff[2], zoff[2];
     auto issue = [&](int ch, int buf) {
         const int px = ch * KPX, pos = px / g.B, b0 = px - pos * g.B;
         const int ho = pos / g.Wo, wo = pos - ho * g.Wo;
@@ -1784,28 +1777,6 @@
             __builtin_amdgcn_raw_ptr_buffer_load_lds(dz_rs, (__attribute__((address_space(3))) void*)(dZ + j * 256), 16, (int)zoff[j], sz, 0, 0);
         }
     };
-
-    f32x16 acc[2][2];
-#pragma unroll
-    for (int a = 0; a < 2; ++a)
-#pragma unroll
-        for (int b = 0; b < 2; ++b)
-#pragma unroll
-            for (int r = 0; r < 16; ++r) acc[a][b][r] = 0.f;
-
-    unsigned hwmask = 0;
-    for (int hw = 0; hw < HoWo; ++hw) hwmask |= (tap_alive_out(g, hw, tap) ? 1u : 0u) << hw;
-    auto seg = [&](int hw) { return (hw * g.B + KPX - 1) / KPX; };
-    int ch0, ch1;
-    {
-        const int L = live_step_count(hwmask, HoWo, n_chunks, seg);
-        const int S = min(max_splits, max(1, (L + chunks_per_split - 1) / chunks_per_split));
-        if (blk.z >= S) { ch0 = ch1 = n_chunks; }
-        else {
-            ch0 = blk.z == 0 ? 0 : live_step_pos(hwmask, HoWo, n_chunks, (int)((long long)L * blk.z / S), seg);
-            ch1 = blk.z == S - 1 ? n_chunks : live_step_pos(hwmask, HoWo, n_chunks, (int)((long long)L * (blk.z + 1) / S), seg);
-        }
-    }
     auto next_live = [&](int ch) -> int {
         while (ch < ch1) {
             const int hw = (ch * KPX) / g.B;
@@ -1814,8 +1785,39 @@
         }
         return ch1;
     };
-    int ch = next_live(ch0);
-    if (ch < ch1) issue(ch, 0);
+    auto take = [&](int lin) {
+        BlockId blk{(int)blockIdx.x, (int)blockIdx.y, (int)blockIdx.z};
+        if (ord.n) {
+            int e = 0;
+            while (e + 1 < ord.n && lin >= ord.first[e + 1]) ++e;
+            const int rel0 = lin - ord.first[e], per = ord.first[e + 1] - ord.first[e], ny = per / ord.tiles_r_per_tap;
+            const int rel = ((per & 7) == 0 && (ord.first[e] & 7) == 0 && ord.xcd) ? (rel0 & 7) * (per >> 3) + (rel0 >> 3) : rel0;
+            const int xr = rel / ny, y = rel - xr * ny;
+            blk.x = (int)ord.tap[e] * ord.tiles_r_per_tap + xr; blk.y = y; blk.z = (int)ord.z[e];
+        }
+        const int grp = blk.y / tiles_o;
+        k0 = blk.x * TR; o_tile0 = (blk.y - grp * tiles_o) * TO;
+        const int tap = k0 / CP;
+        tr = tap / g.kw; tt = tap - tr * g.kw;
+        e_rs = make_rsrc(e_pm0 + (size_t)grp * g.C * HW * P * g.B, e_bytes);
+        dz_rs = make_rsrc(dz_pm0 + (size_t)grp * g.O * HoWo * g.B, dz_bytes);
+        out = dwp0 + (size_t)grp * Krows * Opad + (size_t)blk.z * slab_elems;
+#pragma unroll
+        for (int j = 0; j < 2; ++j) {
+            const int rl = 16 * (wave * 2 + j) + (lane >> 2), cs = (lane & 3) ^ ((rl >> 2) & 3);
+            const int row = k0 + rl, rem = min(row, Krows - 1) - tap * CP, c = fastdiv(rem, divP), pp = rem - c * P;
+            const unsigned va = (unsigned)(((c * HW) * P + pp) * g.B + cs * 4) * 4u, vz = (unsigned)((o_tile0 + rl) * HoWo * g.B + cs * 4) * 4u;
+            aoff[j] = row < Krows ? va : KAN_OOB;
+            zoff[j] = o_tile0 + rl < g.O ? vz : KAN_OOB;
+        }
+        const PmLive live = pm_live_splits(g, tap, chunks_per_split, max_splits);
+        hwmask = live.hwmask;
+        int ch0;
+        pm_split_range(live, g.B, HoWo, n_chunks, blk.z, &ch0, &ch1);
+        ch = next_live(ch0);
+        if (ch < ch1) issue(ch, 0);
+    };
+
 #define KAN_RD4(CUR, h_)                                                                                                    \
     asm volatile("ds_read_b128 %0, %4 offset:%8\n\tds_read_b128 %1, %5 offset:%8\n\tds_read_b128 %2, %6 offset:%8\n\tds_read_b128 %3, %7 offset:%8" \
                  : "=&v"(fa[h_][0]), "=&v"(fa[h_][1]), "=&v"(fb[h_][0]), "=&v"(fb[h_][1])                                      \
@@ -1842,27 +1844,44 @@
         KAN_PM_HALF(1)                                                                                       \
     } while (0)
     static_assert(AB == ZB, "one immediate serves both operands");
-    while (ch < ch1) {
-        KAN_PM_STEP(0);
-        if (ch < ch1) { KAN_PM_STEP(1); }
-    }
+    const int n_items = ord.first[ord.n];
+    f32x16 acc[2][2];
+    auto store_tile = [&](float* st) {
+#pragma unroll
+        for (int mi = 0; mi < 2; ++mi)
+#pragma unroll
+            for (int r = 0; r < 16; ++r)
+#pragma unroll
+                for (int ni = 0; ni < 2; ++ni) st[(size_t)(mi * 32 + (r & 3) + 8 * (r >> 2)) * Opad + ni * 32] = acc[mi][ni][r];
+    };
+    float* st = nullptr;
+    for (int item = (int)blockIdx.x;;) {
+        if constexpr (RES) {
+            if (st) __syncthreads();
+        }
+        take(item);
+        if constexpr (RES) {
+            if (st) store_tile(st);
+        }
+#pragma unroll
+        for (int a = 0; a < 2; ++a)
+#pragma unroll
+            for (int b = 0; b < 2; ++b)
+#pragma unroll
+                for (int r = 0; r < 16; ++r) acc[a][b][r] = 0.f;
+        while (ch < ch1) {
+            KAN_PM_STEP(0);
+            if (ch < ch1) { KAN_PM_STEP(1); }
+        }
+        st = out + (size_t)(k0 + w_r * 64 + 4 * (lane >> 5)) * Opad + o_tile0 + w_c * 64 + (lane & 31);
+        if constexpr (!RES) break;
+        item += (int)gridDim.x;
+        if (item >= n_items) break;
+    }
+    store_tile(st);
 #undef KAN_PM_STEP
 #undef KAN_PM_HALF
 #undef KAN_RD4
-
-    float* out = dwp + (size_t)blk.z * slab_elems;
-#pragma unroll
-    for (int mi = 0; mi < 2; ++mi)
-#pragma unroll
-        for (int r = 0; r < 16; ++r) {
-            const int row = k0 + w_r * 64 + mi * 32 + mfma_row(r, lane);
-            if (row >= Krows) continue;
-#pragma unroll
-            for (int ni = 0; ni < 2; ++ni) {
-                const int o = o_tile0 + w_c * 64 + ni * 32 + (lane & 31);
-                out[(size_t)row * Opad + o] = acc[mi][ni][r];
-            }
-        }
 }
 
 
@@ -2809,6 +2828,12 @@
     return pack_weights_impl(w_base, w_basis, wp, wd, g, b, force ? nullptr : ring, cur, stream);
 }
 
+static bool pm_listed(const KanGeom* g, const ConvPlan& cp) {
+    const int T = g->kh * g->kw, S = cp.pub.bwd_weight_splits, trpt = (g->C * cp.pub.P) / 128;
+    return cp.bwd_weight == Route::EXPANDED && cp.pm_lpt && T * S <= PM_ORDER_MAX && T <= 64 && S < 32 && trpt * T == cp.bw.tiles_r &&
+           (long long)S * cp.pub.bwd_weight_slab_elems * 4 < (1ll << 31);
+}
+
 static int unpack_wgrad_impl(const float* dwp, float* dw_base, float* dw_basis, const KanGeom* g, const KanBasis* b, void* stream, bool iod) {
     ConvPlan cp;
     if (int rc = plan_conv(g, b, &cp)) return rc;
@@ -2832,7 +2857,16 @@
         hipLaunchKernelGGL(k_unpack_iod, dim3(l.blocks), dim3(256), 0, st, dwp, dw_basis, q, l.o_tiles, l.n_tiles, n_slabs, pl.bwd_weight_slab_elems,
                            iod_vec(dw_basis, dwp, g, b));
     } else {
-        hipLaunchKernelGGL(k_unpack, grid, dim3(256), 0, st, dwp, dw_base, dw_basis, q, nb_base, n_slabs, pl.bwd_weight_slab_elems, dwp_gs);
+        SlabLive live{};
+        const bool listed = pm_listed(g, cp) && n_slabs == pl.bwd_weight_splits;
+        for (int tap = 0; listed && tap < T; ++tap) {
+            const int S = pm_live_splits(*g, tap, pl.bwd_weight_target, pl.bwd_weight_splits).S;
+            for (int z = 0; z < S; ++z) live.m[z] |= 1ull << tap;
+        }
+        if (listed)
+            hipLaunchKernelGGL(k_unpack<true>, grid, dim3(256), 0, st, dwp, dw_base, dw_basis, q, nb_base, n_slabs, pl.bwd_weight_slab_elems, dwp_gs, live);
+        else
+            hipLaunchKernelGGL(k_unpack<false>, grid, dim3(256), 0, st, dwp, dw_base, dw_basis, q, nb_base, n_slabs, pl.bwd_weight_slab_elems, dwp_gs, live);
     }
     return launch_ok("unpack");
 }
@@ -3054,6 +3088,8 @@
     const BwCfg& c = cp.bw;
     DevGeom dg = dev_geom(g);
     dg.pix_major = (x_pm && dz_pm && x == xn && cp.pm_bwd_weight) ? 1 : 0;
+    if (!dg.pix_major && pm_listed(g, cp))
+        return fail("the weight-gradient slabs of this geometry hold live splits only (plan.bwd_weight_expanded): call kan_conv_bwd_weight_expanded, or pass x_pm and dz_pm");
     if (dg.pix_major) { x = x_pm; xn = x_pm; dz = dz_pm; }
     DevBasis db = dev_basis(b);
     if ((long long)c.tiles_o * ngroups(g) > 65535) return fail("groups * output tiles exceed the grid limit");
@@ -3140,28 +3176,32 @@
     return conv_fwd_expanded_impl(e_pm, wp, z, g, b, stream, order);
 }
 
-int kan_conv_bwd_weight_expanded(const float* dz_pm, const float* e_pm, float* dwp, const KanGeom* g, const KanBasis* b, void* stream) {
+static int pm_shipped_mode(const KanGeom*) { return KAN_PM_LIVE_ITEMS; }
+
+static int conv_bwd_weight_expanded_impl(const float* dz_pm, const float* e_pm, float* dwp, const KanGeom* g, const KanBasis* b, void* stream, int mode) {
     ConvPlan cp;
     if (int rc = plan_conv(g, b, &cp)) return rc;
     const KanPlan& pl = cp.pub;
     if (!dz_pm || !e_pm || !dwp) return fail("null tensor pointer");
     if (cp.bwd_weight != Route::EXPANDED) return fail("the weight gradient of this geometry / basis does not read the expanded position-major copy (plan.bwd_weight_expanded)");
+    const bool listed = pm_listed(g, cp);
+    if (mode >= 0 && mode != KAN_PM_ALL_SPLITS && !listed) return fail("this geometry runs the plain grid over all splits only (mode KAN_PM_ALL_SPLITS)");
+    if (mode < 0) mode = listed ? pm_shipped_mode(g) : KAN_PM_ALL_SPLITS;
     const BwCfg& c = cp.bw;
     DevGeom dg = dev_geom(g);
     dg.pix_major = 1;
     if ((long long)c.tiles_o * ngroups(g) > 65535) return fail("groups * output tiles exceed the grid limit");
     dim3 grid(c.tiles_r, c.tiles_o * ngroups(g), pl.bwd_weight_splits);
-    PmOrder ord; ord.n = 0; ord.xcd = 0;
+    PmOrder ord; ord.n = 0; ord.xcd = 0; ord.first[0] = 0;
     const int T = g->kh * g->kw, S = pl.bwd_weight_splits, trpt = (g->C * pl.P) / 128;
-    if (cp.pm_lpt && T * S <= PM_ORDER_MAX && T <= 255 && S <= 255 && trpt * T == c.tiles_r) {
+    if (listed) {
         int steps[PM_ORDER_MAX], idx[PM_ORDER_MAX], n = 0;
         unsigned char tp[PM_ORDER_MAX], zz[PM_ORDER_MAX];
-        const int per_pos = ceil_div(g->B, 16), tgt = pl.bwd_weight_target > 0 ? pl.bwd_weight_target : 1;
         for (int tap = 0; tap < T; ++tap) {
-            const int L = live_positions_for_tap(g, tap) * per_pos;
-            int St = ceil_div(L, tgt); St = St < 1 ? 1 : St; St = St > S ? S : St;
+            const PmLive live = pm_live_splits(*g, tap, pl.bwd_weight_target, S);
             for (int z = 0; z < S; ++z) {
-                steps[n] = z < St ? (int)((long long)L * (z + 1) / St - (long long)L * z / St) : 0;
+                if (z >= live.S && mode != KAN_PM_ALL_SPLITS) break;
+                steps[n] = pm_split_steps(live, z);
                 tp[n] = (unsigned char)tap; zz[n] = (unsigned char)z; idx[n] = n; ++n;
             }
         }
@@ -3176,10 +3216,38 @@
         ord.first[n] = n * per_entry;
         grid = dim3((unsigned)(n * per_entry), 1, 1);
     }
-    hipLaunchKernelGGL(k_conv_bwd_weight_pmdma, grid, dim3(256), 0, (hipStream_t)stream, dz_pm, e_pm, dwp, dg, pl.P, make_fastdiv(pl.P), pl.K, pl.Opad, c.chunks,
-                       pl.bwd_weight_target, pl.bwd_weight_slab_elems, (unsigned)(((long long)pl.e_pm_elems - 256) * 4),
-                       (unsigned)((long long)g->B * g->y_bstride * 4), c.tiles_o, pl.bwd_weight_splits, ord);
+    const unsigned e_bytes = (unsigned)(((long long)pl.e_pm_elems - 256) * 4), dz_bytes = (unsigned)((long long)g->B * g->y_bstride * 4);
+    if (mode == KAN_PM_RESIDENT) {
+        int dev = 0, cus = 0;
+        if (hipGetDevice(&dev) != hipSuccess || hipDeviceGetAttribute(&cus, hipDeviceAttributeMultiprocessorCount, dev) != hipSuccess || cus < 1)
+            return fail("cannot read the device's compute-unit count");
+        const unsigned slots = (unsigned)((4 * cus) & ~7) < 8u ? 8u : (unsigned)((4 * cus) & ~7);
+        if (grid.x > slots) grid.x = slots;
+        hipLaunchKernelGGL(k_conv_bwd_weight_pmdma<true>, grid, dim3(256), 0, (hipStream_t)stream, dz_pm, e_pm, dwp, dg, pl.P, make_fastdiv(pl.P), pl.K, pl.Opad,
+                           c.chunks, pl.bwd_weight_target, pl.bwd_weight_slab_elems, e_bytes, dz_bytes, c.tiles_o, pl.bwd_weight_splits, ord);
+    } else {
+        hipLaunchKernelGGL(k_conv_bwd_weight_pmdma<false>, grid, dim3(256), 0, (hipStream_t)stream, dz_pm, e_pm, dwp, dg, pl.P, make_fastdiv(pl.P), pl.K, pl.Opad,
+                           c.chunks, pl.bwd_weight_target, pl.bwd_weight_slab_elems, e_bytes, dz_bytes, c.tiles_o, pl.bwd_weight_splits, ord);
+    }
     return launch_ok("conv_bwd_weight_expanded");
+}
+
+int kan_conv_bwd_weight_expanded(const float* dz_pm, const float* e_pm, float* dwp, const KanGeom* g, const KanBasis* b, void* stream) {
+    return conv_bwd_weight_expanded_impl(dz_pm, e_pm, dwp, g, b, stream, -1);
+}
+
+int kan_conv_bwd_weight_expanded_mode(const float* dz_pm, const float* e_pm, float* dwp, const KanGeom* g, const KanBasis* b, void* stream, int mode) {
+    if (mode != KAN_PM_ALL_SPLITS && mode != KAN_PM_LIVE_ITEMS && mode != KAN_PM_RESIDENT) return fail("mode must be KAN_PM_ALL_SPLITS, KAN_PM_LIVE_ITEMS or KAN_PM_RESIDENT");
+    return conv_bwd_weight_expanded_impl(dz_pm, e_pm, dwp, g, b, stream, mode);
+}
+
+int kan_pm_live_split(const KanGeom* g, int tap, int target, int max_splits, int z, int* out4) {
+    if (!g || !out4 || tap < 0 || tap >= g->kh * g->kw || g->Ho * g->Wo > 32 || g->Ho * g->Wo < 1 || max_splits < 1 || z < 0) return fail("bad live-split arguments");
+    const PmLive live = pm_live_splits(*g, tap, target, max_splits);
+    const int HoWo = g->Ho * g->Wo;
+    out4[0] = live.S; out4[1] = live.L;
+    pm_split_range(live, g->B, HoWo, pm_seg_start(g->B, HoWo), z, &out4[2], &out4[3]);
+    return 0;
 }
 
 int kan_slab_reduce(const float* slabs, int n_slabs, long long slab_elems, float* out, int B, int Cn, int HW, long long bstride, void* stream) {
diff --git a/convolutional-kan-for-image-classification_amd/ops.py b/convolutional-kan-for-image-classification_amd/ops.py
--- a/convolutional-kan-for-image-classification_amd/ops.py
+++ b/convolutional-kan-for-image-classification_amd/ops.py
@@ -147,6 +147,7 @@
 
 
 PROFILE: Optional[list] = None
+PM_BWD_WEIGHT_MODE: Optional[int] = None
 
 
 @dataclass
@@ -650,8 +651,10 @@
         dwp = torch.empty(plan.bwd_weight_splits * plan.bwd_weight_slab_elems, device=x.device, dtype=torch.float32)
         if plan.bwd_weight_expanded and xn is None and dz_pm is not None:
             e_pm = x_pm if (plan.fwd_expanded and not plan.x_pm_wanted and x_pm is not None and mode == 0) else _expand_pm(x, geom, basis, plan, st)
+            head = (_ptr(dz_pm), _ptr(e_pm), _ptr(dwp), C.byref(geom), C.byref(basis), st)
             _launch(_sample("bwd_weight", geom, plan, True, expanded=True), x,
-                    lambda: lib.kan_conv_bwd_weight_expanded(_ptr(dz_pm), _ptr(e_pm), _ptr(dwp), C.byref(geom), C.byref(basis), st))
+                    (lambda: lib.kan_conv_bwd_weight_expanded(*head)) if PM_BWD_WEIGHT_MODE is None else
+                    (lambda: lib.kan_conv_bwd_weight_expanded_mode(*head, PM_BWD_WEIGHT_MODE)))
         else:
             _launch(_sample("bwd_weight", geom, plan, x_pm is not None and dz_pm is not None, xn is not None), x,
                     lambda: lib.kan_conv_bwd_weight(_ptr(dz), _ptr(x), _ptr(xs), _ptr(dwp), C.byref(geom), C.byref(basis), _ptr(x_pm),
diff --git a/include/kanconv.h b/include/kanconv.h
--- a/include/kanconv.h
+++ b/include/kanconv.h
@@ -96,6 +96,12 @@
 int kan_conv_fwd_expanded_order(const float* e_pm, const float* wp, float* z, const KanGeom* geom, const KanBasis* basis, void* stream, int order);
 int kan_conv_bwd_weight_expanded(const float* dz_pm, const float* e_pm, float* dwp,
                                  const KanGeom* geom, const KanBasis* basis, void* stream);
+#define KAN_PM_ALL_SPLITS 0
+#define KAN_PM_LIVE_ITEMS 1
+#define KAN_PM_RESIDENT 2
+int kan_conv_bwd_weight_expanded_mode(const float* dz_pm, const float* e_pm, float* dwp,
+                                      const KanGeom* geom, const KanBasis* basis, void* stream, int mode);
+int kan_pm_live_split(const KanGeom* geom, int tap, int target, int max_splits, int z, int* out4);
 
 int kan_unpack_wgrad(const float* dwp, float* dw_base, float* dw_basis,
                      const KanGeom* geom, const KanBasis* basis, void* stream);
```

Result: no change. 18160, median of 6 (+0.1%).
